# lionnus/I-ViT

Hardware: AMD Instinct MI355X
Metric: images/sec DeiT-B INT8 @batch256, 1→8 MI355X; % INT8 MFMA peak (higher is better)
Workload: dtype int8; 1 GPU; DeiT-B INT8 integer-only forward, batch 256 per GPU, 224x224; global_batch=256, parallelism=dp1, launch=hip-graph replay, bitwidth=8, activation_ranges=power-of-two, operators=I-ViT (IVITIntLayerNorm, Shiftmax, ShiftGELU)

## Files before the change

i-vit_amd/_lib.py:

```python
from __future__ import annotations

import ctypes as C
import os
import subprocess

_HERE = os.path.dirname(os.path.abspath(__file__))
LIB_PATH = os.path.join(_HERE, "libivit_hip.so")
CSRC = os.path.join(_HERE, "csrc")

i64, i32, u32, f32, vp = C.c_int64, C.c_int32, C.c_uint32, C.c_float, C.c_void_p
ci = C.c_int

SIGNATURES = {
    "ivit_quantize_input_f32_i8": [vp, vp, i64, f32, vp],
    "ivit_quantize_patchify_f32_i8": [vp, vp, ci, ci, ci, ci, f32, vp],
    "ivit_gemm_i8_requant": [vp, i64, vp, i64, vp, vp, vp, vp, i64, ci, ci, ci, vp],
    "ivit_gemm_i8_requant_residual": [vp, i64, vp, i64, vp, vp, vp, vp, i64, u32, i32, u32, i32, vp, i64, ci, ci, ci, vp],
    "ivit_attention_fused_i8_ex": [vp, vp, ci, ci, ci, ci, u32, i32, f32, u32, i32, ci, vp],
    "ivit_layernorm_i8_ex": [vp, i64, ci, ci, vp, vp, vp, vp, vp, i64, ci, vp],
    "ivit_layernorm_i8_compat": [vp, i64, ci, ci, vp, vp, vp, vp, vp, vp, vp, i64, ci, vp],
    "ivit_attention_fused_i8_compat": [vp, vp, ci, ci, ci, ci, u32, i32, f32, u32, i32, vp, ci, vp],
    "ivit_attention_fused_i8_compat_band": [vp, vp, ci, ci, ci, ci, u32, i32, f32, u32, i32, vp, vp, ci, ci, vp],
    "ivit_attention_fused_i8_wide": [vp, vp, ci, ci, ci, ci, u32, i32, f32, u32, i32, vp, vp, ci, ci, ci, vp],
    "ivit_attention_fused_i8_long": [vp, vp, ci, ci, ci, ci, u32, i32, f32, u32, i32, vp, vp, ci, ci, vp],
    "ivit_attention_fused_i8_wide_long": [vp, vp, ci, ci, ci, ci, u32, i32, f32, u32, i32, vp, vp, ci, ci, ci, vp],
    "ivit_attention_cls_i8": [vp, vp, vp, vp, i64, ci, ci, ci, ci, u32, i32, f32, u32, i32, vp, vp, ci, vp],
    "ivit_shiftgelu_build_lut_ex": [f32, u32, i32, vp, vp, vp],
    "ivit_shiftgelu_lut_i8_ex": [vp, i64, ci, ci, vp, vp, i64, ci, vp],
    "ivit_pack_weight_frags_i8": [vp, i64, ci, ci, vp, vp],
    "ivit_pack_weight_frags16_i8": [vp, i64, ci, ci, vp, vp],
    "ivit_tile_operand_i8": [vp, i64, i64, ci, vp, vp],
    "ivit_untile_operand_i8": [vp, i64, ci, vp, i64, vp],
    "ivit_gemm_i8_requant_ex": [vp, i64, vp, i64, vp, vp, vp, vp, i64, ci, ci, ci, ci, vp],
    "ivit_gemm_i8_requant_residual_ex": [vp, i64, vp, i64, vp, vp, vp, vp, i64, u32, i32, u32, i32, vp, i64, ci, ci, ci, ci, vp],
    "ivit_gemm_i8_requant_bits_ex": [vp, i64, vp, i64, vp, vp, vp, vp, i64, ci, ci, ci, ci, ci, vp],
    "ivit_gemm_i8_requant_residual_bits_ex": [vp, i64, vp, i64, vp, vp, vp, vp, i64, u32, i32, u32, i32, vp, i64, ci, ci, ci, ci, ci, ci, vp],
    "ivit_gemm_i8_requant_qkv_ex": [vp, i64, vp, i64, vp, vp, vp, vp, ci, ci, ci, ci, ci, ci, ci, vp],
    "ivit_gemm_i8_requant_qkv_planes_ex": [vp, i64, vp, i64, vp, vp, vp, vp, ci, ci, ci, ci, ci, ci, ci, ci, ci, vp],
    "ivit_gemm_plan": [ci, ci, ci, ci, ci, vp],
    "ivit_gemm_i8_requant_residual_i16": [vp, i64, vp, i64, vp, vp, vp, vp, i64, u32, i32, u32, i32, vp, i64, ci, ci, ci, vp],
    "ivit_gemm_i8_requant_lut_ex": [vp, i64, vp, i64, vp, vp, vp, vp, vp, i64, ci, ci, ci, ci, vp],
    "ivit_gemm_i8_requant_i16": [vp, i64, vp, i64, vp, vp, vp, vp, i64, ci, ci, ci, vp],
    "ivit_gemm_i8_requant_residual_i16_ex": [vp, i64, vp, i64, vp, vp, vp, vp, i64, u32, i32, u32, i32, vp, i64, ci, ci, ci, ci, vp],
    "ivit_gemm_i8_requant_i16_residual_i16_ex": [vp, i64, vp, i64, vp, vp, vp, vp, i64, u32, i32, u32, i32, vp, i64, ci, ci, ci, ci, vp],
    "ivit_gemm_i8_requant_qkv": [vp, i64, vp, i64, vp, vp, vp, vp, ci, ci, ci, ci, ci, ci, vp],
    "ivit_gemm_i8_i32": [vp, i64, vp, i64, vp, vp, i64, ci, ci, ci, vp],
    "ivit_attention_fused_i8": [vp, vp, ci, ci, ci, ci, u32, i32, f32, u32, i32, vp],
    "ivit_layernorm_i8": [vp, i64, ci, ci, vp, vp, vp, vp, vp, i64, vp],
    "ivit_layernorm_i32_f32": [vp, i64, ci, ci, vp, vp, vp, i64, vp],
    "ivit_layernorm_i8_f32": [vp, i64, ci, ci, ci, ci, ci, vp, vp, vp, vp, vp, i64, ci, vp],
    "ivit_layernorm_i16_f32": [vp, i64, ci, ci, ci, ci, ci, f32, vp, vp, vp, i64, ci, vp],
    "ivit_ibert_layernorm_i8_f32": [vp, i64, ci, ci, ci, ci, ci, f32, vp, vp, f32, vp, i64, ci, vp],
    "ivit_ibert_layernorm_i16_f32": [vp, i64, ci, ci, ci, ci, ci, f32, vp, vp, f32, vp, i64, ci, vp],
    "ivit_layernorm_f32_f32": [vp, i64, ci, ci, vp, ci, vp, vp, vp, i64, vp],
    "ivit_layernorm_f32_f32_ex": [vp, i64, ci, ci, vp, ci, vp, vp, vp, i64, ci, vp],
    "ivit_shiftmax_f32_i8": [vp, i64, ci, ci, f32, vp, i64, vp],
    "ivit_shiftmax_f32_i16": [vp, i64, ci, ci, f32, ci, vp, i64, vp],
    "ivit_bgemm_pv_i16_i8": [vp, vp, vp, ci, ci, ci, ci, vp],
    "ivit_bgemm_pv_i32_i8": [vp, vp, vp, ci, ci, ci, ci, i64, vp],
    "ivit_quantize_input_f32_i32": [vp, vp, i64, f32, ci, vp],
    "ivit_shiftgelu_i8": [vp, i64, ci, ci, f32, u32, i32, vp, i64, vp],
    "ivit_shiftgelu_i8_i32": [vp, i64, ci, ci, f32, vp, i64, vp],
    "ivit_shiftgelu_build_lut": [f32, u32, i32, vp, vp],
    "ivit_shiftgelu_lut_i8": [vp, i64, ci, ci, vp, vp, i64, vp],
    "ivit_shiftmax_i8": [vp, i64, ci, ci, f32, vp, i64, vp],
    "ivit_requant_i32": [vp, i64, ci, vp, vp, ci, vp, vp, vp, ci, ci, vp, vp],
    "ivit_residual_requant_i8": [vp, u32, i32, vp, u32, i32, vp, i64, vp],
    "ivit_residual_requant_i8_bits": [vp, u32, i32, vp, u32, i32, vp, i64, ci, vp],
    "ivit_embed_assemble_i8": [vp, vp, vp, u32, i32, vp, ci, ci, ci, vp],
    "ivit_embed_assemble_i8_bits": [vp, vp, vp, u32, i32, vp, ci, ci, ci, ci, vp],
    "ivit_embed_assemble_i16": [vp, vp, vp, u32, i32, vp, ci, ci, ci, vp],
    "ivit_head_argmax": [vp, vp, ci, ci, vp, vp, vp],
    "ivit_head_topk": [vp, vp, ci, ci, ci, ci, vp, vp, vp, vp, vp],
    "ivit_logits_topk_f32": [vp, ci, ci, ci, ci, vp, vp, vp, vp],
    "ivit_bgemm_qk_i8": [vp, vp, vp, ci, ci, ci, ci, vp],
    "ivit_bgemm_pv_i8": [vp, vp, vp, ci, ci, ci, ci, vp],
    "ivit_f32_to_i32": [vp, i64, ci, vp, ci, ci, vp, vp],
    "ivit_i32_to_f32": [vp, i64, ci, vp, ci, vp, vp],
    "ivit_narrow_i32_i8": [vp, vp, i64, vp, vp],
    "ivit_quantize_patchify_ld_f32_i8": [vp, vp, i64, ci, ci, ci, ci, f32, vp],
    "ivit_quantize_patchify_u8_i8": [vp, vp, i64, ci, ci, ci, ci, vp, vp],
    "ivit_quantize_patchify_hw_f32_i8": [vp, vp, i64, ci, ci, ci, ci, ci, f32, vp],
    "ivit_quantize_patchify_hw_u8_i8": [vp, vp, i64, ci, ci, ci, ci, ci, vp, vp],
    "ivit_minmax_f32": [vp, i64, vp, vp],
    "ivit_quantile_pair_f32": [vp, i64, f32, f32, vp, vp, i64, vp],
    "ivit_weight_quant_rows_f32_i8": [vp, i64, ci, ci, vp, vp, i64, vp, vp],
    "ivit_bias_quant_f32_i32": [vp, vp, ci, f32, vp, vp, vp, vp],
    "ivit_shiftmax_i32_i8": [vp, i64, ci, ci, f32, vp, i64, vp],
    "ivit_requant_i8_i16": [vp, u32, i32, vp, i64, vp],
    "ivit_residual_requant_i16": [vp, ci, vp, vp, u32, i32, vp, u32, i32, vp, i64, ci, ci, ci, ci, ci, vp],
    "ivit_layernorm_i16_i8": [vp, ci, ci, vp, vp, vp, vp, vp, i64, ci, ci, ci, ci, vp],
    "ivit_layernorm_i16_i8_compat": [vp, ci, ci, f32, ci, vp, vp, vp, vp, vp, i64, ci, ci, ci, ci, vp],
    "ivit_patch_merge_i16": [vp, vp, ci, ci, ci, ci, vp],
    "ivit_window_rows": [vp, vp, ci, ci, ci, i64, ci, ci, ci, vp],
    "ivit_avgpool_requant_i8": [vp, vp, ci, ci, ci, u32, i32, vp],
    "ivit_avgpool_requant_i8_literal": [vp, vp, ci, ci, ci, f32, u32, i32, vp],
    "ivit_avgpool_f32_literal": [vp, vp, ci, ci, ci, vp],
    "ivit_ibert_gelu_i32": [vp, i64, f32, f32, f32, vp, vp],
    "ivit_ibert_softmax_i32": [vp, i64, ci, ci, f32, f32, f32, f32, f32, u32, i32, ci, vp, i64, vp, vp],
    "ivit_ibert_layernorm_i32_f32": [vp, i64, ci, ci, vp, vp, f32, vp, i64, vp],
    "ivit_ibert_layernorm_i32_f32_ex": [vp, i64, ci, ci, vp, vp, f32, vp, i64, ci, vp],
    "ivit_ibert_gelu_build_lut": [f32, f32, f32, f32, f32, u32, i32, vp, vp],
    "ivit_ibert_softmax_build_table": [f32, f32, f32, f32, f32, f32, u32, i32, vp, vp],
    "ivit_attention_fused_i8_ibert": [vp, vp, ci, ci, ci, ci, u32, i32, u32, i32, vp, vp, ci, ci, vp],
    "ivit_attention_fused_i8_ibert_wide": [vp, vp, ci, ci, ci, ci, u32, i32, u32, i32, vp, vp, ci, ci, ci, vp],
    "ivit_attention_fused_i8_ibert_long": [vp, vp, ci, ci, ci, ci, u32, i32, u32, i32, vp, vp, ci, ci, vp],
    "ivit_attention_probs_u8": [vp, vp, i64, ci, ci, ci, ci, ci, u32, i32, f32, vp, vp, ci, vp],
    "ivit_attention_probs_u8_ibert": [vp, vp, i64, ci, ci, ci, ci, ci, u32, i32, vp, vp, ci, vp],
    "ivit_ibert_layernorm_i8": [vp, i64, ci, ci, f32, vp, vp, f32, vp, vp, vp, i64, ci, vp],
    "ivit_ibert_layernorm_i16_i8": [vp, i64, ci, ci, f32, vp, vp, f32, vp, vp, vp, i64, vp],
    "ivit_ibert_layernorm_i16_i8_ex": [vp, i64, ci, ci, f32, vp, vp, f32, vp, vp, vp, i64, ci, vp],
    "ivit_ibert_layernorm_i16_i8_win": [vp, i64, ci, ci, f32, vp, vp, f32, vp, vp, vp, i64, ci, ci, ci, ci, ci, vp],
    "ivit_ibert_gelu_f32_f32": [vp, i64, f32, f32, f32, f32, f32, vp, vp],
    "ivit_ibert_softmax_f32_f32": [vp, i64, ci, ci, f32, f32, f32, f32, f32, f32, u32, i32, ci, vp, i64, vp, vp],
    "ivit_ibert_layernorm_f32_f32": [vp, i64, ci, ci, vp, ci, vp, vp, f32, vp, i64, vp],
    "ivit_ibert_layernorm_f32_f32_ex": [vp, i64, ci, ci, vp, ci, vp, vp, f32, vp, i64, ci, vp],
    "ivit_window_attention_i8": [vp, vp, i64, vp, vp, ci, ci, ci, ci, ci, ci, u32, i32, u32, i32, f32, u32, i32, vp],
    "ivit_window_attention_i8_compat": [vp, vp, i64, vp, vp, ci, ci, ci, ci, ci, ci, u32, i32, u32, i32, f32, u32, i32, vp, vp, vp],
    "ivit_window_attention_i8_band": [vp, vp, i64, vp, vp, ci, ci, ci, ci, ci, u32, i32, u32, i32, f32, u32, i32, vp, ci, ci, ci, ci, ci, ci, vp],
    "ivit_window_attention_i8_unwindow": [vp, vp, i64, vp, vp, ci, ci, ci, ci, ci, ci, u32, i32, u32, i32, f32, u32, i32, vp, vp,
                                          ci, ci, ci, ci, vp],
    "ivit_window_attention_i8_long": [vp, vp, i64, vp, vp, ci, ci, ci, ci, ci, ci, u32, i32, u32, i32, f32, u32, i32, vp, vp, vp, ci,
                                      ci, ci, ci, ci, ci, ci, vp],
    "ivit_window_attention_i8_ibert": [vp, vp, i64, vp, vp, f32, ci, ci, ci, ci, ci, u32, i32, u32, i32, u32, i32, vp, ci, ci, ci, ci,
                                       ci, ci, vp],
    "ivit_window_attention_probs_u8": [vp, vp, i64, vp, vp, ci, ci, ci, ci, ci, ci, u32, i32, u32, i32, f32, vp, vp, vp, ci, ci, vp],
    "ivit_window_attention_probs_u8_ibert": [vp, vp, i64, vp, vp, f32, ci, ci, ci, ci, ci, u32, i32, u32, i32, vp, ci, vp],
    "ivit_eval_geometry": [ci, ci, ci, ci, vp],
    "ivit_resize_crop_workspace": [vp, ci, ci, vp, vp],
    "ivit_resize_crop_bicubic_u8": [vp, vp, vp, ci, ci, ci, ci, ci, vp, i64, vp, vp],
    "ivit_eval_geometry_hw": [ci, ci, ci, ci, ci, ci, ci, vp],
    "ivit_resize_crop_workspace_hw": [vp, ci, ci, ci, vp, vp],
    "ivit_resize_crop_bicubic_hw_u8": [vp, vp, vp, ci, ci, ci, ci, ci, ci, vp, i64, vp, vp],
    "ivit_jpeg_probe": [vp, i64, vp],
    "ivit_jpeg_plan_image": [vp, i64, vp, i64, vp],
    "ivit_jpeg_workspace": [vp, i64, vp, vp, ci, vp, vp],
    "ivit_jpeg_decode_host": [vp, i64, vp, i64],
    "ivit_jpeg_decode_u8": [vp, vp, ci, i64, i64, i64, vp, i64, vp, vp, vp],
    "ivit_tokens_to_nchw_i8_f32": [vp, i64, ci, ci, ci, ci, ci, f32, vp, vp],
    "ivit_tokens_to_nchw_i16_f32": [vp, i64, ci, ci, ci, ci, ci, f32, vp, vp],
    "ivit_tokens_to_nchw_i8": [vp, i64, ci, ci, ci, ci, ci, vp, vp],
    "ivit_tokens_to_nchw_i16": [vp, i64, ci, ci, ci, ci, ci, vp, vp],
    "ivit_dequant_rows_i8_f32": [vp, i64, i64, ci, f32, vp, i64, vp],
    "ivit_rows_rnorm_i8_f32": [vp, i64, i64, ci, vp, vp],
    "ivit_knn_topk_i8": [vp, i64, ci, vp, i64, ci, ci, vp, ci, ci, vp, vp, vp, i64, vp],
    "ivit_knn_workspace_bytes": [ci, ci, ci, ci, vp],
    "ivit_knn_vote_f32": [vp, vp, vp, ci, ci, ci, ci, vp, vp, vp],
    "ivit_gram_i8_i64": [vp, i64, i64, ci, ci, ci, vp, vp, i64, vp],
    "ivit_gram_workspace_bytes": [i64, ci, ci, vp],
    "ivit_group_sums_i8_i64": [vp, i64, i64, ci, vp, vp, ci, ci, vp, vp],
}


LAB_SIGNATURES = {
# ... 99 lines not shown
```

i-vit_amd/csrc/gemm.hip:

```cpp
#include <type_traits>
#include "gemm_common.h"

namespace {

template <int EPIW>
__global__ __launch_bounds__(NT) void gemm_i8_kernel(GemmArgs g)
{
    constexpr int EPI = epi_kind(EPIW);
    __shared__ __attribute__((aligned(16))) char smem[SMEM_BYTES + BN * 8];

    const int nblk = g.tiles_m * g.tiles_n;
    const int bid = blockIdx.x;
    const int q8 = nblk >> 3, r8 = nblk & 7, xcd = bid & 7;
    const int lid = (xcd < r8 ? xcd * (q8 + 1) : r8 * (q8 + 1) + (xcd - r8) * q8) + (bid >> 3);
    const int tm = lid / g.tiles_n, tn = lid - tm * g.tiles_n;
    const int m0 = tm * BM, n0 = tn * BN;

    const int tid = threadIdx.x;
    const int lane = tid & 63, wave = tid >> 6;
    const int wm = wave >> 1, wn = wave & 1;
    const int h = lane >> 5, l31 = lane & 31;
    if constexpr (EPI != EPI_I32 && EPI != EPI_RQ16 && EPI != EPI_RQ16_RES16) fill_rq_table(g, smem + SMEM_BYTES, n0, BN, tid);

    const int srow = tid >> 2, sc = tid & 3;
// ... 653 lines not shown
            lds_read16_async_off<128>(bq[2], ba);
            lds_read16_async_off<192>(bq[3], ba);
#pragma unroll
            for (int i = 0; i < 4; ++i) {
                lds_wait(bq[i]);
#pragma unroll
                for (int j = 0; j < 2 * TJ; ++j) acc16[i][j] = bq[i];
            }
        } else {
        v4i bq[2][4];
#pragma unroll
        for (int i = 0; i < 2; ++i)
#pragma unroll
            for (int q = 0; q < 4; ++q)
                lds_read16_async(bq[i][q], lds_addr(tab) + (unsigned)(WR_CH * 8 + 4 * (64 * wave + 32 * i + 8 * q + 4 * h)));
#pragma unroll
        for (int i = 0; i < 2; ++i)
#pragma unroll
            for (int q = 0; q < 4; ++q) {
                lds_wait(bq[i][q]);
                const v4i b4 = bq[i][q];
#pragma unroll
                for (int j = 0; j < TJ; ++j) {
                    acc[i][j][4 * q + 0] = b4.x;
                    acc[i][j][4 * q + 1] = b4.y;
                    acc[i][j][4 * q + 2] = b4.z;
                    acc[i][j][4 * q + 3] = b4.w;
                }
            }
        }
        load_frags(I0{}, I0{}, af0);
        if constexpr (ABL & 16)
            { if constexpr (ABL & 2048) tv[1] = __builtin_amdgcn_s_memtime(); else if (stamp) stamp[1] = __builtin_amdgcn_s_memtime(); }
        int kt = 0;
        for (; kt + 3 < nk; kt += 3) {
            step(kt, wr0, wr1, wr2, T{}, F{}, I0{});
            step(kt + 1, wr1, wr2, wr0, T{}, F{}, I1{});
            step(kt + 2, wr2, wr0, wr1, T{}, F{}, I2{});
        }
        step(kt, wr0, wr1, wr2, T{}, F{}, I0{});
        step(kt + 1, wr1, wr2, wr0, F{}, F{}, I1{});
        step(kt + 2, wr2, wr0, wr1, F{}, T{}, I2{});
        if constexpr (ABL & 16)
            { if constexpr (ABL & 2048) tv[2] = __builtin_amdgcn_s_memtime(); else if (stamp) stamp[2] = __builtin_amdgcn_s_memtime(); }
        const bool more = nxt.m0 >= 0;
        prefetch(more ? nxt : cur);
        struct Hook {
            decltype(table_issue)& ti;
            decltype(table_write)& tw;
            int n0;
            char* dst;
            bool more;
            mutable PersTableLoad ld;
            IVIT_DEV void issue() const { if (more) ld = ti(n0); }
            IVIT_DEV void consume() const
            {
                asm volatile("s_waitcnt vmcnt(0)" ::: "memory");
                if (more) tw(ld, dst);
            }
        };
        Hook hook{table_issue, table_write, nxt.n0, tab_next, more, PersTableLoad{0u, 0, 0, false}};
        if constexpr (ABL & 1) {
            int sum = 0;
            if constexpr (S16) {
#pragma unroll
                for (int i = 0; i < 4; ++i)
#pragma unroll
                    for (int j = 0; j < 2 * TJ; ++j) sum ^= acc16[i][j][0] ^ acc16[i][j][1] ^ acc16[i][j][2] ^ acc16[i][j][3];
            } else {
#pragma unroll
            for (int i = 0; i < 2; ++i)
#pragma unroll
                for (int j = 0; j < TJ; ++j)
#pragma unroll
                    for (int r = 0; r < 16; ++r) sum ^= acc[i][j][r];
            }
            if (sum == 0x12345679) reinterpret_cast<int*>(g.out)[tid] = sum;
            hook.issue();
            hook.consume();
        } else {
            int tid_o = tid;
            asm volatile("" : "+v"(tid_o));
            if constexpr (S16) asm volatile("s_nop 15\n\ts_nop 15" ::: "memory");
            if constexpr (S16 && (EPI == EPI_RQ || EPI == EPI_RESID || EPI == EPI_QKV)) {
                epilogue_direct_16<EPIW, 2 * TJ, (ABL & (2048 | 4096)), Hook>(acc16, g, tab, cur.m0 + wtok, cur.n0, wch, (tid_o >> 4) & 3, tid_o & 15, hook,
                                                                               g.lut ? reinterpret_cast<const unsigned char*>(smem + WR_LUT) : nullptr,
                                                                               (ABL & 2048) ? tv : nullptr);
            } else if constexpr (S16) {
                static_assert(!S16 || EPI != EPI_RQ16_RES16, "the 16-bit epilogue exists for the 32x32 form only");
                epilogue_i8_16<EPIW, 2 * TJ, BIG_NT, WR_CH, Hook>(acc16, g, cs, tab, cur.m0, cur.n0, 64 * wave, tid_o, (tid_o >> 4) & 3,
                                                                          tid_o & 15, hook,
                                                                          g.lut ? reinterpret_cast<const unsigned char*>(smem + WR_LUT) : nullptr);
            } else if constexpr (EPI == EPI_RQ16_RES16)
                epilogue_rq16_res16<TJ, BIG_NT, Hook>(acc, g, cs, cur.m0, cur.n0, 64 * wave, tid_o, (tid_o >> 5) & 1, tid_o & 31, hook);
            else
            epilogue_i8<EPIW, 2, TJ, 32 * TJ, BIG_NT, WR_CH, Hook>(acc, g, cs, tab, cur.m0, cur.n0, 64 * wave, 0, tid_o, (tid_o >> 5) & 1,
                                                                      tid_o & 31, hook,
                                                                      g.lut ? reinterpret_cast<const unsigned char*>(smem + WR_LUT) : nullptr);
        }
    };

    const int G = gridDim.x, b = blockIdx.x;
    WrWork cur = wr_work(g, 0, b, G);
    if (cur.m0 < 0) return;
    table_write(table_issue(cur.n0), smem + WR_RING + WR_CS);
    if (g.lut) smem[WR_LUT + tid] = (char)g.lut[tid];
    prefetch(cur);
    asm volatile("s_waitcnt vmcnt(1)" ::: "memory");

    for (int it = 0; cur.m0 >= 0; ++it) {
        char* tab = smem + WR_RING + WR_CS + (it & 1) * WR_TAB;
        char* tab_next = smem + WR_RING + WR_CS + ((it + 1) & 1) * WR_TAB;
        const WrWork nxt = wr_work(g, it + 1, b, G);
        if constexpr (ABL & 16) {
            unsigned long long* sbase = (ABL & 2048) ? g.stamp : reinterpret_cast<unsigned long long*>(const_cast<int8_t*>(g.res));
            stamp = (tid == 0 && it < 4) ? sbase + (blockIdx.x * 4 + it) * 32 : nullptr;
            if constexpr (ABL & 2048) {
                tv[0] = __builtin_amdgcn_s_memtime();
                tv[7] = __builtin_amdgcn_s_memrealtime();
            } else if (stamp) {
                stamp[0] = __builtin_amdgcn_s_memtime();
                stamp[16] = __builtin_amdgcn_s_memrealtime();
            }
        }
        if constexpr (S16 && (EPI == EPI_RQ || EPI == EPI_RESID || EPI == EPI_QKV) && !(ABL & 16)) {
            if (cur.half == 2) run(std::integral_constant<int, 2>{}, cur, nxt, tab, tab_next);
            else if (cur.half) run(std::integral_constant<int, 1>{}, cur, nxt, tab, tab_next);
            else run(std::integral_constant<int, 0>{}, cur, nxt, tab, tab_next);
        } else {
            if (cur.half) run(std::integral_constant<int, 1>{}, cur, nxt, tab, tab_next);
            else run(std::integral_constant<int, 0>{}, cur, nxt, tab, tab_next);
        }
        if constexpr (ABL & 16)
            {
                if constexpr (ABL & 2048) {
                    if (stamp) {
                        stamp[0] = tv[0]; stamp[1] = tv[1]; stamp[2] = tv[2]; stamp[3] = __builtin_amdgcn_s_memtime();
                        stamp[20] = tv[4]; stamp[21] = tv[5]; stamp[22] = tv[6]; stamp[16] = tv[7];
                    }
                } else if (stamp) stamp[3] = __builtin_amdgcn_s_memtime();
            }
        cur = nxt;
    }
}

constexpr int SK_MAXN = 320, SK_MAXK = 128, SK_NT = 512, SK_WPB = SK_NT / 64;
constexpr int SK_SMEM = SK_MAXN * SK_MAXK + SK_MAXN * 12 + (SK_MAXN / 4) * 4;

template <int EPIW, int NKS = 0>
__global__ __launch_bounds__(SK_NT, 2) void gemm_i8_skinny_kernel(GemmArgs g)
{
    constexpr int EPI = epi_kind(EPIW);
    constexpr int QLO = epi_lo(EPIW, EPI_NARROW_MID), QHI = epi_hi(EPIW, EPI_NARROW_MID);
    static_assert(EPI == EPI_RQ || EPI == EPI_QKV, "skinny-K form: int8 outputs");
    __shared__ __attribute__((aligned(16))) char smem[SK_SMEM];
    const int tid = threadIdx.x, lane = tid & 63, wave = tid >> 6;
    const int g4 = lane >> 4, l15 = lane & 15;
    const int nks = NKS ? NKS : (g.K >> 5), nsub = g.N >> 4;
    float2* const lohi = reinterpret_cast<float2*>(smem + SK_MAXN * SK_MAXK);
    int* const bias = reinterpret_cast<int*>(smem + SK_MAXN * SK_MAXK + SK_MAXN * 8);
    unsigned* const coff = reinterpret_cast<unsigned*>(smem + SK_MAXN * SK_MAXK + SK_MAXN * 12);
    for (int q = tid; q < nsub * nks * 64; q += SK_NT) {
        const int f = q >> 6, L = q & 63, i = f / nks, ks = f - i * nks;
        *reinterpret_cast<long*>(smem + (size_t)q * 8) =
            *reinterpret_cast<const long*>(g.W + (int64_t)(16 * i + (L & 15)) * g.ldw + 8 * nks * (L >> 4) + 8 * ks);
    }
    if constexpr (EPI == EPI_QKV) {
        const int cdim = g.heads * g.head_dim, nb = g.M / g.tokens;
        for (int j = tid; j < (g.N >> 2); j += SK_NT) {
            const int c = 4 * j, which = c / cdim, rem = c - which * cdim;
            const int hh = rem / g.head_dim, d0 = rem - hh * g.head_dim;
            coff[j] = (unsigned)(((which * nb * g.heads + hh) * g.tokens) * g.head_dim + d0);
        }
    }
    for (int c = tid; c < g.N; c += SK_NT) {
        const int bv = g.bias ? g.bias[c] : 0;
        const double M = dyadic_mult(g.m[c], g.e[c]);
        const float mf = (float)M;
        const int bits = __float_as_int(mf);
        float lo = ((double)mf > M) ? __int_as_float(bits - 1) : mf, hi = ((double)mf < M) ? __int_as_float(bits + 1) : mf;
        lo = __int_as_float(__float_as_int(lo) - 2);
        hi = __int_as_float(__float_as_int(hi) + 2);
        lohi[c] = make_float2(lo, hi);
        bias[c] = bv;
    }
    __syncthreads();
    int8_t* const out = reinterpret_cast<int8_t*>(g.out);
    const int nstrips = (g.M + 15) >> 4;
    for (int strip = blockIdx.x * SK_WPB + wave; strip < nstrips; strip += gridDim.x * SK_WPB) {
        const int t = 16 * strip + l15;
        const int8_t* arow = g.A + (int64_t)min(t, g.M - 1) * g.lda + 8 * nks * g4;
        long bf[SK_MAXK / 32] = {0l, 0l, 0l, 0l};
        if (nks == 4) {
            const int4 u0 = *reinterpret_cast<const int4*>(arow), u1 = *reinterpret_cast<const int4*>(arow + 16);
            bf[0] = ((long)(unsigned)u0.y << 32) | (unsigned)u0.x; bf[1] = ((long)(unsigned)u0.w << 32) | (unsigned)u0.z;
            bf[2] = ((long)(unsigned)u1.y << 32) | (unsigned)u1.x; bf[3] = ((long)(unsigned)u1.w << 32) | (unsigned)u1.z;
        } else if (nks == 2) {
            const int4 u0 = *reinterpret_cast<const int4*>(arow);
            bf[0] = ((long)(unsigned)u0.y << 32) | (unsigned)u0.x; bf[1] = ((long)(unsigned)u0.w << 32) | (unsigned)u0.z;
        } else {
#pragma unroll
            for (int ks = 0; ks < SK_MAXK / 32; ++ks) bf[ks] = ks < nks ? *reinterpret_cast<const long*>(arow + 8 * ks) : 0l;
        }
        unsigned qrow_off = 0;
        if constexpr (EPI == EPI_QKV) {
            const int tt = min(t, g.M - 1);
            const int qb = tt / g.tokens, qtok = tt - qb * g.tokens;
            qrow_off = (unsigned)((qb * g.heads * g.tokens + qtok) * g.head_dim);
        }
        for (int i0 = 0; i0 < nsub; i0 += 4) {
            v4i acc[4];
#pragma unroll
            for (int ii = 0; ii < 4; ++ii) {
                const int i = min(i0 + ii, nsub - 1);
                acc[ii] = *reinterpret_cast<const v4i*>(bias + 16 * i + 4 * g4);
#pragma unroll
                for (int ks = 0; ks < SK_MAXK / 32; ++ks)
                    if (ks < nks)
                        acc[ii] = __builtin_amdgcn_mfma_i32_16x16x32_i8(*reinterpret_cast<const long*>(smem + ((size_t)(i * nks + ks) * 64 + lane) * 8),
                                                                         bf[ks], acc[ii], 0, 0, 0);
            }
            int b[4][4];
            unsigned unc = 0;
#pragma unroll
            for (int ii = 0; ii < 4; ++ii) {
                const int i = min(i0 + ii, nsub - 1);
#pragma unroll
                for (int r = 0; r < 4; ++r) {
                    const float2 lh = lohi[16 * i + 4 * g4 + r];
                    const float a = (float)acc[ii][r];
                    const int tl = __float_as_int(__builtin_fmaf(a, lh.x, 12582912.0f));
                    const int th = __float_as_int(__builtin_fmaf(a, lh.y, 12582912.0f));
                    asm("v_sad_u32 %0, %1, %2, %3" : "=v"(unc) : "v"(tl), "v"(th), "v"(unc));
                    b[ii][r] = clamp_i32(tl, 0x4B400000 + QLO, 0x4B400000 + QHI);
                }
            }
            if (__builtin_amdgcn_ballot_w64(unc != 0) != 0) {
#pragma unroll
                for (int ii = 0; ii < 4; ++ii) {
                    const int c0 = 16 * min(i0 + ii, nsub - 1) + 4 * g4;
#pragma unroll
                    for (int r = 0; r < 4; ++r) {
                        const double tq = (double)acc[ii][r] * dyadic_mult(g.m[c0 + r], g.e[c0 + r]) + IVIT_MAGIC;
                        b[ii][r] = clamp_i32((int)(unsigned)__double_as_longlong(tq), QLO, QHI);
                    }
                }
            }
            unsigned D[4];
#pragma unroll
            for (int ii = 0; ii < 4; ++ii)
                D[ii] = __builtin_amdgcn_perm((unsigned)b[ii][1], (unsigned)b[ii][0], 0x0c0c0400u) |
                        __builtin_amdgcn_perm((unsigned)b[ii][3], (unsigned)b[ii][2], 0x04000c0cu);
            typedef unsigned v2u __attribute__((ext_vector_type(2)));
            const v2u ab = __builtin_amdgcn_permlane32_swap(D[0], D[2], false, false);
            const v2u cd = __builtin_amdgcn_permlane32_swap(D[1], D[3], false, false);
            const v2u ac = __builtin_amdgcn_permlane16_swap(ab.x, cd.x, false, false);
            const v2u bd = __builtin_amdgcn_permlane16_swap(ab.y, cd.y, false, false);
            const int ci = i0 + g4;
            if (ci < nsub && t < g.M) {
                const int4 v = make_int4((int)ac.x, (int)ac.y, (int)bd.x, (int)bd.y);
                if constexpr (EPI == EPI_QKV) *reinterpret_cast<int4*>(out + coff[4 * ci] + qrow_off) = v;
                else *reinterpret_cast<int4*>(out + (int64_t)t * g.ldo + 16 * ci) = v;
            }
        }
    }
}

constexpr bool epi_has_skinny(int epi) { return epi == EPI_RQ || epi == EPI_QKV; }
constexpr bool epi_has_wreg(int epi) { return epi != EPI_I32 && epi != EPI_RQ16; }
constexpr bool epi_has_wreg16(int epi) { return epi_has_wreg(epi) && epi != EPI_RQ16_RES16; }
constexpr bool epi_has_pers(int epi) { return epi_has_wreg(epi) && epi != EPI_RQ16_RES16; }
constexpr bool epi_int8_out(int epi) { return epi == EPI_RQ || epi == EPI_RESID || epi == EPI_QKV; }
constexpr bool wr_tiles_fit(int N) { return (N + WR_CH - 1) / WR_CH * WR_CH * WR_WASTE_DEN <= N * (WR_WASTE_DEN + 1); }

enum { GEMM_SMALL = IVIT_GEMM_FORM_SMALL, GEMM_PERS = IVIT_GEMM_FORM_PERS, GEMM_WREG = IVIT_GEMM_FORM_WREG, GEMM_WREG16 = IVIT_GEMM_FORM_WREG16,
       GEMM_SKINNY = IVIT_GEMM_FORM_SKINNY };
static_assert(EPI_RQ == IVIT_GEMM_EPI_RQ && EPI_RESID == IVIT_GEMM_EPI_RESID && EPI_QKV == IVIT_GEMM_EPI_QKV && EPI_I32 == IVIT_GEMM_EPI_I32 &&
              EPI_RESID16 == IVIT_GEMM_EPI_RESID16 && EPI_RQ16 == IVIT_GEMM_EPI_RQ16 && EPI_RQ16_RES16 == IVIT_GEMM_EPI_RQ16_RES16,
              "include/ivit_hip.h names the epilogue kinds for ivit_gemm_plan");

struct GemmPlan {
    int form;
    int nks;
    int res_f32;
    int narrow, stamped, ablation;
    int grid, lds;
    int tiles_m, tiles_n, split_from;
    int stagger, stagger_units, cu_turns;
};

int gemm_check(int EPI, const GemmArgs& g, const char* name, int qkv_planes)
{
    IVIT_REQUIRE(g.A && g.W && g.out, "%s: NULL operand", name);
    IVIT_REQUIRE(g.M > 0 && g.N > 0 && g.K > 0, "%s: empty problem M=%d N=%d K=%d", name, g.M, g.N, g.K);
    IVIT_REQUIRE(g.K % BK == 0, "%s: K=%d must be a multiple of %d", name, g.K, BK);
    IVIT_REQUIRE(g.lda >= g.K && g.ldw >= g.K && g.lda % 16 == 0 && g.ldw % 16 == 0,
                 "%s: lda=%lld ldw=%lld must be >= K and multiples of 16", name, (long long)g.lda, (long long)g.ldw);
    IVIT_REQUIRE(((uintptr_t)g.A % 16 == 0) && ((uintptr_t)g.W % 16 == 0) && ((uintptr_t)g.out % 16 == 0),
                 "%s: operands must be 16-byte aligned", name);
    if (EPI == EPI_I32 || EPI == EPI_RQ16 || EPI == EPI_RQ16_RES16) {
        IVIT_REQUIRE(g.N % 4 == 0 && g.ldo % 4 == 0 && g.ldo >= g.N, "%s: N=%d ldo=%lld must be multiples of 4", name,
                     g.N, (long long)g.ldo);
        if (EPI == EPI_RQ16 || EPI == EPI_RQ16_RES16)
            IVIT_REQUIRE(g.m && g.e && ((uintptr_t)g.m % 16 == 0) && ((uintptr_t)g.e % 16 == 0) && ((uintptr_t)g.out % 8 == 0),
                         "%s: requantiser tables missing or misaligned", name);
    } else {
        IVIT_REQUIRE(g.m && g.e, "%s: NULL requantiser table", name);
        IVIT_REQUIRE(((uintptr_t)g.bias % 16 == 0), "%s: bias must be 16-byte aligned", name);
        IVIT_REQUIRE(g.N % 16 == 0, "%s: N=%d must be a multiple of 16", name, g.N);
        IVIT_REQUIRE(((uintptr_t)g.m % 16 == 0) && ((uintptr_t)g.e % 16 == 0), "%s: m/e tables must be 16-byte aligned",
                     name);
    }
    if (EPI == EPI_RQ || EPI == EPI_RESID)
        IVIT_REQUIRE(g.ldo >= g.N && g.ldo % 16 == 0, "%s: ldo=%lld must be >= N and a multiple of 16", name,
                     (long long)g.ldo);
    if (EPI == EPI_RESID)
        IVIT_REQUIRE(g.res && g.ldr >= g.N && g.ldr % 16 == 0 && ((uintptr_t)g.res % 16 == 0),
                     "%s: residual operand missing or misaligned", name);
    if (EPI == EPI_RESID16 || EPI == EPI_RQ16_RES16)
        IVIT_REQUIRE(g.res && g.ldr >= g.N && g.ldr % 8 == 0 && ((uintptr_t)g.res % 16 == 0) && g.ldo >= g.N && g.ldo % 8 == 0,
                     "%s: 16-bit residual / output rows must be 16-byte aligned (ld multiples of 8 elements)", name);
    if (EPI == EPI_QKV) {
        IVIT_REQUIRE(g.tokens > 0 && g.heads > 0 && g.head_dim > 0 && g.head_dim % 16 == 0,
                     "%s: bad head geometry tokens=%d heads=%d head_dim=%d", name, g.tokens, g.heads, g.head_dim);
        IVIT_REQUIRE((int64_t)g.M * g.N < 2147483648ll, "%s: q/k/v output of %lld bytes exceeds the 2 GiB the 32-bit head-major offsets cover",
                     name, (long long)g.M * g.N);
        IVIT_REQUIRE(g.N == qkv_planes * g.heads * g.head_dim && g.M % g.tokens == 0,
                     "%s: N=%d != %d*heads*head_dim or M=%d %% tokens=%d != 0", name, g.N, qkv_planes, g.M, g.tokens);
    }
    return IVIT_OK;
}

int gemm_plan(int EPIW, const GemmArgs& g, const char* name, GemmPlan& p)
{
    const int EPI = epi_kind(EPIW);
    const bool lab_forms = IVIT_LAB && EPIW == EPI;
    const bool blocks = g.a_blocks || g.w_blocks;
    p = GemmPlan{};
    if (epi_has_skinny(EPI) && !blocks && !g.w_frags && !g.out_blocks && !g.lut && g.M >= SK_MIN_M && g.K >= 32 && g.K <= SK_MAXK &&
        g.K % 32 == 0 && g.N >= 16 && g.N <= SK_MAXN && g.N % 16 == 0 && g.lda % 16 == 0 && g.ldw % 8 == 0 && (EPI == EPI_QKV || g.ldo % 16 == 0) &&
        (EPI != EPI_QKV || g.head_dim % 16 == 0) && (int64_t)g.M * (EPI == EPI_QKV ? g.N : g.ldo) < 4294967296ll && !g_force_small &&
        !(g_debug_flags2 & LAB2_NO_SKINNY)) {
        const int nstrips = (g.M + 15) >> 4, wgs = (nstrips + SK_WPB - 1) / SK_WPB;
        p.form = GEMM_SKINNY;
        p.grid = wgs < WG_SLOTS ? wgs : WG_SLOTS;
        const bool any_k = (g_debug_flags2 & LAB2_SKINNY_ANY_K) != 0;
        p.nks = any_k ? 0 : g.K == 128 ? 4 : g.K == 64 ? 2 : 0;
        return IVIT_OK;
    }
    const bool big = g.M >= BIG_MIN_M && !g_force_small;
    if (blocks && !g.w_frags) {
        IVIT_REQUIRE(epi_has_wreg(EPI) && big && g.N >= BCH,
                     "%s: block-layout operands need the persistent kernel (M >= 2048, N >= 128, requantising epilogue)", name);
        IVIT_REQUIRE(!g.a_blocks || g.lda == g.K, "%s: a block-layout A operand is dense (lda == K)", name);
        IVIT_REQUIRE(!g.w_blocks || g.ldw == g.K, "%s: a block-layout W operand is dense (ldw == K)", name);
    }
    if (g.w_frags) IVIT_REQUIRE(!g.a_blocks || g.lda == g.K, "%s: a block-layout A operand is dense (lda == K)", name);
    IVIT_REQUIRE(!g.lut || (g.w_frags && EPI == EPI_RQ), "%s: the output map needs the fragment-packed weight form (IVIT_W_FRAGS)", name);
    if (g.w_frags) {
        IVIT_REQUIRE(epi_has_wreg(EPI) && big && g.N >= 128 && g.N % 64 == 0 && (g.K / BK) % 3 == 0 && !g.w_blocks,
                     "%s: the fragment-packed weight needs M >= 2048, N >= 128, N %% 64 == 0, K %% 192 == 0 and a requantising epilogue", name);
        p.tiles_m = (g.M + WR_TOK - 1) / WR_TOK;
        p.tiles_n = (g.N + WR_CH - 1) / WR_CH;
        if (IVIT_LAB && epi_int8_out(EPI) && g.w_frags == 2 && !g.lut && (g_debug_flags2 & LAB2_WR16_NARROW) && !(g_debug_flags2 & LAB2_WR16_STAMPS)) {
            p.narrow = 1;
            p.tiles_n = (g.N + WR_CH / 2 - 1) / (WR_CH / 2);
        }
        const int ntiles = p.tiles_m * p.tiles_n;
        const int rounds = ntiles / WG_SLOTS, R = ntiles - rounds * WG_SLOTS;
        const bool halves = !p.narrow && !(g_debug_flags & LAB_NO_HALVES);
        const bool split = halves && rounds > 0 && R > 0 && 2 * R <= ((g_debug_flags & LAB_SPLIT_ALL_SLOTS) ? WG_SLOTS : HALF_TILE_WGS);
        p.split_from = split ? rounds * WG_SLOTS : ntiles;
        const bool all_halves = halves && g.w_frags == 2 && rounds == 0 && 2 * ntiles <= WG_SLOTS;
        if (all_halves) p.split_from = 0;
        p.grid = all_halves ? 2 * ntiles : (ntiles < WG_SLOTS ? ntiles : WG_SLOTS);
        constexpr unsigned ABLATIONS = 1u << 1 | 1u << 2 | 1u << 4 | 1u << 6 | 1u << 7 | 1u << 8 | 1u << 14 | 1u << 15 | 1u << LAB_WR_STAMPS;
        const int abl = g_debug_flags & LAB_WR_ABLATION;
        if (lab_forms && EPI == EPI_RQ && ((ABLATIONS >> abl) & 1)) {
            p.form = GEMM_WREG;
            p.ablation = abl;
            if (abl == LAB_WR_STAMPS && (g_debug_flags & LAB_ONE_PER_CU)) p.grid = 256, p.lds = 40960;
            return IVIT_OK;
        }
        if (g.w_frags == 1) {
            p.form = GEMM_WREG;
            return IVIT_OK;
        }
        IVIT_REQUIRE(epi_has_wreg16(EPI), "%s: IVIT_W_FRAGS16 has no 16-bit epilogue; pack the weights with ivit_pack_weight_frags_i8", name);
        IVIT_REQUIRE(((int64_t)g.M + 16) * (EPI == EPI_QKV ? g.N : g.ldo) < 4294967296ll &&
                         (EPI != EPI_RESID || ((int64_t)g.M + 16) * g.ldr < 4294967296ll),
                     "%s: IVIT_W_FRAGS16 addresses its output (and residual) with 32-bit offsets: operand of 4 GiB or more", name);
        p.form = GEMM_WREG16;
        p.stamped = lab_forms && (EPI == EPI_RQ || EPI == EPI_RESID) && (g_debug_flags2 & LAB2_WR16_STAMPS) && g.stamp;
        p.res_f32 = EPI == EPI_RESID && g.res_f32;
        return IVIT_OK;
    }
    if (epi_has_pers(EPI) && big && g.N >= BCH) {
        p.form = GEMM_PERS;
        p.stagger = (g_debug_flags & LAB_NO_STAGGER) ? 0 : WG_SLOTS;
        p.tiles_m = (g.M + BTOK - 1) / BTOK;
        p.tiles_n = (g.N + BCH - 1) / BCH;
        const int ntiles = p.tiles_m * p.tiles_n;
        const bool one_per_cu = (g_debug_flags & LAB_ONE_PER_CU) != 0;
        const int SLOTS = (one_per_cu || (g_debug_flags & LAB_GRID_256)) ? WG_SLOTS / 2 : WG_SLOTS;
        const int rounds = ntiles / SLOTS, R = ntiles - rounds * SLOTS;
        const bool split = R > 0 && !(g_debug_flags & LAB_NO_HALVES) &&
                           2 * R <= ((g_debug_flags & LAB_SPLIT_ALL_SLOTS) ? SLOTS : HALF_TILE_WGS) && !one_per_cu;
        p.split_from = split ? rounds * SLOTS : ntiles;
        p.cu_turns = (g_debug_flags & LAB_CU_TURNS) ? 1 : 0;
        p.stagger_units = (g_debug_flags >> LAB_DELAY_SHIFT) & LAB_DELAY_MASK;
        p.grid = rounds > 0 ? SLOTS : (split ? 2 * R : R);
        p.lds = one_per_cu ? 20480 : 0;
        return IVIT_OK;
    }
    p.form = GEMM_SMALL;
    p.tiles_m = (g.M + BM - 1) / BM;
    p.tiles_n = (g.N + BN - 1) / BN;
    p.grid = p.tiles_m * p.tiles_n;
    return IVIT_OK;
}

#if IVIT_LAB
bool launch_wreg_ablation(GemmArgs& g, const GemmPlan& p, ivit_stream_t stream)
{
    if (p.ablation == LAB_WR_STAMPS) g.res = (const int8_t*)g_stamp_buf;
    switch (p.ablation) {
#define IVIT_WR_ABL(v) case v: hipLaunchKernelGGL((gemm_i8_wreg_kernel<EPI_RQ, v>), dim3(p.grid), dim3(BIG_NT), p.lds, ivit_stream(stream), g); return true
        IVIT_WR_ABL(16); IVIT_WR_ABL(1); IVIT_WR_ABL(2); IVIT_WR_ABL(4); IVIT_WR_ABL(6); IVIT_WR_ABL(8); IVIT_WR_ABL(14); IVIT_WR_ABL(15); IVIT_WR_ABL(7);
#undef IVIT_WR_ABL
        default: return false;
    }
}
#endif

template <int EPIW>
int gemm_launch(GemmArgs& g, const GemmPlan& p, const char* name, ivit_stream_t stream)
{
    constexpr int EPI = epi_kind(EPIW);
    g.tiles_m = p.tiles_m; g.tiles_n = p.tiles_n; g.split_from = p.split_from; g.narrow = p.narrow;
    g.stagger = p.stagger; g.stagger_units = p.stagger_units; g.cu_turns = p.cu_turns;
#define IVIT_GEMM_LAUNCH(kernel, threads) hipLaunchKernelGGL(kernel, dim3(p.grid), dim3(threads), p.lds, ivit_stream(stream), g)
#define IVIT_GEMM_NO_KERNEL IVIT_REQUIRE(false, "%s: no kernel of form %d for this epilogue", name, p.form)
    switch (p.form) {
        case GEMM_SKINNY:
            if constexpr (epi_has_skinny(EPI)) {
                if (p.nks == 4) IVIT_GEMM_LAUNCH((gemm_i8_skinny_kernel<EPIW, 4>), SK_NT);
                else if (p.nks == 2) IVIT_GEMM_LAUNCH((gemm_i8_skinny_kernel<EPIW, 2>), SK_NT);
                else IVIT_GEMM_LAUNCH((gemm_i8_skinny_kernel<EPIW, 0>), SK_NT);
                break;
            }
            IVIT_GEMM_NO_KERNEL;
        case GEMM_WREG16:
            if constexpr (epi_has_wreg16(EPI)) {
#if IVIT_LAB
                if constexpr ((EPI == EPI_RQ || EPI == EPI_RESID) && EPIW == EPI) {
                    if (p.stamped) {
                        if (p.res_f32) IVIT_GEMM_LAUNCH((gemm_i8_wreg_kernel<EPI, 16 | 2048 | 4096, true>), BIG_NT);
                        else IVIT_GEMM_LAUNCH((gemm_i8_wreg_kernel<EPI, 16 | 2048, true>), BIG_NT);
                        break;
                    }
                }
#endif
                if constexpr (EPI == EPI_RESID) {
                    if (p.res_f32) {
                        IVIT_GEMM_LAUNCH((gemm_i8_wreg_kernel<EPIW, 4096, true>), BIG_NT);
                        break;
                    }
                }
                IVIT_GEMM_LAUNCH((gemm_i8_wreg_kernel<EPIW, 0, true>), BIG_NT);
                break;
            }
            IVIT_GEMM_NO_KERNEL;
        case GEMM_WREG:
            if constexpr (epi_has_wreg(EPI)) {
#if IVIT_LAB
                if constexpr (EPIW == EPI_RQ) {
                    if (launch_wreg_ablation(g, p, stream)) break;
                }
#endif
                IVIT_GEMM_LAUNCH((gemm_i8_wreg_kernel<EPIW>), BIG_NT);
                break;
            }
            IVIT_GEMM_NO_KERNEL;
        case GEMM_PERS:
            if constexpr (epi_has_pers(EPI)) {
                IVIT_GEMM_LAUNCH((gemm_i8_pers_kernel<EPIW>), BIG_NT);
                break;
            }
            IVIT_GEMM_NO_KERNEL;
        case GEMM_SMALL:
            IVIT_GEMM_LAUNCH(gemm_i8_kernel<EPIW>, NT);
            break;
        default:
            IVIT_GEMM_NO_KERNEL;
    }
#undef IVIT_GEMM_LAUNCH
#undef IVIT_GEMM_NO_KERNEL
    IVIT_CHECK_LAUNCH(name);
}

template <int EPIW>
int launch_gemm(GemmArgs& g, const char* name, ivit_stream_t stream, int qkv_planes = 3)
{
    if (const int rc = gemm_check(epi_kind(EPIW), g, name, qkv_planes)) return rc;
#if IVIT_LAB
    g.stamp = reinterpret_cast<unsigned long long*>(g_stamp_buf);
#endif
    GemmPlan p;
    if (const int rc = gemm_plan(EPIW, g, name, p)) return rc;
    return gemm_launch<EPIW>(g, p, name, stream);
}

GemmArgs gemm_args(const int8_t* A, int64_t lda, const int8_t* W, int64_t ldw, const int32_t* bias, const uint32_t* m, const int32_t* e,
                   void* out, int64_t ldo, int M, int N, int K)
{
    GemmArgs g{};
    g.A = A; g.lda = lda; g.W = W; g.ldw = ldw; g.bias = bias; g.m = m; g.e = e;
    g.out = out; g.ldo = ldo; g.M = M; g.N = N; g.K = K;
    return g;
}

int gemm_layouts(GemmArgs& g, int layouts, int allowed, const char* name)
{
    constexpr int FRAGS = IVIT_W_FRAGS | IVIT_W_FRAGS16;
    IVIT_REQUIRE((layouts & ~allowed) == 0 && (layouts & FRAGS) != FRAGS, "%s: unknown layout bits", name);
    g.a_blocks = (layouts & IVIT_A_BLOCKS) != 0;
    g.w_blocks = (layouts & IVIT_W_BLOCKS) != 0;
    g.out_blocks = (layouts & IVIT_OUT_BLOCKS) != 0;
    g.w_frags = (layouts & IVIT_W_FRAGS16) ? 2 : (layouts & IVIT_W_FRAGS) ? 1 : 0;
    IVIT_REQUIRE(!g.out_blocks || (g.N % 64 == 0 && g.ldo == g.N && ((int64_t)g.M + 15) * g.N < 2147483648ll),
                 "%s: block-layout output needs N %% 64 == 0, ldo == N and a buffer below 2 GiB", name);
    return IVIT_OK;
}
constexpr int LAYOUTS_RQ = IVIT_A_BLOCKS | IVIT_W_BLOCKS | IVIT_OUT_BLOCKS | IVIT_W_FRAGS | IVIT_W_FRAGS16;
constexpr int LAYOUTS_IN = LAYOUTS_RQ & ~IVIT_OUT_BLOCKS;
constexpr int LAYOUTS_RQ16_RES16 = IVIT_A_BLOCKS | IVIT_W_FRAGS;

__global__ __launch_bounds__(256) void pack_weight_frags_kernel(const int8_t* W, int64_t ldw, int N, int K, int8_t* dst)
{
    const int c16 = K >> 4, n64 = (N + 63) & ~63;
    const int64_t total = (int64_t)n64 * c16;
    for (int64_t q = (int64_t)blockIdx.x * 256 + threadIdx.x; q < total; q += (int64_t)gridDim.x * 256) {
        const int n = (int)(q / c16), k = (int)(q - (int64_t)n * c16) << 4;
        int4 v = make_int4(0, 0, 0, 0);
        if (n < N) v = *reinterpret_cast<const int4*>(W + (int64_t)n * ldw + k);
        const int64_t off = ((int64_t)(n >> 6) * (K >> 6) + (k >> 6)) * 4096 + ((((n >> 5) & 1) * 2 + ((k >> 5) & 1)) * 2 + ((k >> 4) & 1)) * 512 + (n & 31) * 16;
        *reinterpret_cast<int4*>(dst + off) = v;
    }
}

__global__ __launch_bounds__(256) void pack_weight_frags16_kernel(const int8_t* W, int64_t ldw, int N, int K, int8_t* dst)
{
    const int c16 = K >> 4, n64 = (N + 63) & ~63;
    const int64_t total = (int64_t)n64 * c16;
    for (int64_t q = (int64_t)blockIdx.x * 256 + threadIdx.x; q < total; q += (int64_t)gridDim.x * 256) {
        const int n = (int)(q / c16), k = (int)(q - (int64_t)n * c16) << 4;
        int4 v = make_int4(0, 0, 0, 0);
        if (n < N) v = *reinterpret_cast<const int4*>(W + (int64_t)n * ldw + k);
        const int64_t off = ((int64_t)(n >> 6) * (K >> 6) + (k >> 6)) * 4096 + ((n >> 4) & 3) * 1024 + ((k >> 4) & 3) * 256 + (n & 15) * 16;
        *reinterpret_cast<int4*>(dst + off) = v;
    }
}

}

IVIT_EXPORT int ivit_pack_weight_frags16_i8(const int8_t* W, int64_t ldw, int N, int K, int8_t* dst, ivit_stream_t stream)
{
    IVIT_REQUIRE(W && dst && N > 0 && K > 0 && K % 64 == 0 && ldw >= K && ldw % 16 == 0 && ((uintptr_t)W % 16 == 0) && ((uintptr_t)dst % 16 == 0),
                 "ivit_pack_weight_frags16_i8: bad operand (K must be a multiple of 64, rows 16-byte aligned)");
    const int64_t total = (int64_t)((N + 63) & ~63) * (K >> 4);
    const int grid = (int)((total + 255) / 256 < 4096 ? (total + 255) / 256 : 4096);
    hipLaunchKernelGGL(pack_weight_frags16_kernel, dim3(grid), dim3(256), 0, ivit_stream(stream), W, ldw, N, K, dst);
    IVIT_CHECK_LAUNCH("ivit_pack_weight_frags16_i8");
}

IVIT_EXPORT int ivit_pack_weight_frags_i8(const int8_t* W, int64_t ldw, int N, int K, int8_t* dst, ivit_stream_t stream)
{
    IVIT_REQUIRE(W && dst && N > 0 && K > 0 && K % 64 == 0 && ldw >= K && ldw % 16 == 0 && ((uintptr_t)W % 16 == 0) && ((uintptr_t)dst % 16 == 0),
                 "ivit_pack_weight_frags_i8: bad operand (K must be a multiple of 64, rows 16-byte aligned)");
    const int64_t total = (int64_t)((N + 63) & ~63) * (K >> 4);
    const int grid = (int)((total + 255) / 256 < 4096 ? (total + 255) / 256 : 4096);
    hipLaunchKernelGGL(pack_weight_frags_kernel, dim3(grid), dim3(256), 0, ivit_stream(stream), W, ldw, N, K, dst);
    IVIT_CHECK_LAUNCH("ivit_pack_weight_frags_i8");
}

template <int EPIW>
static int gemm_requant_ex(const char* name, const int8_t* A, int64_t lda, const int8_t* W, int64_t ldw, const int32_t* bias,
                           const uint32_t* m, const int32_t* e, int8_t* out, int64_t ldo, int M, int N, int K, int layouts,
                           ivit_stream_t stream)
{
    GemmArgs g = gemm_args(A, lda, W, ldw, bias, m, e, out, ldo, M, N, K);
    if (const int rc = gemm_layouts(g, layouts, LAYOUTS_RQ, name)) return rc;
    return launch_gemm<EPIW>(g, name, stream);
}

IVIT_EXPORT int ivit_gemm_i8_requant_ex(const int8_t* A, int64_t lda, const int8_t* W, int64_t ldw, const int32_t* bias,
                                     const uint32_t* m, const int32_t* e, int8_t* out, int64_t ldo, int M, int N,
                                     int K, int layouts, ivit_stream_t stream)
{
    return gemm_requant_ex<EPI_RQ>("ivit_gemm_i8_requant_ex", A, lda, W, ldw, bias, m, e, out, ldo, M, N, K, layouts, stream);
}

IVIT_EXPORT int ivit_gemm_i8_requant_bits_ex(const int8_t* A, int64_t lda, const int8_t* W, int64_t ldw, const int32_t* bias,
                                             const uint32_t* m, const int32_t* e, int8_t* out, int64_t ldo, int M, int N,
                                             int K, int layouts, int bits, ivit_stream_t stream)
{
    const char* name = "ivit_gemm_i8_requant_bits_ex";
    IVIT_REQUIRE(bits == 4 || bits == 8, "%s: bits=%d must be 4 or 8", name, bits);
    if (bits == 8) return gemm_requant_ex<EPI_RQ>(name, A, lda, W, ldw, bias, m, e, out, ldo, M, N, K, layouts, stream);
    return gemm_requant_ex<EPI_RQ | EPI_NARROW_MID>(name, A, lda, W, ldw, bias, m, e, out, ldo, M, N, K, layouts, stream);
}

IVIT_EXPORT int ivit_gemm_i8_requant_lut_ex(const int8_t* A, int64_t lda, const int8_t* W, int64_t ldw, const int32_t* bias,
                                            const uint32_t* m, const int32_t* e, const int8_t* lut, int8_t* out, int64_t ldo,
                                            int M, int N, int K, int layouts, ivit_stream_t stream)
{
    const char* name = "ivit_gemm_i8_requant_lut_ex";
    GemmArgs g = gemm_args(A, lda, W, ldw, bias, m, e, out, ldo, M, N, K);
    g.lut = lut;
// ... 3 lines not shown
}

IVIT_EXPORT int ivit_gemm_i8_requant(const int8_t* A, int64_t lda, const int8_t* W, int64_t ldw, const int32_t* bias,
                                     const uint32_t* m, const int32_t* e, int8_t* out, int64_t ldo, int M, int N,
                                     int K, ivit_stream_t stream)
{
    return ivit_gemm_i8_requant_ex(A, lda, W, ldw, bias, m, e, out, ldo, M, N, K, 0, stream);
}

static void residual_f32_form(GemmArgs& g)
{
    g.Mf_main = (float)g.M_main;
    g.Mf_res = (float)g.M_res;
    g.res_f32 = 0;
    if (!(g.M_main > 0.0 && g.M_res > 0.0 && g.M_main < 16384.0 && g.M_res < 16384.0)) return;
    const double Md[2] = {g.M_main, g.M_res};
    const float Mf[2] = {g.Mf_main, g.Mf_res};
    for (int t = 0; t < 2; ++t)
        for (int k = -128; k <= 127; ++k) {
            const float tf = __builtin_fmaf((float)k, Mf[t], 12582912.0f);
            int bits;
            __builtin_memcpy(&bits, &tf, 4);
            const double td = __builtin_fma((double)k, Md[t], IVIT_MAGIC);
            long long lb;
            __builtin_memcpy(&lb, &td, 8);
            if (bits - 0x4B400000 != (int)(unsigned)lb) return;
        }
    g.res_f32 = 1;
}

template <int EPIW>
static int gemm_residual_ex(const char* name, const int8_t* A, int64_t lda, const int8_t* W, int64_t ldw, const int32_t* bias,
                            const uint32_t* m, const int32_t* e, const int8_t* res, int64_t ldr, uint32_t m_main, int32_t e_main,
                            uint32_t m_res, int32_t e_res, int8_t* out, int64_t ldo, int M, int N, int K, int layouts,
                            ivit_stream_t stream)
{
    GemmArgs g = gemm_args(A, lda, W, ldw, bias, m, e, out, ldo, M, N, K);
    g.res = res; g.ldr = ldr;
    g.M_main = ivit_dyadic_to_double(m_main, e_main);
    g.M_res = ivit_dyadic_to_double(m_res, e_res);
    residual_f32_form(g);
    IVIT_REQUIRE(g.M_main < 1048576.0 && g.M_res < 1048576.0, "%s: residual multiplier >= 2^20 is outside the int8 fast path", name);
    if (const int rc = gemm_layouts(g, layouts, LAYOUTS_IN, name)) return rc;
    return launch_gemm<EPIW>(g, name, stream);
}

IVIT_EXPORT int ivit_gemm_i8_requant_residual_ex(const int8_t* A, int64_t lda, const int8_t* W, int64_t ldw,
                                              const int32_t* bias, const uint32_t* m, const int32_t* e,
                                              const int8_t* res, int64_t ldr, uint32_t m_main, int32_t e_main,
                                              uint32_t m_res, int32_t e_res, int8_t* out, int64_t ldo, int M, int N,
                                              int K, int layouts, ivit_stream_t stream)
{
    return gemm_residual_ex<EPI_RESID>("ivit_gemm_i8_requant_residual_ex", A, lda, W, ldw, bias, m, e, res, ldr, m_main, e_main, m_res,
                                       e_res, out, ldo, M, N, K, layouts, stream);
}

IVIT_EXPORT int ivit_gemm_i8_requant_residual_bits_ex(const int8_t* A, int64_t lda, const int8_t* W, int64_t ldw,
                                                      const int32_t* bias, const uint32_t* m, const int32_t* e,
                                                      const int8_t* res, int64_t ldr, uint32_t m_main, int32_t e_main,
                                                      uint32_t m_res, int32_t e_res, int8_t* out, int64_t ldo, int M, int N,
                                                      int K, int layouts, int bits_mid, int bits_out, ivit_stream_t stream)
{
    const char* name = "ivit_gemm_i8_requant_residual_bits_ex";
    IVIT_REQUIRE((bits_mid == 4 || bits_mid == 8) && (bits_out == 4 || bits_out == 8), "%s: bits_mid=%d, bits_out=%d must be 4 or 8",
                 name, bits_mid, bits_out);
#define IVIT_RESID_BITS(EPIW) \
    return gemm_residual_ex<EPIW>(name, A, lda, W, ldw, bias, m, e, res, ldr, m_main, e_main, m_res, e_res, out, ldo, M, N, K, layouts, stream)
    if (bits_mid == 8 && bits_out == 8) IVIT_RESID_BITS(EPI_RESID);
    if (bits_mid == 4 && bits_out == 8) IVIT_RESID_BITS(EPI_RESID | EPI_NARROW_MID);
    if (bits_mid == 8) IVIT_RESID_BITS(EPI_RESID | EPI_NARROW_OUT);
    IVIT_RESID_BITS(EPI_RESID | EPI_NARROW_MID | EPI_NARROW_OUT);
#undef IVIT_RESID_BITS
}

IVIT_EXPORT int ivit_gemm_i8_requant_residual(const int8_t* A, int64_t lda, const int8_t* W, int64_t ldw,
                                              const int32_t* bias, const uint32_t* m, const int32_t* e,
                                              const int8_t* res, int64_t ldr, uint32_t m_main, int32_t e_main,
                                              uint32_t m_res, int32_t e_res, int8_t* out, int64_t ldo, int M, int N,
                                              int K, ivit_stream_t stream)
{
    return ivit_gemm_i8_requant_residual_ex(A, lda, W, ldw, bias, m, e, res, ldr, m_main, e_main, m_res, e_res, out, ldo, M, N, K, 0, stream);
}

IVIT_EXPORT int ivit_gemm_i8_requant_residual_i16_ex(const int8_t* A, int64_t lda, const int8_t* W, int64_t ldw,
                                                  const int32_t* bias, const uint32_t* m, const int32_t* e,
                                                  const int16_t* res, int64_t ldr, uint32_t m_main, int32_t e_main,
                                                  uint32_t m_res, int32_t e_res, int16_t* out, int64_t ldo, int M, int N,
                                                  int K, int layouts, ivit_stream_t stream)
{
    GemmArgs g = gemm_args(A, lda, W, ldw, bias, m, e, out, ldo, M, N, K);
    if (const int rc = gemm_layouts(g, layouts, LAYOUTS_IN, "ivit_gemm_i8_requant_residual_i16_ex")) return rc;
    g.res = reinterpret_cast<const int8_t*>(res); g.ldr = ldr;
    g.M_main = ivit_dyadic_to_double(m_main, e_main);
    g.M_res = ivit_dyadic_to_double(m_res, e_res);
    IVIT_REQUIRE(g.M_main < 32768.0 && g.M_res < 32768.0, "ivit_gemm_i8_requant_residual_i16: residual multiplier too large");
    return launch_gemm<EPI_RESID16>(g, "ivit_gemm_i8_requant_residual_i16", stream);
}

IVIT_EXPORT int ivit_gemm_i8_requant_residual_i16(const int8_t* A, int64_t lda, const int8_t* W, int64_t ldw,
                                                  const int32_t* bias, const uint32_t* m, const int32_t* e,
                                                  const int16_t* res, int64_t ldr, uint32_t m_main, int32_t e_main,
                                                  uint32_t m_res, int32_t e_res, int16_t* out, int64_t ldo, int M, int N,
                                                  int K, ivit_stream_t stream)
{
    return ivit_gemm_i8_requant_residual_i16_ex(A, lda, W, ldw, bias, m, e, res, ldr, m_main, e_main, m_res, e_res, out, ldo, M, N, K, 0, stream);
}

IVIT_EXPORT int ivit_gemm_i8_requant_qkv_ex(const int8_t* A, int64_t lda, const int8_t* W, int64_t ldw,
                                         const int32_t* bias, const uint32_t* m, const int32_t* e, int8_t* qkv,
                                         int tokens, int heads, int head_dim, int M, int N, int K,
                                         int layouts, ivit_stream_t stream)
{
    GemmArgs g = gemm_args(A, lda, W, ldw, bias, m, e, qkv, 0, M, N, K);
    g.tokens = tokens; g.heads = heads; g.head_dim = head_dim;
    if (const int rc = gemm_layouts(g, layouts, LAYOUTS_IN, "ivit_gemm_i8_requant_qkv_ex")) return rc;
    return launch_gemm<EPI_QKV>(g, "ivit_gemm_i8_requant_qkv_ex", stream);
}

IVIT_EXPORT int ivit_gemm_i8_requant_qkv_planes_ex(const int8_t* A, int64_t lda, const int8_t* W, int64_t ldw,
                                                   const int32_t* bias, const uint32_t* m, const int32_t* e, int8_t* qkv,
                                                   int tokens, int heads, int head_dim, int plane0, int nplanes, int M, int N,
                                                   int K, int layouts, ivit_stream_t stream)
{
    IVIT_REQUIRE(plane0 >= 0 && nplanes >= 1 && plane0 + nplanes <= 3, "ivit_gemm_i8_requant_qkv_planes_ex: planes %d .. %d outside q, k, v",
                 plane0, plane0 + nplanes - 1);
    IVIT_REQUIRE(qkv && M > 0 && heads > 0 && head_dim > 0 && (int64_t)3 * M * heads * head_dim < 2147483648ll,
                 "ivit_gemm_i8_requant_qkv_planes_ex: NULL output or a q/k/v buffer beyond 2 GiB");
    GemmArgs g = gemm_args(A, lda, W, ldw, bias, m, e, qkv + (int64_t)plane0 * M * heads * head_dim, 0, M, N, K);
    g.tokens = tokens; g.heads = heads; g.head_dim = head_dim;
    if (const int rc = gemm_layouts(g, layouts, LAYOUTS_IN, "ivit_gemm_i8_requant_qkv_planes_ex")) return rc;
    return launch_gemm<EPI_QKV>(g, "ivit_gemm_i8_requant_qkv_planes_ex", stream, nplanes);
}

IVIT_EXPORT int ivit_gemm_i8_requant_qkv(const int8_t* A, int64_t lda, const int8_t* W, int64_t ldw,
                                         const int32_t* bias, const uint32_t* m, const int32_t* e, int8_t* qkv,
                                         int tokens, int heads, int head_dim, int M, int N, int K,
                                         ivit_stream_t stream)
{
    return ivit_gemm_i8_requant_qkv_ex(A, lda, W, ldw, bias, m, e, qkv, tokens, heads, head_dim, M, N, K, 0, stream);
}

IVIT_EXPORT int ivit_gemm_i8_requant_i16(const int8_t* A, int64_t lda, const int8_t* W, int64_t ldw, const int32_t* bias,
                                         const uint32_t* m, const int32_t* e, int16_t* out, int64_t ldo, int M, int N, int K,
                                         ivit_stream_t stream)
{
    GemmArgs g = gemm_args(A, lda, W, ldw, bias, m, e, out, ldo, M, N, K);
    return launch_gemm<EPI_RQ16>(g, "ivit_gemm_i8_requant_i16", stream);
}

IVIT_EXPORT int ivit_gemm_i8_requant_i16_residual_i16_ex(const int8_t* A, int64_t lda, const int8_t* W, int64_t ldw,
                                                         const int32_t* bias, const uint32_t* m, const int32_t* e,
                                                         const int16_t* res, int64_t ldr, uint32_t m_main, int32_t e_main,
                                                         uint32_t m_res, int32_t e_res, int16_t* out, int64_t ldo, int M, int N,
                                                         int K, int layouts, ivit_stream_t stream)
{
    GemmArgs g = gemm_args(A, lda, W, ldw, bias, m, e, out, ldo, M, N, K);
    IVIT_REQUIRE((layouts & ~LAYOUTS_RQ16_RES16) == 0 && ((layouts & IVIT_W_FRAGS) || !(layouts & IVIT_A_BLOCKS)),
                 "ivit_gemm_i8_requant_i16_residual_i16_ex: layouts is 0 or IVIT_W_FRAGS (| IVIT_A_BLOCKS)");
    if (const int rc = gemm_layouts(g, layouts, LAYOUTS_RQ16_RES16, "ivit_gemm_i8_requant_i16_residual_i16_ex")) return rc;
    g.res = reinterpret_cast<const int8_t*>(res); g.ldr = ldr;
    g.M_main = ivit_dyadic_to_double(m_main, e_main);
    g.M_res = ivit_dyadic_to_double(m_res, e_res);
    IVIT_REQUIRE(g.M_main < 32768.0 && g.M_res < 32768.0, "ivit_gemm_i8_requant_i16_residual_i16_ex: residual multiplier too large");
    IVIT_REQUIRE(ldo % 8 == 0 && ldr % 8 == 0 && ((uintptr_t)res % 16 == 0) && ((uintptr_t)out % 16 == 0) && N % 8 == 0,
                 "ivit_gemm_i8_requant_i16_residual_i16_ex: 16-bit rows must be 16-byte aligned");
    return launch_gemm<EPI_RQ16_RES16>(g, "ivit_gemm_i8_requant_i16_residual_i16_ex", stream);
}

IVIT_EXPORT int ivit_gemm_i8_i32(const int8_t* A, int64_t lda, const int8_t* W, int64_t ldw, const int32_t* bias,
                                 int32_t* out, int64_t ldo, int M, int N, int K, ivit_stream_t stream)
{
    GemmArgs g = gemm_args(A, lda, W, ldw, bias, nullptr, nullptr, out, ldo, M, N, K);
    return launch_gemm<EPI_I32>(g, "ivit_gemm_i8_i32", stream);
}

IVIT_EXPORT int ivit_gemm_plan(int epilogue, int M, int N, int K, int layouts, int32_t* out8)
{
    alignas(16) static int8_t operand[16];
    static const int allowed[] = {LAYOUTS_RQ, LAYOUTS_IN, LAYOUTS_IN, 0, LAYOUTS_IN, 0, LAYOUTS_RQ16_RES16};
    const char* name = "ivit_gemm_plan";
    IVIT_REQUIRE(out8 && epilogue >= EPI_RQ && epilogue <= EPI_RQ16_RES16, "%s: NULL out8 or epilogue %d outside IVIT_GEMM_EPI_*", name, epilogue);
    const bool qkv = epilogue == EPI_QKV;
    GemmArgs g = gemm_args(operand, K, operand, K, reinterpret_cast<const int32_t*>(operand), reinterpret_cast<const uint32_t*>(operand),
                           reinterpret_cast<const int32_t*>(operand), operand, qkv ? 0 : N, M, N, K);
    g.res = operand; g.ldr = N;
    g.tokens = 1; g.heads = N / 16; g.head_dim = 16;
    if (const int rc = gemm_layouts(g, layouts, allowed[epilogue], name)) return rc;
    IVIT_REQUIRE(epilogue != EPI_RQ16_RES16 || g.w_frags || !g.a_blocks, "%s: layouts is 0 or IVIT_W_FRAGS (| IVIT_A_BLOCKS)", name);
    if (const int rc = gemm_check(epilogue, g, name, 1)) return rc;
    GemmPlan p;
    if (const int rc = gemm_plan(epilogue, g, name, p)) return rc;
    const int32_t v[8] = {p.form, p.grid, p.tiles_m, p.tiles_n, p.split_from, p.nks, p.lds, wr_tiles_fit(N) ? 1 : 0};
    for (int i = 0; i < 8; ++i) out8[i] = v[i];
    return IVIT_OK;
}

#if IVIT_LAB
bool g_force_small = false;
void* g_stamp_buf = nullptr;
int g_debug_flags = 0;
int g_debug_flags2 = 0;

IVIT_EXPORT int ivit_debug_force_small_gemm(int on)
{
    g_force_small = (on != 0);
    return IVIT_OK;
}

IVIT_EXPORT int ivit_debug_set_gemm_flags(int flags)
{
    g_debug_flags = flags;
    return IVIT_OK;
}

IVIT_EXPORT int ivit_debug_set_gemm_flags2(int flags)
{
    g_debug_flags2 = flags;
    return IVIT_OK;
}

IVIT_EXPORT int ivit_debug_set_stamp_buffer(void* buf)
{
    g_stamp_buf = buf;
    return IVIT_OK;
}
#endif
```

i-vit_amd/csrc/gemm_common.h:

```cpp
#pragma once
#include <type_traits>

#include "common.h"

#if IVIT_LAB
extern bool g_force_small;
extern void* g_stamp_buf;
extern int g_debug_flags;
extern int g_debug_flags2;
#else
constexpr bool g_force_small = false;
constexpr int g_debug_flags = 0;
constexpr int g_debug_flags2 = 0;
#endif
constexpr int LAB_WR_ABLATION = 31;
constexpr int LAB_WR_STAMPS = 16;
constexpr int LAB_NO_STAGGER = 64;
constexpr int LAB_SPLIT_ALL_SLOTS = 2048;
constexpr int LAB_ONE_PER_CU = 4096;
constexpr int LAB_CU_TURNS = 32768;
constexpr int LAB_DELAY_SHIFT = 16, LAB_DELAY_MASK = 63;
constexpr int LAB_GRID_256 = 1 << 26;
constexpr int LAB_NO_HALVES = 1 << 27;
constexpr int LAB2_WR16_STAMPS = 256;
constexpr int LAB2_WR16_NARROW = 8192;
constexpr int LAB2_NO_SKINNY = 1 << 20;
constexpr int LAB2_SKINNY_ANY_K = 1 << 21;

namespace {

constexpr int BM = 128;
constexpr int BN = 128;
constexpr int BK = 64;
constexpr int NT = 256;
constexpr int STAGE_BYTES = (BM + BN) * BK;
constexpr int W_OFF = BM * BK;
constexpr int SMEM_BYTES = 2 * STAGE_BYTES;

enum { EPI_RQ = 0, EPI_RESID = 1, EPI_QKV = 2, EPI_I32 = 3, EPI_RESID16 = 4, EPI_RQ16 = 5, EPI_RQ16_RES16 = 6 };
constexpr int EPI_NARROW_MID = 0x100, EPI_NARROW_OUT = 0x200;
constexpr int epi_kind(int epiw) { return epiw & 0xff; }
constexpr int epi_lo(int epiw, int flag) { return (epiw & flag) ? -8 : -128; }
constexpr int epi_hi(int epiw, int flag) { return (epiw & flag) ? 7 : 127; }


struct GemmArgs {
    const int8_t* A;
    int64_t lda;
    const int8_t* W;
    int64_t ldw;
    const int32_t* bias;
    const uint32_t* m;
    const int32_t* e;
    void* out;
    int64_t ldo;
    const int8_t* res;
    int64_t ldr;
    double M_main, M_res;
    float Mf_main, Mf_res;
    int res_f32;
    int M, N, K;
    int tokens, heads, head_dim;
    int tiles_m, tiles_n;
    int flags;
    int stagger;
    int cu_turns;
    int stagger_units;
    int split_from;
    int narrow;
    int a_blocks, w_blocks;
    int out_blocks;
    int w_frags;
    unsigned long long* stamp;
    const int8_t* lut;
};

IVIT_DEV int swz(int r, int c) { return r * BK + ((c ^ ((r >> 2) & 3)) << 4); }

typedef __attribute__((address_space(3))) void* lds_ptr_t;
typedef float v4f __attribute__((ext_vector_type(4)));
typedef int v2i __attribute__((ext_vector_type(2)));
IVIT_DEV unsigned lds_addr(const void* p) { return (unsigned)(__UINTPTR_TYPE__)(lds_ptr_t)p; }
IVIT_DEV void lds_read16_async(v4f& d, unsigned a) { asm volatile("ds_read_b128 %0, %1" : "=v"(d) : "v"(a)); }
IVIT_DEV void lds_read16_async(v4i& d, unsigned a) { asm volatile("ds_read_b128 %0, %1" : "=v"(d) : "v"(a)); }
template <int OFF> IVIT_DEV void lds_read16_async_off(v4i& d, unsigned a) { asm volatile("ds_read_b128 %0, %1 offset:%2" : "=v"(d) : "v"(a), "n"(OFF)); }
template <int OFF> IVIT_DEV void lds_read16_async_off(v4f& d, unsigned a) { asm volatile("ds_read_b128 %0, %1 offset:%2" : "=v"(d) : "v"(a), "n"(OFF)); }
IVIT_DEV void lds_read8x2_async(v2i& d, unsigned a) { asm volatile("ds_read2_b32 %0, %1 offset1:1" : "=v"(d) : "v"(a)); }
IVIT_DEV void lds_wait(v4f& a, v4f& b) { asm volatile("s_waitcnt lgkmcnt(0)" : "+v"(a), "+v"(b)); }
IVIT_DEV void lds_wait(v4i& a) { asm volatile("s_waitcnt lgkmcnt(0)" : "+v"(a)); }
IVIT_DEV void lds_wait(v2i& a, v2i& b) { asm volatile("s_waitcnt lgkmcnt(0)" : "+v"(a), "+v"(b)); }

IVIT_DEV int rne_clamp16(double p)
{
    p = __builtin_fmin(__builtin_fmax(p, -32768.0), 32767.0);
    return (int)(unsigned)__double_as_longlong(p + IVIT_MAGIC);
}

IVIT_DEV int pack4_i8(int a, int b, int c, int d)
{
    return (a & 0xff) | ((b & 0xff) << 8) | ((c & 0xff) << 16) | ((d & 0xff) << 24);
}


IVIT_DEV void fill_rq_table(const GemmArgs& g, char* rq_lds, int n0, int nch, int tid)
{
    if (tid < nch) {
        float2 lh = make_float2(0.f, 0.f);
        const int c = n0 + tid;
        if (c < g.N) {
            const double M = dyadic_mult(g.m[c], g.e[c]);
            const float mf = (float)M;
            const double back = (double)mf;
            const int bits = __float_as_int(mf);
            lh.x = (back > M) ? __int_as_float(bits - 1) : mf;
            lh.y = (back < M) ? __int_as_float(bits + 1) : mf;
        }
        reinterpret_cast<float2*>(rq_lds)[tid] = lh;
    }
}

struct NoHook {
    IVIT_DEV void issue() const {}
    IVIT_DEV void consume() const {}
};

template <int EPIW, int TOK, int NTHREADS, int CH, typename Hook>
IVIT_DEV void epilogue_phase2(const GemmArgs& g, char* smem, int m0, int n0, int tid, const Hook& hook, const unsigned char* lut_lds)
{
    constexpr int EPI = epi_kind(EPIW);
    constexpr int CSS = CH + 4;
    constexpr int CPR = CH / 16;
    constexpr int NIT = TOK * CPR / NTHREADS;
    int4 rv[NIT];
    int4 rw[EPI == EPI_RESID16 ? NIT : 1][2];
    const bool interior = (m0 + TOK <= g.M) && (n0 + CH <= g.N);
    constexpr int RPI = NTHREADS / CPR;
    static_assert(NTHREADS % CPR == 0, "a thread keeps its chunk column");
    if constexpr (EPI == EPI_RESID || EPI == EPI_RESID16) {
        const int8_t* rbase = g.res + (int64_t)(m0 + tid / CPR) * g.ldr + (n0 + 16 * (tid % CPR));
#pragma unroll
        for (int it = 0; it < NIT; ++it) {
            const int q = tid + NTHREADS * it;
            const int tl = q / CPR, cc = q % CPR;
            const int t = min(m0 + tl, g.M - 1), cn = min(n0 + 16 * cc, g.N - 16);
            if constexpr (EPI == EPI_RESID) {
                rv[it] = *reinterpret_cast<const int4*>(interior ? rbase + (int64_t)(it * RPI) * g.ldr : g.res + (int64_t)t * g.ldr + cn);
            } else {
                const int4* rp = reinterpret_cast<const int4*>(reinterpret_cast<const int16_t*>(g.res) + (int64_t)t * g.ldr + cn);
                rw[it][0] = rp[0];
                rw[it][1] = rp[1];
            }
        }
    }
    asm volatile("s_waitcnt lgkmcnt(0)" ::: "memory");
    __builtin_amdgcn_s_barrier();
    asm volatile("" ::: "memory");

// ... 211 lines not shown
            int b[4][4];
            unsigned unc = 0;
#pragma unroll
            for (int j = 0; j < 4; ++j)
#pragma unroll
                for (int r = 0; r < 4; ++r) {
                    const float a = (float)acc[i][jb + j][r];
                    const int tl = __float_as_int(__builtin_fmaf(a, lo[r], 12582912.0f));
                    const int th = __float_as_int(__builtin_fmaf(a, hi[r], 12582912.0f));
                    asm("v_sad_u32 %0, %1, %2, %3" : "=v"(unc) : "v"(tl), "v"(th), "v"(unc));
                    b[j][r] = clamp_i32(tl, 0x4B400000 + QLO, 0x4B400000 + QHI);
                }
            const bool bad = unc != 0;
            if (__builtin_amdgcn_ballot_w64(bad) != 0) {
                const int c0 = min(n0 + cl, g.N - 4);
                const uint4 m4 = *reinterpret_cast<const uint4*>(g.m + c0);
                const int4 e4 = *reinterpret_cast<const int4*>(g.e + c0);
                const double Mc[4] = {dyadic_mult(m4.x, e4.x), dyadic_mult(m4.y, e4.y), dyadic_mult(m4.z, e4.z), dyadic_mult(m4.w, e4.w)};
#pragma unroll
                for (int j = 0; j < 4; ++j)
#pragma unroll
                    for (int r = 0; r < 4; ++r) {
                        const double t = (double)acc[i][jb + j][r] * Mc[r] + IVIT_MAGIC;
                        b[j][r] = clamp_i32((int)(unsigned)__double_as_longlong(t), QLO, QHI);
                    }
            }
#pragma unroll
            for (int j = 0; j < 4; ++j) {
                const int tl_ = 16 * (jb + j) + l15;
                const unsigned w01 = __builtin_amdgcn_perm((unsigned)b[j][1], (unsigned)b[j][0], 0x0c0c0400u);
                const unsigned w23 = __builtin_amdgcn_perm((unsigned)b[j][3], (unsigned)b[j][2], 0x04000c0cu);
                *reinterpret_cast<unsigned*>(smem + tl_ * CSS + cl) = w01 | w23;
            }
        }
        __builtin_amdgcn_sched_barrier(0);
    }
    epilogue_phase2<EPIW, 16 * NJ, NTHREADS, CH, Hook>(g, smem, m0, n0, tid, hook, lut_lds);
}

template <int LO = -128, int HI = 127>
IVIT_DEV void residual_chunk_f32(int (&v)[4], const int4& res, float Mf_main, float Mf_res, float magic_v)
{
    const int rr[4] = {res.x, res.y, res.z, res.w};
#pragma unroll
    for (int d = 0; d < 4; ++d) {
        unsigned o[4];
#pragma unroll
        for (int bb = 0; bb < 4; ++bb) {
            const float kf = (float)(int)(int8_t)(v[d] >> (8 * bb));
            const float xf = (float)(int)(int8_t)(rr[d] >> (8 * bb));
            float f1, f2;
            asm("v_fma_f32 %0, %1, %2, %3" : "=v"(f1) : "v"(kf), "s"(Mf_main), "v"(magic_v));
            asm("v_fma_f32 %0, %1, %2, %3" : "=v"(f2) : "v"(xf), "s"(Mf_res), "v"(magic_v));
            o[bb] = (unsigned)clamp_i32((int)((unsigned)__float_as_int(f1) + (unsigned)__float_as_int(f2) - 2u * 0x4B400000u), LO, HI);
        }
        v[d] = (int)(__builtin_amdgcn_perm(o[1], o[0], 0x0c0c0400u) | __builtin_amdgcn_perm(o[3], o[2], 0x04000c0cu));
    }
}

template <int LO = -128, int HI = 127>
IVIT_DEV void residual_chunk_f64(int (&v)[4], const int4& res, double M_main, double M_res)
{
    const int rr[4] = {res.x, res.y, res.z, res.w};
#pragma unroll
    for (int d = 0; d < 4; ++d) {
        int o[4];
#pragma unroll
        for (int bb = 0; bb < 4; ++bb) {
            const int k3 = (int)(int8_t)(v[d] >> (8 * bb));
            const int xr = (int)(int8_t)(rr[d] >> (8 * bb));
            o[bb] = clamp_i32(requant_exact(k3, M_main) + requant_exact(xr, M_res), LO, HI);
        }
        v[d] = pack4_i8(o[0], o[1], o[2], o[3]);
    }
}

template <int EPIW, int NJ, int ABL, typename Hook>
IVIT_DEV void epilogue_direct_16(v4i (&acc)[4][NJ], const GemmArgs& g, const char* rq_lds, int m0, int n0, int wch, int g4, int l15,
                                 const Hook& hook, const unsigned char* lut_lds, unsigned long long* st = nullptr)
{
    constexpr int EPI = epi_kind(EPIW);
    constexpr int QLO = epi_lo(EPIW, EPI_NARROW_MID), QHI = epi_hi(EPIW, EPI_NARROW_MID);
    constexpr int RLO = epi_lo(EPIW, EPI_NARROW_OUT), RHI = epi_hi(EPIW, EPI_NARROW_OUT);
    static_assert(NJ % 4 == 0 && (EPI == EPI_RQ || EPI == EPI_RESID || EPI == EPI_QKV), "direct epilogue: int8 outputs");
    __builtin_amdgcn_s_setprio(2);
    hook.issue();
    const unsigned rq_a = lds_addr(rq_lds) + 8u * (unsigned)(wch + 4 * g4);
    const int ncol = n0 + wch;
    const bool col_ok = ncol < g.N;
    const int c = ncol + 16 * g4;
    constexpr int NB = NJ / 4;
    unsigned D[NB][4][4];
    int4 rv[EPI == EPI_RESID ? NB : 1][4];
    v4f lhbuf[2][2];
    lds_read16_async(lhbuf[0][0], rq_a);
    lds_read16_async(lhbuf[0][1], rq_a + 16u);
#pragma unroll
    for (int bi = 0; bi < NB; ++bi) {
        const int jb = 4 * bi;
#pragma unroll
        for (int i = 0; i < 4; ++i) {
            const int sidx = jb + i;
            v4f& lh01 = lhbuf[sidx & 1][0];
            v4f& lh23 = lhbuf[sidx & 1][1];
            lds_wait(lh01, lh23);
            if (sidx + 1 < NJ) {
                const unsigned nxt = rq_a + 8u * (unsigned)(16 * ((i + 1) & 3));
                lds_read16_async(lhbuf[(sidx + 1) & 1][0], nxt);
                lds_read16_async(lhbuf[(sidx + 1) & 1][1], nxt + 16u);
            }
            const float lo[4] = {lh01.x, lh01.z, lh23.x, lh23.z};
            const float hi[4] = {lh01.y, lh01.w, lh23.y, lh23.w};
            int b[4][4];
            unsigned unc = 0;
#pragma unroll
            for (int j = 0; j < 4; ++j)
#pragma unroll
                for (int r = 0; r < 4; ++r) {
                    const float a = (float)acc[i][jb + j][r];
                    const int tl = __float_as_int(__builtin_fmaf(a, lo[r], 12582912.0f));
                    const int th = __float_as_int(__builtin_fmaf(a, hi[r], 12582912.0f));
                    asm("v_sad_u32 %0, %1, %2, %3" : "=v"(unc) : "v"(tl), "v"(th), "v"(unc));
                    b[j][r] = clamp_i32(tl, 0x4B400000 + QLO, 0x4B400000 + QHI);
                }
            if (__builtin_amdgcn_ballot_w64(unc != 0) != 0) {
                const int c0 = min(ncol + 16 * i + 4 * g4, g.N - 4);
                const uint4 m4 = *reinterpret_cast<const uint4*>(g.m + c0);
                const int4 e4 = *reinterpret_cast<const int4*>(g.e + c0);
                const double Mc[4] = {dyadic_mult(m4.x, e4.x), dyadic_mult(m4.y, e4.y), dyadic_mult(m4.z, e4.z), dyadic_mult(m4.w, e4.w)};
#pragma unroll
                for (int j = 0; j < 4; ++j)
#pragma unroll
                    for (int r = 0; r < 4; ++r) {
                        const double t = (double)acc[i][jb + j][r] * Mc[r] + IVIT_MAGIC;
                        b[j][r] = clamp_i32((int)(unsigned)__double_as_longlong(t), QLO, QHI);
                    }
            }
#pragma unroll
            for (int j = 0; j < 4; ++j)
                D[bi][i][j] = __builtin_amdgcn_perm((unsigned)b[j][1], (unsigned)b[j][0], 0x0c0c0400u) |
                              __builtin_amdgcn_perm((unsigned)b[j][3], (unsigned)b[j][2], 0x04000c0cu);
        }
        if constexpr (EPI == EPI_RESID) {
#pragma unroll
            for (int b2 = 0; b2 < NB; ++b2) {
                if (bi != 0) continue;
#pragma unroll
                for (int j = 0; j < 4; ++j) {
                    const int t = min(m0 + 16 * (4 * b2 + j) + l15, g.M - 1);
                    rv[b2][j] = *reinterpret_cast<const int4*>(g.res + ((unsigned)t * (unsigned)g.ldr + (unsigned)min(c, g.N - 16)));
                }
            }
        }
        __builtin_amdgcn_sched_barrier(0);
    }
    int8_t* const out = reinterpret_cast<int8_t*>(g.out);
    float magic_v = 12582912.0f;
    asm volatile("" : "+v"(magic_v));
    unsigned off0, ostep;
    int q_b = 0, q_tok = 0;
    if constexpr (EPI == EPI_QKV) {
        const int cc = min(c, g.N - 16);
        const int cdim = g.heads * g.head_dim;
        const int which = cc / cdim, rem = cc - which * cdim;
        const int hh = rem / g.head_dim, d0 = rem - hh * g.head_dim;
        const int nb = g.M / g.tokens;
        off0 = (unsigned)(((which * nb * g.heads + hh) * g.tokens) * g.head_dim + d0);
        ostep = 0;
        const int t0 = min(m0 + l15, g.M - 1);
        q_b = t0 / g.tokens;
        q_tok = t0 - q_b * g.tokens;
    } else if (EPI == EPI_RQ && g.out_blocks) {
        off0 = block_off(block_row(m0 + l15, g.N), block_col(min(c, g.N - 16)));
        ostep = (unsigned)(g.N >> 6) * 1024u;
    } else {
        off0 = (unsigned)(m0 + l15) * (unsigned)g.ldo + (unsigned)c;
        ostep = 16u * (unsigned)g.ldo;
    }
    if constexpr (ABL & 2048) st[4] = __builtin_amdgcn_s_memtime();
#pragma unroll
    for (int bi = 0; bi < NB; ++bi) {
        const int jb = 4 * bi;
        if (bi == NB - 1) {
            if constexpr (ABL & 2048) st[5] = __builtin_amdgcn_s_memtime();
            hook.consume();
            if constexpr (ABL & 2048) st[6] = __builtin_amdgcn_s_memtime();
        }
#pragma unroll
        for (int j = 0; j < 4; ++j) {
            typedef unsigned v2u __attribute__((ext_vector_type(2)));
            const v2u ab = __builtin_amdgcn_permlane32_swap(D[bi][0][j], D[bi][2][j], false, false);
            const v2u cd = __builtin_amdgcn_permlane32_swap(D[bi][1][j], D[bi][3][j], false, false);
            const v2u ac = __builtin_amdgcn_permlane16_swap(ab.x, cd.x, false, false);
            const v2u bd = __builtin_amdgcn_permlane16_swap(ab.y, cd.y, false, false);
            int v[4] = {(int)ac.x, (int)ac.y, (int)bd.x, (int)bd.y};
            if constexpr (EPI == EPI_RESID) {
                if constexpr (ABL & 4096) residual_chunk_f32<RLO, RHI>(v, rv[bi][j], g.Mf_main, g.Mf_res, magic_v);
                else residual_chunk_f64<RLO, RHI>(v, rv[bi][j], g.M_main, g.M_res);
            }
            if constexpr (EPI == EPI_RQ) {
                if (lut_lds) {
#pragma unroll
                    for (int d = 0; d < 4; ++d) {
                        const unsigned u = (unsigned)v[d] ^ 0x80808080u;
                        v[d] = (int)((unsigned)lut_lds[u & 255] | ((unsigned)lut_lds[(u >> 8) & 255] << 8) |
                                     ((unsigned)lut_lds[(u >> 16) & 255] << 16) | ((unsigned)lut_lds[u >> 24] << 24));
                    }
                }
            }
            const int t = m0 + 16 * (jb + j) + l15;
            unsigned off;
            if constexpr (EPI == EPI_QKV) {
                if (jb + j > 0) {
                    if (g.tokens >= 16) {
                        q_tok += 16;
                        if (q_tok >= g.tokens) { q_tok -= g.tokens; ++q_b; }
                    } else {
                        const int tt = min(t, g.M - 1);
                        q_b = tt / g.tokens;
                        q_tok = tt - q_b * g.tokens;
                    }
                }
                off = off0 + (unsigned)((q_b * g.heads * g.tokens + q_tok) * g.head_dim);
            } else {
                off = off0 + (unsigned)(jb + j) * ostep;
            }
            if (col_ok && t < g.M) *reinterpret_cast<int4*>(out + off) = make_int4(v[0], v[1], v[2], v[3]);
        }
    }
}

template <int TJ, int NTHREADS, typename Hook>
IVIT_DEV void epilogue_rq16_res16(v16i (&acc)[2][TJ], const GemmArgs& g, char* cs, int m0, int n0, int wch, int tid, int h, int l31,
                                  const Hook& hook)
{
    constexpr int CH = 256;
    constexpr int RS = CH * 2 + 8;
    constexpr int CPR = CH / 8;
    constexpr int NIT = 64 * CPR / NTHREADS;
    static_assert(TJ % 2 == 0 && 64 * CPR % NTHREADS == 0, "rounds of 64 tokens");
    __builtin_amdgcn_s_setprio(2);
    hook.issue();
    const int16_t* res = reinterpret_cast<const int16_t*>(g.res);
    int16_t* out = reinterpret_cast<int16_t*>(g.out);
#pragma unroll
    for (int rd = 0; rd < TJ / 2; ++rd) {
#pragma unroll
        for (int grp = 0; grp < 8; ++grp) {
            const int i = grp >> 2, q = grp & 3;
            const int cl = wch + 32 * i + 8 * q + 4 * h;
            const int c0 = min(n0 + cl, g.N - 4);
            const uint4 m4 = *reinterpret_cast<const uint4*>(g.m + c0);
            const int4 e4 = *reinterpret_cast<const int4*>(g.e + c0);
            const double Mc[4] = {dyadic_mult(m4.x, e4.x), dyadic_mult(m4.y, e4.y), dyadic_mult(m4.z, e4.z), dyadic_mult(m4.w, e4.w)};
#pragma unroll
            for (int jj = 0; jj < 2; ++jj) {
                int o[4];
#pragma unroll
                for (int r = 0; r < 4; ++r) {
                    const double p = (double)acc[i][2 * rd + jj][4 * q + r] * Mc[r];
                    o[r] = rne_clamp16(p);
                }
                v2i ow;
                ow.x = (o[0] & 0xffff) | (o[1] << 16);
                ow.y = (o[2] & 0xffff) | (o[3] << 16);
                *reinterpret_cast<v2i*>(cs + (32 * jj + l31) * RS + 2 * cl) = ow;
            }
        }
        v4i rr[NIT];
#pragma unroll
        for (int it = 0; it < NIT; ++it) {
            const int qd = tid + NTHREADS * it;
            const int tl = qd / CPR, cc = qd % CPR;
            const int t = min(m0 + 64 * rd + tl, g.M - 1), cn = min(n0 + 8 * cc, g.N - 8);
            rr[it] = *reinterpret_cast<const v4i*>(res + (int64_t)t * g.ldr + cn);
        }
        asm volatile("s_waitcnt lgkmcnt(0)" ::: "memory");
        __builtin_amdgcn_s_barrier();
        asm volatile("" ::: "memory");
#pragma unroll
        for (int hb = 0; hb < 2; ++hb) {
            constexpr int NH = NIT / 2;
            v4i kk[NH];
#pragma unroll
            for (int u = 0; u < NH; ++u) {
                const int qd = tid + NTHREADS * (NH * hb + u);
                lds_read16_async(kk[u], lds_addr(cs) + (unsigned)((qd / CPR) * RS + 16 * (qd % CPR)));
            }
#pragma unroll
            for (int u = 0; u < NH; ++u) lds_wait(kk[u]);
            if (hb == 1 && rd + 1 < TJ / 2) {
                __builtin_amdgcn_s_barrier();
                asm volatile("" ::: "memory");
            }
            if (rd == 0 && hb == 0) hook.consume();
#pragma unroll
            for (int u = 0; u < NH; ++u) {
                const int it = NH * hb + u;
                const int qd = tid + NTHREADS * it;
                const int tl = qd / CPR, cc = qd % CPR;
                const int t = m0 + 64 * rd + tl, cn = n0 + 8 * cc;
                v4i ov;
#pragma unroll
                for (int d = 0; d < 4; ++d) {
                    const int kw = kk[u][d], rw = rr[it][d];
                    const int lo = clamp_i32(requant_exact((int)(int16_t)kw, g.M_main) + requant_exact((int)(int16_t)rw, g.M_res), -32768, 32767);
// ... 133 lines not shown
```

i-vit_amd/csrc/rowops.hip:

```cpp
#include <limits.h>

#include "common.h"
#include "rowsum.h"

#if IVIT_LAB
int g_ln_wave_per_row = 0;
int g_ln_ablate = 0;
int g_ln_stream_cfg = 0;
unsigned long long* g_ln_stamps = nullptr;
#else
constexpr int g_ln_wave_per_row = 0;
constexpr int g_ln_ablate = 0;
constexpr int g_ln_stream_cfg = 0;
#endif

namespace {

constexpr int NT = 256;
constexpr int WPB = NT / 64;

IVIT_DEV int sx8(int v, int byte) { return (int)(int8_t)(v >> (8 * byte)); }

IVIT_DEV int pack4(int a, int b, int c, int d)
{
    return (a & 0xff) | ((b & 0xff) << 8) | ((c & 0xff) << 16) | ((d & 0xff) << 24);
}

#include "ln_chain.h"

static inline int grid_for_rows(int64_t rows, int rows_per_wave = 1)
{
    int64_t blocks = (rows + WPB * rows_per_wave - 1) / (WPB * rows_per_wave);
    return (int)(blocks < 4096 ? blocks : 4096);
}

struct LnArgs {
    const void* x;
    int64_t ldx;
    int rows, C;
    const float* bias_int;
    const float* s_ln;
    const uint32_t* m;
    const int32_t* e;
    void* out;
    int64_t ldo;
    int out_blocks;
    const int8_t* remap;
    const float* phi;
    int abl;
    int outer;
#if IVIT_LAB
    unsigned long long* stamps;
#endif
};

IVIT_DEV void ln_mean(int sum, int C, int& mean_int)
{
    float mean = (float)sum / (float)C;
    mean_int = (int)rintf(mean);
}

IVIT_DEV float ln_factor(long long var)
{
    const float t = ln_newton10_literal((float)var);
    return floorf((1.0f / t) * 2147483648.0f);
}

IVIT_DEV float ln_newton10(float varf)
{
    float t = 65536.0f;
#pragma unroll
    for (int it = 0; it < 10; ++it) {
        float q = floorf(varf * __builtin_amdgcn_rcpf(t));
        const float r = __builtin_fmaf(-q, t, varf);
        q = (r >= t) ? q + 1.0f : q;
        q = (r < 0.0f) ? q - 1.0f : q;
        t = floorf((t + q) * 0.5f);
    }
    return t;
}

constexpr float LN_NEWTON_CONVERGED = 142883.0f;
IVIT_DEV float ln_std10(int var)
// ... 887 lines not shown
    int64_t i = ((int64_t)blockIdx.x * NT + threadIdx.x) * 4;
    const int64_t stride = (int64_t)gridDim.x * NT * 4;
    for (; i + 3 < n; i += stride) {
        float4 v = *reinterpret_cast<const float4*>(x + i);
        *reinterpret_cast<int*>(out + i) = pack4(quant_sym_i8(v.x, inv_scale), quant_sym_i8(v.y, inv_scale),
                                                 quant_sym_i8(v.z, inv_scale), quant_sym_i8(v.w, inv_scale));
    }
    if (blockIdx.x == 0 && threadIdx.x == 0)
        for (int64_t t = n & ~(int64_t)3; t < n; ++t) out[t] = (int8_t)quant_sym_i8(x[t], inv_scale);
}

__global__ __launch_bounds__(NT) void quantize_i32_kernel(const float* x, int32_t* out, int64_t n, float inv_scale, float lo,
                                                          float hi)
{
    for (int64_t i = (int64_t)blockIdx.x * NT + threadIdx.x; i < n; i += (int64_t)gridDim.x * NT) {
        float v = rintf(inv_scale * x[i]);
        v = fminf(fmaxf(v, lo), hi);
        out[i] = (int32_t)fminf(v, 2147483520.0f);
    }
}

__global__ __launch_bounds__(NT) void patchify_kernel(const float* img, int8_t* A, int64_t lda, int batch, int chans,
                                                      int hw, int patch, float inv_scale)
{
    const int g = hw / patch;
    const int pw4 = patch >> 2;
    const int64_t total = (int64_t)batch * chans * hw * (hw >> 2);
    if (total < 2147483648ll) {
        const unsigned w4 = (unsigned)(hw >> 2), tot = (unsigned)total;
        for (unsigned q = blockIdx.x * NT + threadIdx.x; q < tot; q += gridDim.x * NT) {
            const unsigned r = q / w4, x4 = q - r * w4;
            const unsigned r2 = r / (unsigned)hw, y = r - r2 * (unsigned)hw;
            const unsigned b = r2 / (unsigned)chans, c = r2 - b * (unsigned)chans;
            const float4 v = *reinterpret_cast<const float4*>(img + (size_t)r * hw + 4 * x4);
            const unsigned px = x4 / (unsigned)pw4, kw = (x4 - px * pw4) * 4;
            const unsigned py = y / (unsigned)patch, kh = y - py * patch;
            const int64_t row = ((int64_t)b * g + py) * g + px;
            const unsigned col = (c * patch + kh) * patch + kw;
            *reinterpret_cast<int*>(A + row * lda + col) = pack4(quant_sym_i8(v.x, inv_scale), quant_sym_i8(v.y, inv_scale),
                                                                 quant_sym_i8(v.z, inv_scale), quant_sym_i8(v.w, inv_scale));
        }
        return;
    }
    for (int64_t q = (int64_t)blockIdx.x * NT + threadIdx.x; q < total; q += (int64_t)gridDim.x * NT) {
        int x4 = (int)(q % (hw >> 2));
        int64_t r = q / (hw >> 2);
        int y = (int)(r % hw);
        r /= hw;
        int c = (int)(r % chans);
        int b = (int)(r / chans);
        float4 v = *reinterpret_cast<const float4*>(img + (((int64_t)b * chans + c) * hw + y) * hw + 4 * x4);
        int px = x4 / pw4, kw = (x4 - px * pw4) * 4;
        int py = y / patch, kh = y - py * patch;
        int64_t row = ((int64_t)b * g + py) * g + px;
        int col = (c * patch + kh) * patch + kw;
        *reinterpret_cast<int*>(A + row * lda + col) = pack4(quant_sym_i8(v.x, inv_scale), quant_sym_i8(v.y, inv_scale),
                                                             quant_sym_i8(v.z, inv_scale), quant_sym_i8(v.w, inv_scale));
    }
}

__global__ __launch_bounds__(NT) void patchify_u8_kernel(const uint8_t* img, int8_t* A, int64_t lda, int batch, int chans, int hw,
                                                         int patch, const int8_t* lut)
{
    __shared__ int8_t s_lut[4 * 256];
    for (int i = threadIdx.x; i < chans * 256; i += NT) s_lut[i] = lut[i];
    __syncthreads();
    const int g = hw / patch;
    const int pw4 = patch >> 2;
    const int64_t total = (int64_t)batch * chans * hw * (hw >> 2);
    for (int64_t q = (int64_t)blockIdx.x * NT + threadIdx.x; q < total; q += (int64_t)gridDim.x * NT) {
        int x4 = (int)(q % (hw >> 2));
        int64_t r = q / (hw >> 2);
        int y = (int)(r % hw);
        r /= hw;
        int c = (int)(r % chans);
        int b = (int)(r / chans);
        const unsigned v = *reinterpret_cast<const unsigned*>(img + (((int64_t)b * chans + c) * hw + y) * hw + 4 * x4);
        const int8_t* t = s_lut + 256 * c;
        int px = x4 / pw4, kw = (x4 - px * pw4) * 4;
        int py = y / patch, kh = y - py * patch;
        int64_t row = ((int64_t)b * g + py) * g + px;
        int col = (c * patch + kh) * patch + kw;
        *reinterpret_cast<int*>(A + row * lda + col) = pack4(t[v & 255], t[(v >> 8) & 255], t[(v >> 16) & 255], t[v >> 24]);
    }
}

template <typename TP>
__global__ __launch_bounds__(NT) void patchify_hw_kernel(const TP* img, int8_t* A, int64_t lda, int batch, int chans, int h, int w,
                                                         int patch, float inv_scale, const int8_t* lut)
{
    constexpr bool U8 = sizeof(TP) == 1;
    __shared__ int8_t s_lut[U8 ? 4 * 256 : 4];
    if constexpr (U8) {
        for (int i = threadIdx.x; i < chans * 256; i += NT) s_lut[i] = lut[i];
        __syncthreads();
    }
    const unsigned gh = (unsigned)(h / patch), gw = (unsigned)(w / patch), pw4 = (unsigned)patch >> 2, w4 = (unsigned)w >> 2;
    auto run = [&](auto q, auto total, auto stride) {
        using IT = decltype(q);
        for (; q < total; q += stride) {
            const IT r = q / (IT)w4;
            const unsigned x4 = (unsigned)(q - r * (IT)w4);
            const IT r2 = r / (IT)h;
            const unsigned y = (unsigned)(r - r2 * (IT)h);
            const IT b = r2 / (IT)chans;
            const unsigned c = (unsigned)(r2 - b * (IT)chans);
            const unsigned px = x4 / pw4, kw = (x4 - px * pw4) * 4;
            const unsigned py = y / (unsigned)patch, kh = y - py * (unsigned)patch;
            const int64_t row = ((int64_t)b * gh + py) * gw + px;
            const unsigned col = (c * patch + kh) * patch + kw;
            const TP* src = img + (size_t)r * w + 4 * x4;
            int packed;
            if constexpr (U8) {
                const unsigned v = *reinterpret_cast<const unsigned*>(src);
                const int8_t* t = s_lut + 256 * c;
                packed = pack4(t[v & 255], t[(v >> 8) & 255], t[(v >> 16) & 255], t[v >> 24]);
            } else {
                const float4 v = *reinterpret_cast<const float4*>(src);
                packed = pack4(quant_sym_i8(v.x, inv_scale), quant_sym_i8(v.y, inv_scale), quant_sym_i8(v.z, inv_scale),
                               quant_sym_i8(v.w, inv_scale));
            }
            *reinterpret_cast<int*>(A + row * lda + col) = packed;
        }
    };
    const int64_t total = (int64_t)batch * chans * h * w4;
    if (total < 2147483648ll)
        run((unsigned)(blockIdx.x * NT + threadIdx.x), (unsigned)total, (unsigned)(gridDim.x * NT));
    else
        run((int64_t)blockIdx.x * NT + threadIdx.x, total, (int64_t)gridDim.x * NT);
}

template <int LO, int HI>
__global__ __launch_bounds__(NT) void embed_kernel(const int8_t* patch, const int16_t* pos_add, const int8_t* cls_row,
                                                   double Mq, int8_t* out, int batch, int tokens, int C)
{
    const int cd = C >> 2;
    const int64_t total = (int64_t)batch * tokens * cd;
    for (int64_t q = (int64_t)blockIdx.x * NT + threadIdx.x; q < total; q += (int64_t)gridDim.x * NT) {
        int d = (int)(q % cd);
        int64_t r = q / cd;
        int tok = (int)(r % tokens);
        int b = (int)(r / tokens);
        int res;
        if (tok == 0) {
            res = *reinterpret_cast<const int*>(cls_row + 4 * d);
        } else {
            int w = *reinterpret_cast<const int*>(patch + ((int64_t)b * (tokens - 1) + tok - 1) * C + 4 * d);
            const int16_t* pa = pos_add + (int64_t)tok * C + 4 * d;
            int o[4];
#pragma unroll
            for (int c = 0; c < 4; ++c) o[c] = clamp_i32(requant_exact(sx8(w, c), Mq) + (int)pa[c], LO, HI);
            res = pack4(o[0], o[1], o[2], o[3]);
        }
        *reinterpret_cast<int*>(out + ((int64_t)b * tokens + tok) * C + 4 * d) = res;
    }
}

__global__ __launch_bounds__(NT) void embed16_kernel(const int16_t* patch, const int32_t* pos_add, const int16_t* cls_row,
                                                     double Mq, int16_t* out, int batch, int tokens, int C)
{
    const int cd = C >> 2;
    const int64_t total = (int64_t)batch * tokens * cd;
    for (int64_t q = (int64_t)blockIdx.x * NT + threadIdx.x; q < total; q += (int64_t)gridDim.x * NT) {
        const int d = (int)(q % cd);
        const int64_t r = q / cd;
        const int tok = (int)(r % tokens);
// ... 676 lines not shown
                                 ivit_stream_t stream)
{
    return launch_shiftmax<int8_t>("ivit_shiftmax_i8", x, ldx, rows, L, s, out, ldo, stream);
}

IVIT_EXPORT int ivit_shiftmax_i32_i8(const int32_t* x, int64_t ldx, int rows, int L, float s, int8_t* out, int64_t ldo,
                                     ivit_stream_t stream)
{
    return launch_shiftmax<int32_t>("ivit_shiftmax_i32_i8", x, ldx, rows, L, s, out, ldo, stream);
}

IVIT_EXPORT int ivit_minmax_f32(const float* x, int64_t n, float* out_min_max, ivit_stream_t stream)
{
    IVIT_REQUIRE(x && out_min_max && n > 0, "ivit_minmax_f32: bad operand");
    IVIT_REQUIRE(((uintptr_t)out_min_max % 4 == 0) && ((uintptr_t)x % 4 == 0), "ivit_minmax_f32: misaligned");
    hipStream_t st = ivit_stream(stream);
    unsigned* keys = reinterpret_cast<unsigned*>(out_min_max);
    hipLaunchKernelGGL(minmax_init_kernel, dim3(1), dim3(1), 0, st, keys);
    hipLaunchKernelGGL(minmax_kernel, dim3(ew_grid(n) < 2048 ? ew_grid(n) : 2048), dim3(NT), 0, st, x, n, keys);
    hipLaunchKernelGGL(minmax_finish_kernel, dim3(1), dim3(1), 0, st, keys);
    IVIT_CHECK_LAUNCH("ivit_minmax_f32");
}

IVIT_EXPORT int ivit_quantize_input_f32_i8(const float* x, int8_t* out, int64_t n, float inv_scale,
                                           ivit_stream_t stream)
{
    IVIT_REQUIRE(x && out && n > 0, "ivit_quantize_input_f32_i8: bad operand");
    IVIT_REQUIRE(((uintptr_t)x % 16 == 0) && ((uintptr_t)out % 4 == 0), "ivit_quantize_input_f32_i8: misaligned");
    hipLaunchKernelGGL(quantize_kernel, dim3(ew_grid(n / 4 + 1)), dim3(NT), 0, ivit_stream(stream), x, out, n,
                       inv_scale);
    IVIT_CHECK_LAUNCH("ivit_quantize_input_f32_i8");
}

IVIT_EXPORT int ivit_quantize_input_f32_i32(const float* x, int32_t* out, int64_t n, float inv_scale, int bits,
                                            ivit_stream_t stream)
{
    IVIT_REQUIRE(x && out && n > 0 && bits >= 2 && bits <= 32, "ivit_quantize_input_f32_i32: bad operand");
    const float lo = -__builtin_ldexpf(1.0f, bits - 1), hi = __builtin_ldexpf(1.0f, bits - 1) - 1.0f;
    hipLaunchKernelGGL(quantize_i32_kernel, dim3(ew_grid(n)), dim3(NT), 0, ivit_stream(stream), x, out, n, inv_scale, lo, hi);
    IVIT_CHECK_LAUNCH("ivit_quantize_input_f32_i32");
}

static int launch_patchify(const char* who, const float* img, int8_t* A, int64_t lda, int batch, int chans, int hw, int patch,
                           float inv_scale, ivit_stream_t stream)
{
    IVIT_REQUIRE(img && A && batch > 0 && chans > 0, "%s: bad operand", who);
    IVIT_REQUIRE(patch > 0 && patch % 4 == 0 && hw % patch == 0, "%s: hw=%d patch=%d", who, hw, patch);
    IVIT_REQUIRE(lda >= (int64_t)chans * patch * patch && lda % 4 == 0, "%s: lda=%lld too small or not a multiple of 4", who,
                 (long long)lda);
    IVIT_REQUIRE(((uintptr_t)img % 16 == 0) && ((uintptr_t)A % 4 == 0), "%s: misaligned", who);
    const int64_t total = (int64_t)batch * chans * hw * (hw / 4);
    hipLaunchKernelGGL(patchify_kernel, dim3(ew_grid(total)), dim3(NT), 0, ivit_stream(stream), img, A, lda, batch, chans,
                       hw, patch, inv_scale);
    IVIT_CHECK_LAUNCH(who);
}

IVIT_EXPORT int ivit_quantize_patchify_f32_i8(const float* img, int8_t* A, int batch, int chans, int hw, int patch,
                                              float inv_scale, ivit_stream_t stream)
{
    return launch_patchify("ivit_quantize_patchify_f32_i8", img, A, (int64_t)chans * patch * patch, batch, chans, hw, patch,
                           inv_scale, stream);
}

IVIT_EXPORT int ivit_quantize_patchify_u8_i8(const uint8_t* img, int8_t* A, int64_t lda, int batch, int chans, int hw, int patch,
                                             const int8_t* lut, ivit_stream_t stream)
{
    IVIT_REQUIRE(img && A && lut && batch > 0 && chans > 0 && chans <= 4 && hw > 0 && patch > 0 && hw % patch == 0 && patch % 4 == 0,
                 "ivit_quantize_patchify_u8_i8: bad shape (up to 4 channels, hw %% patch == 0, patch %% 4 == 0)");
    IVIT_REQUIRE(lda >= (int64_t)chans * patch * patch && lda % 4 == 0 && ((uintptr_t)img % 4 == 0) && ((uintptr_t)A % 4 == 0),
                 "ivit_quantize_patchify_u8_i8: lda too small or misaligned operand");
    const int64_t total = (int64_t)batch * chans * hw * (hw / 4);
    hipLaunchKernelGGL(patchify_u8_kernel, dim3(ew_grid(total)), dim3(NT), 0, ivit_stream(stream), img, A, lda, batch, chans, hw,
                       patch, lut);
    IVIT_CHECK_LAUNCH("ivit_quantize_patchify_u8_i8");
}

IVIT_EXPORT int ivit_quantize_patchify_ld_f32_i8(const float* img, int8_t* A, int64_t lda, int batch, int chans, int hw,
                                                 int patch, float inv_scale, ivit_stream_t stream)
{
    return launch_patchify("ivit_quantize_patchify_ld_f32_i8", img, A, lda, batch, chans, hw, patch, inv_scale, stream);
}

template <typename TP>
static int launch_patchify_hw(const char* who, const TP* img, int8_t* A, int64_t lda, int batch, int chans, int h, int w, int patch,
                              float inv_scale, const int8_t* lut, ivit_stream_t stream)
{
    constexpr bool U8 = sizeof(TP) == 1;
    IVIT_REQUIRE(img && A && (lut || !U8), "%s: NULL operand", who);
    IVIT_REQUIRE(batch > 0 && chans > 0 && (!U8 || chans <= 4), "%s: batch=%d chans=%d (at least 1%s)", who, batch, chans,
                 U8 ? ", at most 4 channels" : "");
    IVIT_REQUIRE(patch > 0 && patch % 4 == 0 && h > 0 && w > 0 && h % patch == 0 && w % patch == 0,
                 "%s: h=%d w=%d patch=%d (h %% patch == 0, w %% patch == 0, patch %% 4 == 0)", who, h, w, patch);
    IVIT_REQUIRE(lda >= (int64_t)chans * patch * patch && lda % 4 == 0, "%s: lda=%lld too small or not a multiple of 4", who,
                 (long long)lda);
    IVIT_REQUIRE(((uintptr_t)img % (4 * sizeof(TP)) == 0) && ((uintptr_t)A % 4 == 0), "%s: misaligned", who);
    const int64_t total = (int64_t)batch * chans * h * (w / 4);
    hipLaunchKernelGGL(patchify_hw_kernel<TP>, dim3(ew_grid(total)), dim3(NT), 0, ivit_stream(stream), img, A, lda, batch, chans, h,
                       w, patch, inv_scale, lut);
    IVIT_CHECK_LAUNCH(who);
}

IVIT_EXPORT int ivit_quantize_patchify_hw_f32_i8(const float* img, int8_t* A, int64_t lda, int batch, int chans, int h, int w,
                                                 int patch, float inv_scale, ivit_stream_t stream)
{
    return launch_patchify_hw<float>("ivit_quantize_patchify_hw_f32_i8", img, A, lda, batch, chans, h, w, patch, inv_scale, nullptr,
                                     stream);
}

IVIT_EXPORT int ivit_quantize_patchify_hw_u8_i8(const uint8_t* img, int8_t* A, int64_t lda, int batch, int chans, int h, int w,
                                                int patch, const int8_t* lut, ivit_stream_t stream)
{
    return launch_patchify_hw<uint8_t>("ivit_quantize_patchify_hw_u8_i8", img, A, lda, batch, chans, h, w, patch, 0.0f, lut, stream);
}

namespace {
int launch_embed_i8(const char* name, const int8_t* patch, const int16_t* pos_add, const int8_t* cls_row, uint32_t m, int32_t e,
                    int8_t* out, int batch, int tokens, int C, int bits, ivit_stream_t stream)
{
    IVIT_REQUIRE(bits == 4 || bits == 8, "%s: bits=%d must be 4 or 8", name, bits);
    IVIT_REQUIRE(patch && pos_add && cls_row && out, "%s: NULL operand", name);
    IVIT_REQUIRE(batch > 0 && tokens > 1 && C > 0 && C % 4 == 0, "%s: bad shape", name);
    IVIT_REQUIRE(((uintptr_t)patch % 4 == 0) && ((uintptr_t)out % 4 == 0) && ((uintptr_t)cls_row % 4 == 0) &&
                     ((uintptr_t)pos_add % 8 == 0),
                 "%s: misaligned", name);
    const double Mq = ivit_dyadic_to_double(m, e);
    IVIT_REQUIRE(Mq < 1048576.0, "%s: requant multiplier too large", name);
    const int64_t total = (int64_t)batch * tokens * (C / 4);
    if (bits == 8)
        hipLaunchKernelGGL((embed_kernel<-128, 127>), dim3(ew_grid(total)), dim3(NT), 0, ivit_stream(stream), patch, pos_add, cls_row,
                           Mq, out, batch, tokens, C);
    else
        hipLaunchKernelGGL((embed_kernel<-8, 7>), dim3(ew_grid(total)), dim3(NT), 0, ivit_stream(stream), patch, pos_add, cls_row,
                           Mq, out, batch, tokens, C);
    IVIT_CHECK_LAUNCH(name);
}
}

IVIT_EXPORT int ivit_embed_assemble_i8(const int8_t* patch, const int16_t* pos_add, const int8_t* cls_row, uint32_t m,
                                       int32_t e, int8_t* out, int batch, int tokens, int C, ivit_stream_t stream)
{
    return launch_embed_i8("ivit_embed_assemble_i8", patch, pos_add, cls_row, m, e, out, batch, tokens, C, 8, stream);
}

IVIT_EXPORT int ivit_embed_assemble_i8_bits(const int8_t* patch, const int16_t* pos_add, const int8_t* cls_row, uint32_t m,
                                            int32_t e, int8_t* out, int batch, int tokens, int C, int bits, ivit_stream_t stream)
{
    return launch_embed_i8("ivit_embed_assemble_i8_bits", patch, pos_add, cls_row, m, e, out, batch, tokens, C, bits, stream);
}

IVIT_EXPORT int ivit_embed_assemble_i16(const int16_t* patch, const int32_t* pos_add, const int16_t* cls_row, uint32_t m,
                                        int32_t e, int16_t* out, int batch, int tokens, int C, ivit_stream_t stream)
{
    IVIT_REQUIRE(patch && pos_add && cls_row && out, "ivit_embed_assemble_i16: NULL operand");
    IVIT_REQUIRE(batch > 0 && tokens > 1 && C > 0 && C % 4 == 0, "ivit_embed_assemble_i16: bad shape");
    IVIT_REQUIRE(((uintptr_t)patch % 8 == 0) && ((uintptr_t)out % 8 == 0) && ((uintptr_t)cls_row % 8 == 0) &&
                     ((uintptr_t)pos_add % 16 == 0),
                 "ivit_embed_assemble_i16: misaligned");
    const double Mq = ivit_dyadic_to_double(m, e);
    IVIT_REQUIRE(Mq < 32768.0, "ivit_embed_assemble_i16: requant multiplier too large");
    const int64_t total = (int64_t)batch * tokens * (C / 4);
    hipLaunchKernelGGL(embed16_kernel, dim3(ew_grid(total)), dim3(NT), 0, ivit_stream(stream), patch, pos_add, cls_row,
                       Mq, out, batch, tokens, C);
    IVIT_CHECK_LAUNCH("ivit_embed_assemble_i16");
}

IVIT_EXPORT int ivit_head_argmax(const int32_t* acc, const float* s_acc, int batch, int N, float* logits_f32,
// ... 154 lines not shown
```

i-vit_amd/engine.py:

```python
from __future__ import annotations

import os

import numpy as np
import torch

from . import _lib, gemm_forms
from .engine_common import (EngineBase, _np, attention, attention_probs, attention_spec, block_copy, frag_copy, intermediate_indices,
                            layernorm, layernorm_f32, ln_spec, token_format, tokens_to_nchw)
from .prepare import dyadic, dyadic1, f32, pad_head, quant_sym, requant_host
from .topk import TOPK_MAX


class IntViTEngine(EngineBase):
    frags16 = os.environ.get("IVIT_FRAGS16", "1") != "0"
    LONG_TOKENS = 1025

    def __init__(self, float_state=None, ranges=None, embed_dim: int = 768, depth: int = 12, num_heads: int = 12,
                 device="cuda:0", max_batch: int = 256, source=None, family: str = "ivit", stream_bits: int = 8,
                 softmax_bits: int = 8, pos_bits: int = 8, img_size=224, patch_size: int = 16, int_sqrt: bool = False):
        self.C, self.D, self.H = embed_dim, depth, num_heads
        ih, iw = (int(v) for v in img_size) if isinstance(img_size, (tuple, list)) else (int(img_size),) * 2
        self.IMG_H, self.IMG_W, self.P = ih, iw, int(patch_size)
        self.IMG = ih if ih == iw else (ih, iw)
        tokens = (ih // self.P) * (iw // self.P) + 1 if self.P > 0 else 0
        if self.P <= 0 or ih % self.P or iw % self.P or (3 * self.P * self.P) % 64 or tokens > self.LONG_TOKENS:
            raise ValueError(f"geometry {self.IMG} / {self.P}: needs height and width % patch_size == 0, 3 * patch_size^2 % 64 == 0 and "
                             f"at most {self.LONG_TOKENS} tokens")
        self.grid = (ih // self.P, iw // self.P)
        self.NP = self.grid[0] * self.grid[1]
        self.T = self.NP + 1
        if family not in ("ivit", "ibert"):
            raise ValueError(f"operator family {family!r}: the fused engine implements 'ivit' and 'ibert'")
        self.family = family
        if int_sqrt and family != "ibert":
            raise ValueError("int_sqrt (use_int_sqrt) is a parameter of the 'ibert' LayerNorm")
        self.int_sqrt = bool(int_sqrt)
        if stream_bits not in (4, 8, 16):
            raise ValueError("stream_bits must be 4, 8 or 16")
        if self.T > 207 and (family != "ivit" or stream_bits == 16):
            raise ValueError(f"geometry {self.IMG} / {self.P}: {self.T} tokens; the I-BERT softmax and the 16-bit stream take at most "
                             "207 tokens (more: family 'ivit' with stream_bits = 8 or 4)")
        self.stream_bits = sb = stream_bits
        other = {8: (8,), 16: (8, 16), 4: (4, 8)}[sb]
        if softmax_bits not in other or pos_bits not in other:
            raise ValueError("softmax_bits / pos_bits: 8, or 16 together with stream_bits = 16, or 4 together with stream_bits = 4")
        self.softmax_bits, self.pos_bits = softmax_bits, pos_bits
        self.hd = embed_dim // num_heads
        if self.hd != 64:
            raise ValueError("fused attention kernel supports head_dim 64 only")
        self.dev = torch.device(device)
        self.max_batch = max_batch
        _lib.lib()
        if source is None:
            from .export import FloatSource
            source = FloatSource({k: _np(v) for k, v in float_state.items()}, ranges)
        C, H, hd = self.C, self.H, self.hd
        T = self.T
        s = source.act_scale

        dev = self._upload

        def lin_dev(lp, s_out):
            m, e = lp.requant_to(s_out)
            return dict(W=dev(lp.W8), b=dev(lp.b32), m=dev(m.view(np.int32)), e=dev(e), K=lp.K, N=lp.W8.shape[0])

        def ln_shift(prefix):
            if family != "ibert":
                return None
            try:
                return float(np.asarray(source.tensor(prefix + ".shift")).reshape(-1)[0])
            except KeyError:
                return 0.0

        def ln_dev(prefix, s_out, s_in):
            return self._ln_spec(source.layernorm(prefix, s_out), s_in, 16 if sb == 16 else 8, ln_shift(prefix), self.int_sqrt)

        def ranges_of(name):
            if ranges is None or name not in ranges:
                raise KeyError(f"the 'ibert' engine needs the range of {name} (the softmax's internal 16-bit QuantAct)")
            return float(ranges[name][0]), float(ranges[name][1])

        self.natural_sites = 0
        s0 = s("qact_input")
        self.inv_s0 = float(f32(1.0) / s0)
        self.s0 = float(s0)
        self.input_lut = None
        pe = source.linear("patch_embed.proj", s0)
        s_pe = s("patch_embed.qact", sb)
        self.patch = lin_dev(pe, s_pe)
        s_pos, s_x = s("qact_pos", pos_bits), s("qact1", sb)
        m1, e1 = dyadic(s_pe, s_x)
        m2, e2 = dyadic(s_pos, s_x)
        kpos = quant_sym(source.tensor("pos_embed").reshape(T, C), s_pos, pos_bits)
        pos_add = requant_host(kpos, m2[0], e2[0])
        z_cls = np.rint((source.tensor("cls_token").reshape(C) / s_pe).astype(f32))
        qlim = 2 ** (sb - 1)
        cls_row = np.clip(requant_host(z_cls, m1[0], e1[0]) + pos_add[0], -qlim, qlim - 1)
        if sb == 16:
            assert np.abs(pos_add).max() < 2 ** 31
            self.pos_add = dev(pos_add.astype(np.int32))
            self.cls_row = dev(cls_row.astype(np.int16))
        else:
            assert np.abs(pos_add).max() < 32768
            self.pos_add = dev(pos_add.astype(np.int16))
            self.cls_row = dev(cls_row.astype(np.int8))
        self.embed_me = (int(m1[0]), int(e1[0]))

        self.blocks = []
        for i in range(depth):
            p = f"blocks.{i}."
            blk = {}
            s_q1 = s(p + "qact1")
            blk["ln1"] = ln_dev(p + "norm1", s_q1, s_x)
            s_a1 = s(p + "attn.qact1")
            blk["qkv"] = lin_dev(source.linear(p + "attn.qkv", s_q1), s_a1)
            s_S = f32(f32(s_a1 * s_a1) * f32(hd ** -0.5))
            s_at = s(p + "attn.qact_attn1")
            s_pv = f32(f32(1.0 / 2 ** (softmax_bits - 1)) * s_a1)
            s_a2 = s(p + "attn.qact2")
            blk["attn"] = a = attention_spec(family, s_S, s_at, s_pv, s_a2, dev, self.dev, self._stream(),
                                             ranges_of(p + "attn.int_softmax.act") if family == "ibert" else None)
            self.natural_sites += int(family == "ivit" and (a["band"] is not None or a["exp2d"] is not None))
            s_a3 = s(p + "attn.qact3", sb)
            blk["proj"] = lin_dev(source.linear(p + "attn.proj", s_a2), s_a3)
            s_b2 = s(p + "qact2", sb)
            blk["res1"] = dyadic1(s_a3, s_b2) + dyadic1(s_x, s_b2)
            s_b3 = s(p + "qact3")
            blk["ln2"] = ln_dev(p + "norm2", s_b3, s_b2)
            s_g = s(p + "mlp.qact_gelu")
            blk["fc1"] = lin_dev(source.linear(p + "mlp.fc1", s_b3), s_g)
            s_m1 = s(p + "mlp.qact1")
            blk["gelu_lut"] = self._gelu_lut(family, s_g, s_m1)
            s_m2 = s(p + "mlp.qact2", sb)
            blk["fc2"] = lin_dev(source.linear(p + "mlp.fc2", s_m1), s_m2)
            s_b4 = s(p + "qact4", sb)
            blk["res2"] = dyadic1(s_m2, s_b4) + dyadic1(s_b2, s_b4)
            s_x = s_b4
            blk["s_out"] = float(s_b4)
            self.blocks.append(blk)

        s_q2 = s("qact2")
        self.ln_f = ln_dev("norm", s_q2, s_x)
        self._norm_lp = source.layernorm("norm", s_q2)
        self._norm_shift = ln_shift("norm")
        self._ln_tok = {depth - 1: self.ln_f}
        self.s_feat = float(s_q2)
        try:
            head = source.linear("head", s_q2)
        except KeyError:
            head = None
        if head is None:
            self.head, self.head_scale, self.num_classes = None, None, 0
        else:
            hW, hb, hs, self.num_classes = pad_head(head.W8, head.b32, head.s_acc)
            self.head = dict(W=dev(hW), b=dev(hb), K=head.K, N=hW.shape[0])
            self.head_scale = dev(hs)
        self.int8_weight_bytes = sum(int(b[k]["W"].numel()) for b in self.blocks for k in ("qkv", "proj", "fc1", "fc2")) \
            + int(self.patch["W"].numel()) + (0 if self.head is None else int(self.head["W"].numel()))
        lins = [self.patch] + [b[k] for b in self.blocks for k in ("qkv", "proj", "fc1", "fc2")]
        for lin in lins:
            lin["Wb"] = block_copy(lin["W"], self._stream())
        wide = {id(b[k]) for b in self.blocks for k in ("proj", "fc2")} if self.stream_bits == 16 else set()
        for lin in lins:
            narrow = id(lin) not in wide
            lin["Wf"], lin["Wf_bit"] = frag_copy(lin["W"], self._stream(), order16=self.frags16 and narrow, narrow=narrow)
        for b in self.blocks:
            b["q"] = dict(b["qkv"], N=C)
        self.weight_frags = True
        self.block_operands = True
        self.block_a = {"ln": True, "attn": True, "gelu": True}
        self.gelu_in_place = True
        self.fuse_res16 = True
        self.fuse_ibert_gelu = True
        self.probe = None
        self._alloc(max_batch)
        self._compact(True)
        torch.cuda.synchronize(self.dev)

    def _alloc(self, B):
        C, T = self.C, self.T
        M = B * T
        M16 = (M + 15) // 16 * 16
        i8 = dict(dtype=torch.int8, device=self.dev)
        self.ws = dict(
            a0=torch.empty(B * self.NP, 3 * self.P * self.P, **i8),
            pe=torch.empty(B * self.NP, C, **i8),
            x=torch.empty(M, C, **i8), x2=torch.empty(M, C, **i8), h=torch.empty(M16, C, **i8),
            qkv=torch.empty(3 * M * C, **i8), ao=torch.empty(M16, C, **i8),
            f1=torch.empty(M16, 4 * C, **i8), g=torch.empty(M16, 4 * C, **i8), untile=torch.empty(M, 4 * C, **i8),
            cls=torch.empty(B, C, **i8),
            c_h=torch.empty(B, C, **i8), c_q=torch.empty(B, C, **i8), c_ao=torch.empty(B, C, **i8), c_x=torch.empty(B, C, **i8),
            c_y=torch.empty(B, C, **i8), c_f1=torch.empty(B, 4 * C, **i8),
            **({} if self.stream_bits == 8 else dict(
                pe16=torch.empty(B * self.NP, C, dtype=torch.int16, device=self.dev),
                x16=torch.empty(M, C, dtype=torch.int16, device=self.dev), y16=torch.empty(M, C, dtype=torch.int16, device=self.dev),
                k16=torch.empty(M, C, dtype=torch.int16, device=self.dev),
                cls16=torch.empty(B, C, dtype=torch.int16, device=self.dev))),
            **({} if self.head is None else dict(
                logits=torch.empty(B, self.head["N"], dtype=torch.int32, device=self.dev),
                logits_f=torch.empty(B, self.head["N"], dtype=torch.float32, device=self.dev))),
            top1=torch.empty(B, dtype=torch.int32, device=self.dev),
            topk=torch.empty(B * TOPK_MAX, dtype=torch.int32, device=self.dev),
        )

    def _w(self, lin, epi, M, blocks, row0=0):
        W, bit = gemm_forms.weight(lin, epi, M, frags=blocks and self.weight_frags, blocks=blocks)
        assert row0 % 64 == 0
        return _lib.ptr(W.view(-1)[row0 * lin["K"]:] if row0 else W), bit

    def _compact(self, on=True):
        ws = self.ws
        if "_own" not in ws:
            ws["_own"] = {k: ws[k] for k in ("x2", "ao", "qkv")}
        if on:
            ws["x2"] = ws["x"]
            ws["ao"] = ws["h"]
            ws["qkv"] = ws["f1"].view(-1)[: ws["_own"]["qkv"].numel()]
        else:
            ws.update(ws["_own"])

    def _gemm(self, A, lda, lin, out, ldo, M, st, a_blocks=False, blocks=False, out_blocks=False, bits=8):
        w, lay = self._w(lin, gemm_forms.RQ, M, blocks)
        lay |= (gemm_forms.A_BLOCKS if a_blocks else 0) | (gemm_forms.OUT_BLOCKS if out_blocks else 0)
        if bits == 8:
            _lib.call("ivit_gemm_i8_requant_ex", _lib.ptr(A), lda, w, lin["K"], _lib.ptr(lin["b"]),
                      _lib.ptr(lin["m"]), _lib.ptr(lin["e"]), _lib.ptr(out), ldo, M, lin["N"], lin["K"], lay, st)
        else:
            _lib.call("ivit_gemm_i8_requant_bits_ex", _lib.ptr(A), lda, w, lin["K"], _lib.ptr(lin["b"]),
                      _lib.ptr(lin["m"]), _lib.ptr(lin["e"]), _lib.ptr(out), ldo, M, lin["N"], lin["K"], lay, bits, st)

    def _gemm_res(self, A, lda, lin, res, me4, out, M, st, blocks=False, a_blocks=False, ldr=None):
        C, r = self.C, me4
        ldr = C if ldr is None else ldr
        if self.stream_bits == 16 and not self.fuse_res16:
            k16 = self.ws["k16"]
            _lib.call("ivit_gemm_i8_requant_i16", _lib.ptr(A), lda, _lib.ptr(lin["W"]), lin["K"], _lib.ptr(lin["b"]),
                      _lib.ptr(lin["m"]), _lib.ptr(lin["e"]), _lib.ptr(k16), C, M, C, lin["K"], st)
            _lib.call("ivit_residual_requant_i16", _lib.ptr(k16), 16, None, None, r[0], r[1], _lib.ptr(res), r[2], r[3],
                      _lib.ptr(out), M, C, 0, 0, 0, 0, st)
            return
        probe = self.probe
        if probe is not None:
            probe.begin("gemm_resid", st)
        w, lay = self._w(lin, gemm_forms.RESID if self.stream_bits != 16 else gemm_forms.RQ16_RES16, M, blocks)
        lay |= gemm_forms.A_BLOCKS if a_blocks else 0
        if self.stream_bits == 8:
            _lib.call("ivit_gemm_i8_requant_residual_ex", _lib.ptr(A), lda, w, lin["K"],
                      _lib.ptr(lin["b"]), _lib.ptr(lin["m"]), _lib.ptr(lin["e"]), _lib.ptr(res), ldr,
                      r[0], r[1], r[2], r[3], _lib.ptr(out), C, M, lin["N"], lin["K"], lay, st)
        elif self.stream_bits == 4:
            _lib.call("ivit_gemm_i8_requant_residual_bits_ex", _lib.ptr(A), lda, w, lin["K"],
                      _lib.ptr(lin["b"]), _lib.ptr(lin["m"]), _lib.ptr(lin["e"]), _lib.ptr(res), ldr,
                      r[0], r[1], r[2], r[3], _lib.ptr(out), C, M, lin["N"], lin["K"], lay, 4, 4, st)
        else:
            _lib.call("ivit_gemm_i8_requant_i16_residual_i16_ex", _lib.ptr(A), lda, w,
                      lin["K"], _lib.ptr(lin["b"]), _lib.ptr(lin["m"]), _lib.ptr(lin["e"]), _lib.ptr(res), C, r[0], r[1], r[2], r[3],
                      _lib.ptr(out), C, M, C, lin["K"], lay, st)
        if probe is not None:
            probe.end("gemm_resid", st, (M, lin["N"], lin["K"]))

    def _patchify(self, images, B, st):
        ws = self.ws
        if images.dtype == torch.uint8 and self.input_lut is None:
            self.set_input_normalisation()
        if self.IMG_H != self.IMG_W:
            if images.dtype == torch.uint8:
                _lib.call("ivit_quantize_patchify_hw_u8_i8", _lib.ptr(images), _lib.ptr(ws["a0"]), 3 * self.P * self.P, B, 3, self.IMG_H,
                          self.IMG_W, self.P, _lib.ptr(self.input_lut), st)
            else:
                _lib.call("ivit_quantize_patchify_hw_f32_i8", _lib.ptr(images), _lib.ptr(ws["a0"]), 3 * self.P * self.P, B, 3, self.IMG_H,
                          self.IMG_W, self.P, self.inv_s0, st)
        elif images.dtype == torch.uint8:
            _lib.call("ivit_quantize_patchify_u8_i8", _lib.ptr(images), _lib.ptr(ws["a0"]), 3 * self.P * self.P, B, 3, self.IMG, self.P,
                      _lib.ptr(self.input_lut), st)
        else:
            _lib.call("ivit_quantize_patchify_f32_i8", _lib.ptr(images), _lib.ptr(ws["a0"]), B, 3, self.IMG, self.P, self.inv_s0, st)

    def forward(self, images: torch.Tensor, taps: dict | None = None, cls_tail: bool = False):
        return self._forward(images, taps, cls_tail=cls_tail)

    @property
    def cls_tail_ok(self):
        return self.family == "ivit" and self.stream_bits == 8 and self.T <= 207

    def _graph_forward(self, images):
        return self._forward(images, cls_tail=self.cls_tail_ok)

    def _graph_forward_topk(self, images, k, targets, hits):
        return self._forward(images, None, (k, targets, hits), cls_tail=self.cls_tail_ok)

    def _cls_block(self, blk, x, B, st, a_ln, blk_l):
        C, H, hd, T = self.C, self.H, self.hd, self.T
        M, ws, q = B * T, self.ws, blk["qkv"]
        layernorm(blk["ln1"], x, C, M, C, ws["h"], C, st, blocks=a_ln)
        kvw, kvlay = self._w(q, gemm_forms.QKV, M, blk_l, row0=C)
        _lib.call("ivit_gemm_i8_requant_qkv_planes_ex", _lib.ptr(ws["h"]), C, kvw, q["K"], _lib.ptr(q["b"][C:]),
                  _lib.ptr(q["m"][C:]), _lib.ptr(q["e"][C:]), _lib.ptr(ws["qkv"]), T, H, hd, 1, 2, M, 2 * C, C, kvlay | (gemm_forms.A_BLOCKS if a_ln else 0), st)
        layernorm(blk["ln1"], x, T * C, B, C, ws["c_h"], C, st, blocks=False)
        self._gemm(ws["c_h"], C, blk["q"], ws["c_q"], C, B, st)
        a = blk["attn"]
        _lib.call("ivit_attention_cls_i8", _lib.ptr(ws["qkv"][M * C:]), _lib.ptr(ws["qkv"][2 * M * C:]), _lib.ptr(ws["c_q"]),
                  _lib.ptr(ws["c_ao"]), C, B, H, T, hd, a["ms"][0], a["ms"][1], a["s_attn"], a["mo"][0], a["mo"][1],
                  _lib.ptr(a["exp2d"]), _lib.ptr(a["band"]), a["band_w"], st)
        self._gemm_res(ws["c_ao"], C, blk["proj"], x, blk["res1"], ws["c_x"], B, st, ldr=T * C)
        layernorm(blk["ln2"], ws["c_x"], C, B, C, ws["c_h"], C, st, blocks=False)
        self._gemm(ws["c_h"], C, blk["fc1"], ws["c_f1"], 4 * C, B, st)
        _lib.call("ivit_shiftgelu_lut_i8_ex", _lib.ptr(ws["c_f1"]), 4 * C, B, 4 * C, _lib.ptr(blk["gelu_lut"]),
                  _lib.ptr(ws["c_f1"]), 4 * C, 0, st)
        self._gemm_res(ws["c_f1"], 4 * C, blk["fc2"], ws["c_x"], blk["res2"], ws["c_y"], B, st)
        return ws["c_y"]

    def attention_maps(self, images: torch.Tensor, layers=None, rows: str = "cls"):
        if self.softmax_bits != 8:
            raise ValueError(f"attention_maps: the softmax output is {self.softmax_bits} bits wide (the probability kernel writes 8-bit "
                             "probabilities only)")
        if rows not in ("cls", "all"):
            raise ValueError(f"rows={rows!r}: 'cls' (the class token's row) or 'all' (the full map)")
        layers = range(self.D) if layers is None else [int(i) for i in layers]
        if any(not 0 <= i < self.D for i in layers):
            raise ValueError(f"layers {list(layers)}: block indices in 0..{self.D - 1}")
        B, R = images.shape[0], 1 if rows == "cls" else self.T
        maps = {i: torch.empty(B, self.H, R, self.T, dtype=torch.uint8, device=self.dev) for i in layers}
        self._forward(images, maps=maps, stop="features" if self.head is None else None)
        return maps, 2.0 ** -7

    def forward_features(self, images: torch.Tensor, integers: bool = False, out: torch.Tensor | None = None):
        B = images.shape[0]
        out = self._features_out(B, self.C, integers, out)
        self._forward(images, cls_tail=self.cls_tail_ok, stop="features")
        return self._features_emit(self.ws["cls"], B, self.C, self.s_feat, out), self.s_feat

    def _graph_features(self, images, integers):
        return self.forward_features(images, integers)

    def forward_intermediates_early(self, images: torch.Tensor, indices=None, integers: bool = False):
        return self._intermediates(images, indices, integers, True)

    def forward_intermediates(self, images: torch.Tensor, indices=None, integers: bool = False):
        return self._intermediates(images, indices, integers, self.head is None)

    def _intermediates(self, images, indices, integers, stop_early):
        idx = intermediate_indices(indices, self.D, "block")
        B = images.shape[0]
        dt = torch.float32 if not integers else torch.int16 if self.stream_bits == 16 else torch.int8
        feats = {i: torch.empty(B, self.C, *self.grid, dtype=dt, device=self.dev) for i in idx}
        self._forward(images, feats=feats, stop=max(idx) if stop_early else None)
        return feats, {i: self.blocks[i]["s_out"] for i in idx}

    def _ln_tokens(self, i):
        if i not in self._ln_tok:
            self._ln_tok[i] = ln_spec(self._norm_lp, self._upload, self.blocks[i]["s_out"], 16 if self.stream_bits == 16 else 8,
                                      self._norm_shift, self.int_sqrt)
        return self._ln_tok[i]

    def forward_tokens(self, images: torch.Tensor, indices=None, fmt: str = "NLC", prefix: bool = True, integers: bool = False):
        token_format(fmt)
        idx = [self.D - 1] if indices is None else intermediate_indices(indices, self.D, "block")
        if integers and idx != [self.D - 1]:
            raise ValueError(f"integers=True: qact2 belongs to the last block's norm; indices must be ({self.D - 1},) or None, not {idx}")
        B, C, T, NP = images.shape[0], self.C, self.T, self.NP
        tokens, prefixes = {}, {}

        def emit(i, x, st):
            if integers:
                q = torch.empty(B * T, C, dtype=torch.int8, device=self.dev)
                layernorm(self.ln_f, x, C, B * T, C, q, C, st, blocks=False)
                q = q.view(B, T, C)
                if prefix:
                    prefixes[i] = q[:, :1]
                if fmt == "NLC":
                    tokens[i] = q[:, 1:]
                else:
                    tokens[i] = torch.empty(B, C, *self.grid, dtype=torch.int8, device=self.dev)
                    tokens_to_nchw(q, C, B, T, 1, NP, C, 1.0, tokens[i], st)
                return
            ln = self._ln_tokens(i)
            if fmt == "NLC":
                t0 = 0 if prefix else 1
                full = torch.empty(B, T - t0, C, dtype=torch.float32, device=self.dev)
                layernorm_f32(ln, x, C, B, T, t0, T - t0, C, full, C, st)
                tokens[i] = full[:, 1 - t0:]
                if prefix:
                    prefixes[i] = full[:, :1]
                return
            tokens[i] = torch.empty(B, C, *self.grid, dtype=torch.float32, device=self.dev)
            layernorm_f32(ln, x, C, B, T, 1, NP, C, tokens[i], NP, st, fmt="NCHW")
            if prefix:
                prefixes[i] = torch.empty(B, 1, C, dtype=torch.float32, device=self.dev)
                layernorm_f32(ln, x, C, B, T, 0, 1, C, prefixes[i], C, st)

        self._forward(images, toks={i: emit for i in idx}, stop=max(idx) if self.head is None else None)
        return {i: tokens[i] for i in idx}, {i: prefixes[i] for i in idx if prefix}, (self.s_feat if integers else self.ln_f["s"])

    def _forward(self, images: torch.Tensor, taps: dict | None = None, topk=None, cls_tail: bool = False, maps: dict | None = None,
                 feats: dict | None = None, stop=None, toks: dict | None = None):
        assert images.is_cuda and images.dtype in (torch.float32, torch.uint8) and images.is_contiguous()
        B = images.shape[0]
        assert images.shape[1:] == (3, self.IMG_H, self.IMG_W) and 0 < B <= self.max_batch
        if stop is None:
            self._require_head("forward")
        wide = self.stream_bits == 16
        if wide and taps is not None:
            raise NotImplementedError("taps are not recorded on the 16-bit-stream path")
        if cls_tail and (taps is not None or not self.cls_tail_ok):
            raise ValueError("cls_tail: I-ViT operators, 8-bit stream, at most 207 tokens, no taps (ivit_attention_cls_i8 has no width)")
        C, H, hd, T = self.C, self.H, self.hd, self.T
        M = B * T
        ws = self.ws
        st = self._stream()

        blk_l = bool(self.block_operands) and gemm_forms.block_operands_apply(M, C, C)
        a_ln, a_at, a_ge = (blk_l and not wide and self.block_a[k] for k in ("ln", "attn", "gelu"))

        def tap(name, t, shape, blocks=False):
            if taps is not None:
                if blocks:
                    rows, K = int(np.prod(shape[:-1])), shape[-1]
                    _lib.call("ivit_untile_operand_i8", _lib.ptr(t), rows, K, _lib.ptr(ws["untile"]), K, st)
                    t = ws["untile"]
                taps[name] = t.reshape(-1)[: int(np.prod(shape))].view(shape).clone()

        self._patchify(images, B, st)
        if wide:
            pt = self.patch
            _lib.call("ivit_gemm_i8_requant_i16", _lib.ptr(ws["a0"]), 3 * self.P * self.P, _lib.ptr(pt["W"]), pt["K"], _lib.ptr(pt["b"]),
                      _lib.ptr(pt["m"]), _lib.ptr(pt["e"]), _lib.ptr(ws["pe16"]), C, B * self.NP, C, pt["K"], st)
            x, x2 = ws["x16"], (ws["x16"] if self.fuse_res16 else ws["y16"])
        else:
            self._gemm(ws["a0"], 3 * self.P * self.P, self.patch, ws["pe"], C, B * self.NP, st,
                       blocks=bool(self.block_operands), bits=self.stream_bits)
            tap("patch_embed.qact", ws["pe"], (B, self.NP, C))
            x, x2 = ws["x"], ws["x2"]
        if self.stream_bits == 4:
            _lib.call("ivit_embed_assemble_i8_bits", _lib.ptr(ws["pe"]), _lib.ptr(self.pos_add), _lib.ptr(self.cls_row), self.embed_me[0],
                      self.embed_me[1], _lib.ptr(x), B, T, C, 4, st)
        else:
            _lib.call("ivit_embed_assemble_i16" if wide else "ivit_embed_assemble_i8", _lib.ptr(ws["pe16" if wide else "pe"]),
                      _lib.ptr(self.pos_add), _lib.ptr(self.cls_row), self.embed_me[0], self.embed_me[1], _lib.ptr(x), B, T, C, st)
        tap("qact1", x, (B, T, C))
        y_cls = None
        for i, blk in enumerate(self.blocks):
            p = f"blocks.{i}."
            if cls_tail and i == self.D - 1:
                y_cls = self._cls_block(blk, x, B, st, a_ln, blk_l)
                break
            layernorm(blk["ln1"], x, C, M, C, ws["h"], C, st, blocks=a_ln)
            tap(p + "qact1", ws["h"], (B, T, C), a_ln)
            q = blk["qkv"]
            qw, qlay = self._w(q, gemm_forms.QKV, M, blk_l)
            _lib.call("ivit_gemm_i8_requant_qkv_ex", _lib.ptr(ws["h"]), C, qw, q["K"], _lib.ptr(q["b"]),
                      _lib.ptr(q["m"]), _lib.ptr(q["e"]), _lib.ptr(ws["qkv"]), T, H, hd, M, 3 * C, C, qlay | (gemm_forms.A_BLOCKS if a_ln else 0), st)
            tap(p + "attn.qkv_headmajor", ws["qkv"], (3, B, H, T, hd))
            if maps is not None and i in maps:
                attention_probs(blk["attn"], self.family, ws["qkv"], maps[i], B, H, T, hd, maps[i].shape[2], st)
            attention(blk["attn"], self.family, ws["qkv"], ws["ao"], B, H, T, hd, st, blocks=a_at,
                      softmax_bits=self.softmax_bits if self.stream_bits != 8 else None)
            tap(p + "attn.qact2", ws["ao"], (B, T, C), a_at)
            self._gemm_res(ws["ao"], C, blk["proj"], x, blk["res1"], x2, M, st, blocks=blk_l, a_blocks=a_at)
            tap(p + "qact2", x2, (B, T, C))
            layernorm(blk["ln2"], x2, C, M, C, ws["h"], C, st, blocks=a_ln)
            tap(p + "qact3", ws["h"], (B, T, C), a_ln)
            f1 = blk["fc1"]
            f1w, f1lay = self._w(f1, gemm_forms.RQ, M, blk_l) if self.family == "ibert" and self.fuse_ibert_gelu and taps is None else (None, 0)
            if f1lay & gemm_forms.FRAGS:
                g_buf = ws["f1"]
                _lib.call("ivit_gemm_i8_requant_lut_ex", _lib.ptr(ws["h"]), C, f1w, f1["K"], _lib.ptr(f1["b"]),
                          _lib.ptr(f1["m"]), _lib.ptr(f1["e"]), _lib.ptr(blk["gelu_lut"]), _lib.ptr(g_buf), 4 * C, M, f1["N"], f1["K"],
                          f1lay | (gemm_forms.A_BLOCKS if a_ln else 0) | (gemm_forms.OUT_BLOCKS if a_ge else 0), st)
            else:
                self._gemm(ws["h"], C, f1, ws["f1"], 4 * C, M, st, a_blocks=a_ln, blocks=blk_l, out_blocks=a_ge)
                tap(p + "mlp.qact_gelu", ws["f1"], (B, T, 4 * C), a_ge)
                g_buf = ws["f1"] if self.gelu_in_place or wide else ws["g"]
                _lib.call("ivit_shiftgelu_lut_i8_ex", _lib.ptr(ws["f1"]), 4 * C, M, 4 * C, _lib.ptr(blk["gelu_lut"]),
                          _lib.ptr(g_buf), 4 * C, 3 if a_ge else 0, st)
            tap(p + "mlp.qact1", g_buf, (B, T, 4 * C), a_ge)
            self._gemm_res(g_buf, 4 * C, blk["fc2"], x2, blk["res2"], x, M, st, blocks=blk_l, a_blocks=a_ge)
            tap(p + "qact4", x, (B, T, C))
            if feats is not None and i in feats:
                tokens_to_nchw(x, C, B, T, 1, T - 1, C, blk["s_out"], feats[i], st)
            if toks is not None and i in toks:
                toks[i](i, x, st)
            if stop == i:
                return None
        if wide:
            ws["cls16"][:B].copy_(x.view(-1, T, C)[:B, 0])
            layernorm(self.ln_f, ws["cls16"], C, B, C, ws["cls"], C, st, blocks=False)
        elif y_cls is not None:
            layernorm(self.ln_f, y_cls, C, B, C, ws["cls"], C, st, blocks=False)
        else:
            layernorm(self.ln_f, x, T * C, B, C, ws["cls"], C, st, blocks=False)
        tap("qact2", ws["cls"], (B, C))
        if stop == "features":
            return None
        hd_ = self.head
        _lib.call("ivit_gemm_i8_i32", _lib.ptr(ws["cls"]), C, _lib.ptr(hd_["W"]), hd_["K"], _lib.ptr(hd_["b"]),
                  _lib.ptr(ws["logits"]), hd_["N"], B, hd_["N"], C, st)
        return self._classify(B, st, topk)

    __call__ = forward
```

i-vit_amd/gemm_forms.py:

```python
from __future__ import annotations

A_BLOCKS, W_BLOCKS, OUT_BLOCKS, W_FRAGS, W_FRAGS16 = 1, 2, 4, 8, 16
FRAGS = W_FRAGS | W_FRAGS16
RQ, RESID, QKV, I32, RESID16, RQ16, RQ16_RES16 = range(7)
SMALL, PERS, WREG, WREG16, SKINNY = range(5)
LAYOUTS = {RQ: A_BLOCKS | W_BLOCKS | OUT_BLOCKS | FRAGS, RESID: A_BLOCKS | W_BLOCKS | FRAGS, QKV: A_BLOCKS | W_BLOCKS | FRAGS, I32: 0,
           RESID16: A_BLOCKS | W_BLOCKS | FRAGS, RQ16: 0, RQ16_RES16: A_BLOCKS | W_FRAGS}

BIG_MIN_M, BIG_MIN_N = 2048, 128
SK_MIN_M, SK_MAXK, SK_MAXN = 8192, 128, 320
WR_CH, WR_WASTE_DEN = 256, 8

_INT8_OUT = (RQ, RESID, QKV)
_NO_TILE_LOOP = (I32, RQ16)


def skinny_applies(epi: int, M: int, N: int, K: int) -> bool:
    return (epi in (RQ, QKV) and M >= SK_MIN_M and 32 <= K <= SK_MAXK and K % 32 == 0 and 16 <= N <= SK_MAXN and N % 16 == 0
            and M * N < 1 << 32)


def pers_applies(epi: int, M: int, N: int) -> bool:
    return epi not in _NO_TILE_LOOP and epi != RQ16_RES16 and M >= BIG_MIN_M and N >= BIG_MIN_N


def frags_shape(N: int, K: int) -> bool:
    return N >= BIG_MIN_N and N % 64 == 0 and K % 192 == 0


def frags_apply(epi: int, M: int, N: int, K: int, bit: int = W_FRAGS16) -> bool:
    return (epi not in _NO_TILE_LOOP and (bit == W_FRAGS or epi != RQ16_RES16) and M >= BIG_MIN_M and frags_shape(N, K)
            and (bit == W_FRAGS or (M + 16) * N < 1 << 32))


def tiles_fit(N: int) -> bool:
    return -(-N // WR_CH) * WR_CH * WR_WASTE_DEN <= N * (WR_WASTE_DEN + 1)


def frag_items_ok(bit: int, narrow: bool, N: int) -> bool:
    return (bit == W_FRAGS16 and narrow) or tiles_fit(N)


def blocks_shape(N: int, K: int) -> bool:
    return N >= BIG_MIN_N and N % 16 == 0 and K % 64 == 0


def block_operands_apply(M: int, N: int, K: int) -> bool:
    return M >= BIG_MIN_M and blocks_shape(N, K)


def form(epi: int, M: int, N: int, K: int, layouts: int = 0):
    int8_acc = epi not in (I32, RQ16, RQ16_RES16)
    if min(M, N, K) <= 0 or K % 64 or N % (16 if int8_acc else 8 if epi == RQ16_RES16 else 4):
        return None
    if layouts & ~LAYOUTS[epi] or layouts & FRAGS == FRAGS or (epi == RQ16_RES16 and layouts & A_BLOCKS and not layouts & FRAGS):
        return None
    if layouts & OUT_BLOCKS and (N % 64 or (M + 15) * N >= 1 << 31):
        return None
    if epi == QKV and M * N >= 1 << 31:
        return None
    if not layouts and skinny_applies(epi, M, N, K):
        return SKINNY
    if layouts & (A_BLOCKS | W_BLOCKS) and not layouts & FRAGS and not pers_applies(epi, M, N):
        return None
    if layouts & FRAGS:
        bit = layouts & FRAGS
        if layouts & W_BLOCKS or not frags_apply(epi, M, N, K, bit):
            return None
        return WREG if bit == W_FRAGS else WREG16
    return PERS if pers_applies(epi, M, N) else SMALL


def weight(lin: dict, epi: int, M: int, frags: bool = True, blocks: bool = True):
    N, K = lin["N"], lin["K"]
    if frags:
        for W, bit in ((lin.get("Wf"), lin.get("Wf_bit")), (lin.get("Wf32"), W_FRAGS)):
            if W is not None and frags_apply(epi, M, N, K, bit) and frag_items_ok(bit, epi in _INT8_OUT, N):
                return W, bit
    if blocks and lin.get("Wb") is not None and not skinny_applies(epi, M, N, K) and pers_applies(epi, M, N):
        return lin["Wb"], W_BLOCKS
    return lin["W"], 0
```

include/ivit_hip.h:

```cpp
#ifndef IVIT_HIP_H
#define IVIT_HIP_H

#include <stdint.h>

#ifdef __cplusplus
extern "C" {
#endif

#define IVIT_OK 0
#define IVIT_ERR_INVALID (-1)
#define IVIT_ERR_UNSUPPORTED (-2)
#define IVIT_ERR_LAUNCH (-3)

typedef void* ivit_stream_t;

int ivit_version(void);
const char* ivit_last_error_string(void);

int ivit_minmax_f32(const float* x, int64_t n, float* out_min_max, ivit_stream_t stream);

#define IVIT_QUANTILE_WS_BYTES 16640
int ivit_quantile_pair_f32(const float* x, int64_t n, float q_lo, float q_hi, float* out2, void* workspace, int64_t workspace_bytes,
                           ivit_stream_t stream);

int ivit_weight_quant_rows_f32_i8(const float* w, int64_t ldw, int rows, int cols, float* scale, int8_t* w8, int64_t ldo, float* w_int,
                                  ivit_stream_t stream);

int ivit_bias_quant_f32_i32(const float* bias, const float* scale, int n, float s_in, float* s_acc, int32_t* b32, float* b_int,
                            ivit_stream_t stream);

int ivit_quantize_input_f32_i8(const float* x, int8_t* out, int64_t n, float inv_scale, ivit_stream_t stream);
int ivit_quantize_input_f32_i32(const float* x, int32_t* out, int64_t n, float inv_scale, int bits, ivit_stream_t stream);

int ivit_quantize_patchify_f32_i8(const float* img, int8_t* A, int batch, int chans, int hw, int patch,
                                  float inv_scale, ivit_stream_t stream);
int ivit_quantize_patchify_ld_f32_i8(const float* img, int8_t* A, int64_t lda, int batch, int chans, int hw, int patch,
                                     float inv_scale, ivit_stream_t stream);
int ivit_quantize_patchify_u8_i8(const uint8_t* img, int8_t* A, int64_t lda, int batch, int chans, int hw, int patch,
                                 const int8_t* lut, ivit_stream_t stream);
int ivit_quantize_patchify_hw_f32_i8(const float* img, int8_t* A, int64_t lda, int batch, int chans, int h, int w, int patch,
                                     float inv_scale, ivit_stream_t stream);
int ivit_quantize_patchify_hw_u8_i8(const uint8_t* img, int8_t* A, int64_t lda, int batch, int chans, int h, int w, int patch,
                                    const int8_t* lut, ivit_stream_t stream);


#define IVIT_A_BLOCKS 1
#define IVIT_W_BLOCKS 2
#define IVIT_OUT_BLOCKS 4
#define IVIT_W_FRAGS 8
int ivit_pack_weight_frags_i8(const int8_t* W, int64_t ldw, int N, int K, int8_t* dst, ivit_stream_t stream);
#define IVIT_W_FRAGS16 16
int ivit_pack_weight_frags16_i8(const int8_t* W, int64_t ldw, int N, int K, int8_t* dst, ivit_stream_t stream);
int ivit_tile_operand_i8(const int8_t* src, int64_t ld, int64_t rows, int K, int8_t* dst, ivit_stream_t stream);
int ivit_untile_operand_i8(const int8_t* src, int64_t rows, int K, int8_t* dst, int64_t ld, ivit_stream_t stream);

int ivit_gemm_i8_requant(const int8_t* A, int64_t lda, const int8_t* W, int64_t ldw, const int32_t* bias,
                         const uint32_t* m, const int32_t* e, int8_t* out, int64_t ldo,
                         int M, int N, int K, ivit_stream_t stream);

int ivit_gemm_i8_requant_ex(const int8_t* A, int64_t lda, const int8_t* W, int64_t ldw, const int32_t* bias,
                            const uint32_t* m, const int32_t* e, int8_t* out, int64_t ldo,
                            int M, int N, int K, int layouts, ivit_stream_t stream);

int ivit_gemm_i8_requant_bits_ex(const int8_t* A, int64_t lda, const int8_t* W, int64_t ldw, const int32_t* bias,
                                 const uint32_t* m, const int32_t* e, int8_t* out, int64_t ldo,
                                 int M, int N, int K, int layouts, int bits, ivit_stream_t stream);

int ivit_gemm_i8_requant_lut_ex(const int8_t* A, int64_t lda, const int8_t* W, int64_t ldw, const int32_t* bias,
                                const uint32_t* m, const int32_t* e, const int8_t* lut, int8_t* out, int64_t ldo,
                                int M, int N, int K, int layouts, ivit_stream_t stream);

int ivit_gemm_i8_requant_residual(const int8_t* A, int64_t lda, const int8_t* W, int64_t ldw,
                                  const int32_t* bias, const uint32_t* m, const int32_t* e,
                                  const int8_t* res, int64_t ldr, uint32_t m_main, int32_t e_main,
                                  uint32_t m_res, int32_t e_res, int8_t* out, int64_t ldo,
                                  int M, int N, int K, ivit_stream_t stream);

int ivit_gemm_i8_requant_residual_ex(const int8_t* A, int64_t lda, const int8_t* W, int64_t ldw,
                                     const int32_t* bias, const uint32_t* m, const int32_t* e,
                                     const int8_t* res, int64_t ldr, uint32_t m_main, int32_t e_main,
                                     uint32_t m_res, int32_t e_res, int8_t* out, int64_t ldo,
                                     int M, int N, int K, int layouts, ivit_stream_t stream);

int ivit_gemm_i8_requant_residual_bits_ex(const int8_t* A, int64_t lda, const int8_t* W, int64_t ldw,
                                          const int32_t* bias, const uint32_t* m, const int32_t* e,
                                          const int8_t* res, int64_t ldr, uint32_t m_main, int32_t e_main,
                                          uint32_t m_res, int32_t e_res, int8_t* out, int64_t ldo,
                                          int M, int N, int K, int layouts, int bits_mid, int bits_out, ivit_stream_t stream);

int ivit_gemm_i8_requant_residual_i16(const int8_t* A, int64_t lda, const int8_t* W, int64_t ldw,
                                      const int32_t* bias, const uint32_t* m, const int32_t* e,
                                      const int16_t* res, int64_t ldr, uint32_t m_main, int32_t e_main,
                                      uint32_t m_res, int32_t e_res, int16_t* out, int64_t ldo,
                                      int M, int N, int K, ivit_stream_t stream);
int ivit_gemm_i8_requant_residual_i16_ex(const int8_t* A, int64_t lda, const int8_t* W, int64_t ldw,
                                         const int32_t* bias, const uint32_t* m, const int32_t* e,
                                         const int16_t* res, int64_t ldr, uint32_t m_main, int32_t e_main,
                                         uint32_t m_res, int32_t e_res, int16_t* out, int64_t ldo,
                                         int M, int N, int K, int layouts, ivit_stream_t stream);

int ivit_gemm_i8_requant_qkv(const int8_t* A, int64_t lda, const int8_t* W, int64_t ldw, const int32_t* bias,
                             const uint32_t* m, const int32_t* e, int8_t* qkv, int tokens, int heads,
                             int head_dim, int M, int N, int K, ivit_stream_t stream);
int ivit_gemm_i8_requant_qkv_ex(const int8_t* A, int64_t lda, const int8_t* W, int64_t ldw, const int32_t* bias,
                                const uint32_t* m, const int32_t* e, int8_t* qkv, int tokens, int heads,
                                int head_dim, int M, int N, int K, int layouts, ivit_stream_t stream);
int ivit_gemm_i8_requant_qkv_planes_ex(const int8_t* A, int64_t lda, const int8_t* W, int64_t ldw, const int32_t* bias,
                                       const uint32_t* m, const int32_t* e, int8_t* qkv, int tokens, int heads,
                                       int head_dim, int plane0, int nplanes, int M, int N, int K, int layouts,
                                       ivit_stream_t stream);

int ivit_gemm_i8_requant_i16(const int8_t* A, int64_t lda, const int8_t* W, int64_t ldw, const int32_t* bias,
                             const uint32_t* m, const int32_t* e, int16_t* out, int64_t ldo, int M, int N, int K,
                             ivit_stream_t stream);

int ivit_gemm_i8_requant_i16_residual_i16_ex(const int8_t* A, int64_t lda, const int8_t* W, int64_t ldw, const int32_t* bias,
                                             const uint32_t* m, const int32_t* e, const int16_t* res, int64_t ldr,
                                             uint32_t m_main, int32_t e_main, uint32_t m_res, int32_t e_res, int16_t* out,
                                             int64_t ldo, int M, int N, int K, int layouts, ivit_stream_t stream);

int ivit_gemm_i8_i32(const int8_t* A, int64_t lda, const int8_t* W, int64_t ldw, const int32_t* bias,
                     int32_t* out, int64_t ldo, int M, int N, int K, ivit_stream_t stream);

#define IVIT_GEMM_EPI_RQ 0
#define IVIT_GEMM_EPI_RESID 1
#define IVIT_GEMM_EPI_QKV 2
#define IVIT_GEMM_EPI_I32 3
#define IVIT_GEMM_EPI_RESID16 4
#define IVIT_GEMM_EPI_RQ16 5
#define IVIT_GEMM_EPI_RQ16_RES16 6
#define IVIT_GEMM_FORM_SMALL 0
#define IVIT_GEMM_FORM_PERS 1
#define IVIT_GEMM_FORM_WREG 2
#define IVIT_GEMM_FORM_WREG16 3
#define IVIT_GEMM_FORM_SKINNY 4
int ivit_gemm_plan(int epilogue, int M, int N, int K, int layouts, int32_t* out8);

int ivit_attention_fused_i8(const int8_t* qkv, int8_t* out, int batch, int heads, int tokens, int head_dim,
                            uint32_t m_s, int32_t e_s, float s_attn, uint32_t m_o, int32_t e_o,
                            ivit_stream_t stream);
int ivit_attention_fused_i8_ex(const int8_t* qkv, int8_t* out, int batch, int heads, int tokens, int head_dim,
                               uint32_t m_s, int32_t e_s, float s_attn, uint32_t m_o, int32_t e_o, int out_blocks,
                               ivit_stream_t stream);

int ivit_attention_fused_i8_compat(const int8_t* qkv, int8_t* out, int batch, int heads, int tokens, int head_dim,
                                   uint32_t m_s, int32_t e_s, float s_attn, uint32_t m_o, int32_t e_o,
                                   const uint32_t* exp2d, int out_blocks, ivit_stream_t stream);

int ivit_attention_fused_i8_compat_band(const int8_t* qkv, int8_t* out, int batch, int heads, int tokens, int head_dim,
                                        uint32_t m_s, int32_t e_s, float s_attn, uint32_t m_o, int32_t e_o,
                                        const uint32_t* exp2d, const uint32_t* band, int band_w, int out_blocks,
                                        ivit_stream_t stream);
int ivit_attention_fused_i8_wide(const int8_t* qkv, int8_t* out, int batch, int heads, int tokens, int head_dim, uint32_t m_s,
                                 int32_t e_s, float s_attn, uint32_t m_o, int32_t e_o, const uint32_t* exp2d,
                                 const uint32_t* band, int band_w, int softmax_bits, int out_blocks, ivit_stream_t stream);

int ivit_attention_fused_i8_long(const int8_t* qkv, int8_t* out, int batch, int heads, int tokens, int head_dim, uint32_t m_s,
                                 int32_t e_s, float s_attn, uint32_t m_o, int32_t e_o, const uint32_t* exp2d,
                                 const uint32_t* band, int band_w, int out_blocks, ivit_stream_t stream);

int ivit_attention_fused_i8_wide_long(const int8_t* qkv, int8_t* out, int batch, int heads, int tokens, int head_dim,
                                      uint32_t m_s, int32_t e_s, float s_attn, uint32_t m_o, int32_t e_o, const uint32_t* exp2d,
                                      const uint32_t* band, int band_w, int softmax_bits, int out_blocks, ivit_stream_t stream);

int ivit_attention_cls_i8(const int8_t* k, const int8_t* v, const int8_t* q, int8_t* out, int64_t ldo, int batch, int heads,
                          int tokens, int head_dim, uint32_t m_s, int32_t e_s, float s_attn, uint32_t m_o, int32_t e_o,
                          const uint32_t* exp2d, const uint32_t* band, int band_w, ivit_stream_t stream);

int ivit_layernorm_i8(const int8_t* x, int64_t ldx, int rows, int C, const float* bias_int, const float* s_ln,
                      const uint32_t* m, const int32_t* e, int8_t* out, int64_t ldo, ivit_stream_t stream);
int ivit_layernorm_i8_ex(const int8_t* x, int64_t ldx, int rows, int C, const float* bias_int, const float* s_ln,
                         const uint32_t* m, const int32_t* e, int8_t* out, int64_t ldo, int out_blocks,
                         ivit_stream_t stream);

int ivit_layernorm_i8_compat(const int8_t* x, int64_t ldx, int rows, int C, const float* bias_int, const float* s_ln,
                             const uint32_t* m, const int32_t* e, const int8_t* remap ,
                             const float* phi , int8_t* out, int64_t ldo, int flags,
                             ivit_stream_t stream);
#define IVIT_LN_OUT_BLOCKS 1
#define IVIT_LN_OUTER_MEAN(L) ((L) << 8)

int ivit_layernorm_i32_f32(const int32_t* x, int64_t ldx, int rows, int C, const float* bias_int,
                           const float* s_ln, float* out, int64_t ldo, ivit_stream_t stream);

#define IVIT_LN_F32_CHANNEL_MAJOR 1
#define IVIT_LN_F32_FAST_DIV 2
int ivit_layernorm_i8_f32(const int8_t* x, int64_t ldx, int B, int T_all, int t0, int T, int C, const float* bias_int,
                          const float* s_ln, const int8_t* remap , const float* phi ,
                          float* out, int64_t ldo, int flags, ivit_stream_t stream);
int ivit_layernorm_i16_f32(const int16_t* x, int64_t ldx, int B, int T_all, int t0, int T, int C, float s_in, const float* bias_int,
                           const float* s_ln, float* out, int64_t ldo, int flags, ivit_stream_t stream);

int ivit_layernorm_f32_f32(const float* x, int64_t ldx, int rows, int C, const float* s_in, int n_s,
                           const float* bias_int, const float* s_ln, float* out, int64_t ldo, ivit_stream_t stream);
int ivit_layernorm_f32_f32_ex(const float* x, int64_t ldx, int rows, int C, const float* s_in, int n_s,
                              const float* bias_int, const float* s_ln, float* out, int64_t ldo, int outer_mean,
                              ivit_stream_t stream);

int ivit_shiftgelu_i8(const int8_t* x, int64_t ldx, int rows, int L, float s, uint32_t m, int32_t e,
                      int8_t* out, int64_t ldo, ivit_stream_t stream);
int ivit_shiftgelu_i8_i32(const int8_t* x, int64_t ldx, int rows, int L, float s, int32_t* out, int64_t ldo,
                          ivit_stream_t stream);
int ivit_shiftgelu_build_lut(float s, uint32_t m, int32_t e, int8_t* lut , ivit_stream_t stream);
int ivit_shiftgelu_build_lut_ex(float s, uint32_t m, int32_t e, const int8_t* remap, int8_t* lut ,
                                ivit_stream_t stream);
int ivit_shiftgelu_lut_i8(const int8_t* x, int64_t ldx, int rows, int L, const int8_t* lut, int8_t* out,
                          int64_t ldo, ivit_stream_t stream);
int ivit_shiftgelu_lut_i8_ex(const int8_t* x, int64_t ldx, int rows, int L, const int8_t* lut, int8_t* out,
                             int64_t ldo, int layouts, ivit_stream_t stream);

int ivit_shiftmax_i8(const int8_t* x, int64_t ldx, int rows, int L, float s, int8_t* out, int64_t ldo,
                     ivit_stream_t stream);
int ivit_shiftmax_f32_i8(const float* x, int64_t ldx, int rows, int L, float s, int8_t* out, int64_t ldo,
                         ivit_stream_t stream);
int ivit_shiftmax_f32_i16(const float* x, int64_t ldx, int rows, int L, float s, int output_bit, int16_t* out, int64_t ldo,
                          ivit_stream_t stream);
int ivit_shiftmax_i32_i8(const int32_t* x, int64_t ldx, int rows, int L, float s, int8_t* out, int64_t ldo,
                         ivit_stream_t stream);

int ivit_requant_i32(const int32_t* z, int64_t rows, int C, const uint32_t* m, const int32_t* e, int n_me,
                     const int32_t* z2, const uint32_t* m2, const int32_t* e2, int n_me2, int bits,
                     int32_t* out, ivit_stream_t stream);

int ivit_residual_requant_i8(const int8_t* a, uint32_t m_a, int32_t e_a, const int8_t* b, uint32_t m_b,
                             int32_t e_b, int8_t* out, int64_t n, ivit_stream_t stream);
int ivit_residual_requant_i8_bits(const int8_t* a, uint32_t m_a, int32_t e_a, const int8_t* b, uint32_t m_b,
                                  int32_t e_b, int8_t* out, int64_t n, int bits, ivit_stream_t stream);

int ivit_embed_assemble_i8(const int8_t* patch, const int16_t* pos_add, const int8_t* cls_row, uint32_t m,
                           int32_t e, int8_t* out, int batch, int tokens, int C, ivit_stream_t stream);
int ivit_embed_assemble_i8_bits(const int8_t* patch, const int16_t* pos_add, const int8_t* cls_row, uint32_t m,
                                int32_t e, int8_t* out, int batch, int tokens, int C, int bits, ivit_stream_t stream);

int ivit_embed_assemble_i16(const int16_t* patch, const int32_t* pos_add, const int16_t* cls_row, uint32_t m,
                            int32_t e, int16_t* out, int batch, int tokens, int C, ivit_stream_t stream);

int ivit_head_argmax(const int32_t* acc, const float* s_acc, int batch, int N, float* logits_f32,
                     int32_t* top1, ivit_stream_t stream);

#define IVIT_TOPK_MAX 8
int ivit_head_topk(const int32_t* acc, const float* s_acc, int batch, int ld, int N, int k, float* logits_f32,
                   int32_t* topk, const int32_t* targets, uint64_t* hits, ivit_stream_t stream);
int ivit_logits_topk_f32(const float* logits, int batch, int ld, int N, int k, int32_t* topk, const int32_t* targets,
                         uint64_t* hits, ivit_stream_t stream);

int ivit_bgemm_qk_i8(const int8_t* Q, const int8_t* K, int32_t* S, int batch, int Tq, int Tk, int D,
                     ivit_stream_t stream);
int ivit_bgemm_pv_i8(const int8_t* P, const int8_t* V, int32_t* O, int batch, int Tq, int Tk, int D,
                     ivit_stream_t stream);
int ivit_bgemm_pv_i16_i8(const int16_t* P, const int8_t* V, int32_t* O, int batch, int Tq, int Tk, int D,
                         ivit_stream_t stream);
int ivit_bgemm_pv_i32_i8(const int32_t* P, const int8_t* V, int32_t* O, int batch, int Tq, int Tk, int D, int64_t p_absmax,
                         ivit_stream_t stream);

int ivit_f32_to_i32(const float* x, int64_t rows, int C, const float* s, int n_s, int mode, int32_t* z,
                    ivit_stream_t stream);
int ivit_i32_to_f32(const int32_t* z, int64_t rows, int C, const float* s, int n_s, float* y,
                    ivit_stream_t stream);

int ivit_narrow_i32_i8(const int32_t* z, int8_t* out, int64_t n, int32_t* overflow_flag, ivit_stream_t stream);


int ivit_requant_i8_i16(const int8_t* x, uint32_t m, int32_t e, int16_t* out, int64_t n, ivit_stream_t stream);

int ivit_residual_requant_i16(const void* a, int a_bits, const uint32_t* m_pre, const int32_t* e_pre, uint32_t m_a,
                              int32_t e_a, const int16_t* res, uint32_t m_r, int32_t e_r, int16_t* out, int64_t rows,
                              int C, int H, int W, int ws, int shift, ivit_stream_t stream);

int ivit_layernorm_i16_i8(const int16_t* x, int rows, int C, const float* bias_int, const float* s_ln,
                          const uint32_t* m, const int32_t* e, int8_t* out, int64_t ldo, int H, int W, int ws, int shift,
                          ivit_stream_t stream);
int ivit_layernorm_i16_i8_compat(const int16_t* x, int rows, int C, float s_in, int fast_division, const float* bias_int,
                                 const float* s_ln, const uint32_t* m, const int32_t* e, int8_t* out, int64_t ldo, int H, int W,
                                 int ws, int shift, ivit_stream_t stream);

int ivit_patch_merge_i16(const int16_t* x, int16_t* out, int batch, int H, int W, int C, ivit_stream_t stream);

int ivit_window_rows(const void* src, void* dst, int batch, int H, int W, int64_t row_bytes, int ws, int shift, int inverse,
                     ivit_stream_t stream);

int ivit_avgpool_requant_i8(const int8_t* x, int8_t* out, int batch, int tokens, int C, uint32_t m, int32_t e,
                            ivit_stream_t stream);
int ivit_avgpool_requant_i8_literal(const int8_t* x, int8_t* out, int batch, int tokens, int C, float s_in, uint32_t m, int32_t e,
                                    ivit_stream_t stream);
int ivit_avgpool_f32_literal(const float* x, float* out, int batch, int tokens, int C, ivit_stream_t stream);

int ivit_window_attention_i8(const int8_t* qkv, int8_t* out, int64_t ldo, const int16_t* bias_add,
                             const uint8_t* mask_region, int mask_value, int windows, int windows_per_image, int heads,
                             int tokens, int head_dim, uint32_t m_s, int32_t e_s, uint32_t m_b, int32_t e_b,
                             float s_attn, uint32_t m_o, int32_t e_o, ivit_stream_t stream);
int ivit_window_attention_i8_compat(const int8_t* qkv, int8_t* out, int64_t ldo, const int16_t* bias_add,
                                    const uint8_t* mask_region, int mask_value, int windows, int windows_per_image, int heads,
                                    int tokens, int head_dim, uint32_t m_s, int32_t e_s, uint32_t m_b, int32_t e_b,
                                    float s_attn, uint32_t m_o, int32_t e_o, const float* phi, const float* phi_masked,
                                    ivit_stream_t stream);
int ivit_window_attention_i8_band(const int8_t* qkv, int8_t* out, int64_t ldo, const int16_t* bias_add, const uint8_t* mask_region,
                                  int windows, int windows_per_image, int heads, int tokens, int head_dim, uint32_t m_s, int32_t e_s,
                                  uint32_t m_b, int32_t e_b, float s_attn, uint32_t m_o, int32_t e_o, const uint32_t* band,
                                  int band_w, int band_rows, int H, int W, int ws, int shift, ivit_stream_t stream);
int ivit_window_attention_i8_unwindow(const int8_t* qkv, int8_t* out, int64_t ldo, const int16_t* bias_add,
                                      const uint8_t* mask_region, int mask_value, int windows, int windows_per_image, int heads,
                                      int tokens, int head_dim, uint32_t m_s, int32_t e_s, uint32_t m_b, int32_t e_b,
                                      float s_attn, uint32_t m_o, int32_t e_o, const float* phi, const float* phi_masked,
                                      int H, int W, int ws, int shift, ivit_stream_t stream);
int ivit_window_attention_i8_long(const int8_t* qkv, int8_t* out, int64_t ldo, const int16_t* bias_add, const uint8_t* mask_region,
                                  int mask_value, int windows, int windows_per_image, int heads, int tokens, int head_dim, uint32_t m_s,
                                  int32_t e_s, uint32_t m_b, int32_t e_b, float s_attn, uint32_t m_o, int32_t e_o, const float* phi,
                                  const float* phi_masked, const uint32_t* band, int band_w, int band_rows, int H, int W, int ws,
                                  int shift, int image_order, ivit_stream_t stream);
int ivit_window_attention_i8_ibert(const int8_t* qkv, int8_t* out, int64_t ldo, const int16_t* bias_add, const uint8_t* mask_region,
                                   float masked_exp, int windows, int windows_per_image, int heads, int tokens, int head_dim,
                                   uint32_t m_s, int32_t e_s, uint32_t m_b, int32_t e_b, uint32_t m_o, int32_t e_o, const float* table,
                                   int band_w, int H, int W, int ws, int shift, int image_order, ivit_stream_t stream);
int ivit_window_attention_probs_u8(const int8_t* qkv, uint8_t* probs, int64_t ldp, const int16_t* bias, const uint8_t* region,
                                   int mask_value, int nwin, int windows_per_image, int heads, int tokens, int head_dim,
// ... 120 lines not shown
```

Before: 45440 images/s.

## Fuse patch-embed GEMM with positional add and class-token assembly

```diff
diff --git a/i-vit_amd/_lib.py b/i-vit_amd/_lib.py
--- a/i-vit_amd/_lib.py
+++ b/i-vit_amd/_lib.py
@@ -70,6 +70,9 @@
     "ivit_embed_assemble_i8": [vp, vp, vp, u32, i32, vp, ci, ci, ci, vp],
     "ivit_embed_assemble_i8_bits": [vp, vp, vp, u32, i32, vp, ci, ci, ci, ci, vp],
     "ivit_embed_assemble_i16": [vp, vp, vp, u32, i32, vp, ci, ci, ci, vp],
+    "ivit_quantize_patchify_f32_i8_ex": [vp, vp, ci, ci, ci, ci, f32, ci, vp],
+    "ivit_quantize_patchify_u8_i8_ex": [vp, vp, ci, ci, ci, ci, vp, ci, vp],
+    "ivit_gemm_i8_requant_embed_ex": [vp, i64, vp, i64, vp, vp, vp, vp, vp, u32, i32, u32, i32, vp, i64, ci, ci, ci, ci, ci, vp],
     "ivit_head_argmax": [vp, vp, ci, ci, vp, vp, vp],
     "ivit_head_topk": [vp, vp, ci, ci, ci, ci, vp, vp, vp, vp, vp],
     "ivit_logits_topk_f32": [vp, ci, ci, ci, ci, vp, vp, vp, vp],
diff --git a/i-vit_amd/csrc/gemm.hip b/i-vit_amd/csrc/gemm.hip
--- a/i-vit_amd/csrc/gemm.hip
+++ b/i-vit_amd/csrc/gemm.hip
@@ -759,7 +759,7 @@
             int tid_o = tid;
             asm volatile("" : "+v"(tid_o));
             if constexpr (S16) asm volatile("s_nop 15\n\ts_nop 15" ::: "memory");
-            if constexpr (S16 && (EPI == EPI_RQ || EPI == EPI_RESID || EPI == EPI_QKV)) {
+            if constexpr (S16 && (EPI == EPI_RQ || EPI == EPI_RESID || EPI == EPI_QKV || EPI == EPI_EMBED)) {
                 epilogue_direct_16<EPIW, 2 * TJ, (ABL & (2048 | 4096)), Hook>(acc16, g, tab, cur.m0 + wtok, cur.n0, wch, (tid_o >> 4) & 3, tid_o & 15, hook,
                                                                                g.lut ? reinterpret_cast<const unsigned char*>(smem + WR_LUT) : nullptr,
                                                                                (ABL & 2048) ? tv : nullptr);
@@ -800,7 +800,7 @@
                 stamp[16] = __builtin_amdgcn_s_memrealtime();
             }
         }
-        if constexpr (S16 && (EPI == EPI_RQ || EPI == EPI_RESID || EPI == EPI_QKV) && !(ABL & 16)) {
+        if constexpr (S16 && (EPI == EPI_RQ || EPI == EPI_RESID || EPI == EPI_QKV || EPI == EPI_EMBED) && !(ABL & 16)) {
             if (cur.half == 2) run(std::integral_constant<int, 2>{}, cur, nxt, tab, tab_next);
             else if (cur.half) run(std::integral_constant<int, 1>{}, cur, nxt, tab, tab_next);
             else run(std::integral_constant<int, 0>{}, cur, nxt, tab, tab_next);
@@ -944,16 +944,18 @@
 }
 
 constexpr bool epi_has_skinny(int epi) { return epi == EPI_RQ || epi == EPI_QKV; }
-constexpr bool epi_has_wreg(int epi) { return epi != EPI_I32 && epi != EPI_RQ16; }
-constexpr bool epi_has_wreg16(int epi) { return epi_has_wreg(epi) && epi != EPI_RQ16_RES16; }
+constexpr bool epi_has_small(int epi) { return epi != EPI_EMBED; }
+constexpr bool epi_has_wreg(int epi) { return epi != EPI_I32 && epi != EPI_RQ16 && epi != EPI_EMBED; }
+constexpr bool epi_has_wreg16(int epi) { return (epi_has_wreg(epi) && epi != EPI_RQ16_RES16) || epi == EPI_EMBED; }
 constexpr bool epi_has_pers(int epi) { return epi_has_wreg(epi) && epi != EPI_RQ16_RES16; }
-constexpr bool epi_int8_out(int epi) { return epi == EPI_RQ || epi == EPI_RESID || epi == EPI_QKV; }
+constexpr bool epi_int8_out(int epi) { return epi == EPI_RQ || epi == EPI_RESID || epi == EPI_QKV || epi == EPI_EMBED; }
 constexpr bool wr_tiles_fit(int N) { return (N + WR_CH - 1) / WR_CH * WR_CH * WR_WASTE_DEN <= N * (WR_WASTE_DEN + 1); }
 
 enum { GEMM_SMALL = IVIT_GEMM_FORM_SMALL, GEMM_PERS = IVIT_GEMM_FORM_PERS, GEMM_WREG = IVIT_GEMM_FORM_WREG, GEMM_WREG16 = IVIT_GEMM_FORM_WREG16,
        GEMM_SKINNY = IVIT_GEMM_FORM_SKINNY };
 static_assert(EPI_RQ == IVIT_GEMM_EPI_RQ && EPI_RESID == IVIT_GEMM_EPI_RESID && EPI_QKV == IVIT_GEMM_EPI_QKV && EPI_I32 == IVIT_GEMM_EPI_I32 &&
-              EPI_RESID16 == IVIT_GEMM_EPI_RESID16 && EPI_RQ16 == IVIT_GEMM_EPI_RQ16 && EPI_RQ16_RES16 == IVIT_GEMM_EPI_RQ16_RES16,
+              EPI_RESID16 == IVIT_GEMM_EPI_RESID16 && EPI_RQ16 == IVIT_GEMM_EPI_RQ16 && EPI_RQ16_RES16 == IVIT_GEMM_EPI_RQ16_RES16 &&
+              EPI_EMBED == IVIT_GEMM_EPI_EMBED,
               "include/ivit_hip.h names the epilogue kinds for ivit_gemm_plan");
 
 struct GemmPlan {
@@ -988,12 +990,17 @@
         IVIT_REQUIRE(((uintptr_t)g.m % 16 == 0) && ((uintptr_t)g.e % 16 == 0), "%s: m/e tables must be 16-byte aligned",
                      name);
     }
-    if (EPI == EPI_RQ || EPI == EPI_RESID)
+    if (EPI == EPI_RQ || EPI == EPI_RESID || EPI == EPI_EMBED)
         IVIT_REQUIRE(g.ldo >= g.N && g.ldo % 16 == 0, "%s: ldo=%lld must be >= N and a multiple of 16", name,
                      (long long)g.ldo);
-    if (EPI == EPI_RESID)
+    if (EPI == EPI_RESID || EPI == EPI_EMBED)
         IVIT_REQUIRE(g.res && g.ldr >= g.N && g.ldr % 16 == 0 && ((uintptr_t)g.res % 16 == 0),
                      "%s: residual operand missing or misaligned", name);
+    if (EPI == EPI_EMBED) {
+        IVIT_REQUIRE(g.cls_row && ((uintptr_t)g.cls_row % 16 == 0), "%s: class row missing or misaligned", name);
+        IVIT_REQUIRE(g.tokens >= 2 && g.M % (g.tokens - 1) == 0, "%s: M=%d is not a whole number of images of tokens - 1 = %d patches", name,
+                     g.M, g.tokens - 1);
+    }
     if (EPI == EPI_RESID16 || EPI == EPI_RQ16_RES16)
         IVIT_REQUIRE(g.res && g.ldr >= g.N && g.ldr % 8 == 0 && ((uintptr_t)g.res % 16 == 0) && g.ldo >= g.N && g.ldo % 8 == 0,
                      "%s: 16-bit residual / output rows must be 16-byte aligned (ld multiples of 8 elements)", name);
@@ -1014,6 +1021,7 @@
     const bool lab_forms = IVIT_LAB && EPIW == EPI;
     const bool blocks = g.a_blocks || g.w_blocks;
     p = GemmPlan{};
+    IVIT_REQUIRE(EPI != EPI_EMBED || g.w_frags == 2, "%s: the embedding epilogue exists for the IVIT_W_FRAGS16 form only", name);
     if (epi_has_skinny(EPI) && !blocks && !g.w_frags && !g.out_blocks && !g.lut && g.M >= SK_MIN_M && g.K >= 32 && g.K <= SK_MAXK &&
         g.K % 32 == 0 && g.N >= 16 && g.N <= SK_MAXN && g.N % 16 == 0 && g.lda % 16 == 0 && g.ldw % 8 == 0 && (EPI == EPI_QKV || g.ldo % 16 == 0) &&
         (EPI != EPI_QKV || g.head_dim % 16 == 0) && (int64_t)g.M * (EPI == EPI_QKV ? g.N : g.ldo) < 4294967296ll && !g_force_small &&
@@ -1035,7 +1043,7 @@
     if (g.w_frags) IVIT_REQUIRE(!g.a_blocks || g.lda == g.K, "%s: a block-layout A operand is dense (lda == K)", name);
     IVIT_REQUIRE(!g.lut || (g.w_frags && EPI == EPI_RQ), "%s: the output map needs the fragment-packed weight form (IVIT_W_FRAGS)", name);
     if (g.w_frags) {
-        IVIT_REQUIRE(epi_has_wreg(EPI) && big && g.N >= 128 && g.N % 64 == 0 && (g.K / BK) % 3 == 0 && !g.w_blocks,
+        IVIT_REQUIRE((epi_has_wreg(EPI) || epi_has_wreg16(EPI)) && big && g.N >= 128 && g.N % 64 == 0 && (g.K / BK) % 3 == 0 && !g.w_blocks,
                      "%s: the fragment-packed weight needs M >= 2048, N >= 128, N %% 64 == 0, K %% 192 == 0 and a requantising epilogue", name);
         p.tiles_m = (g.M + WR_TOK - 1) / WR_TOK;
         p.tiles_n = (g.N + WR_CH - 1) / WR_CH;
@@ -1069,7 +1077,7 @@
                      "%s: IVIT_W_FRAGS16 addresses its output (and residual) with 32-bit offsets: operand of 4 GiB or more", name);
         p.form = GEMM_WREG16;
         p.stamped = lab_forms && (EPI == EPI_RQ || EPI == EPI_RESID) && (g_debug_flags2 & LAB2_WR16_STAMPS) && g.stamp;
-        p.res_f32 = EPI == EPI_RESID && g.res_f32;
+        p.res_f32 = (EPI == EPI_RESID || EPI == EPI_EMBED) && g.res_f32;
         return IVIT_OK;
     }
     if (epi_has_pers(EPI) && big && g.N >= BCH) {
@@ -1138,7 +1146,7 @@
                     }
                 }
 #endif
-                if constexpr (EPI == EPI_RESID) {
+                if constexpr (EPI == EPI_RESID || EPI == EPI_EMBED) {
                     if (p.res_f32) {
                         IVIT_GEMM_LAUNCH((gemm_i8_wreg_kernel<EPIW, 4096, true>), BIG_NT);
                         break;
@@ -1166,8 +1174,11 @@
             }
             IVIT_GEMM_NO_KERNEL;
         case GEMM_SMALL:
-            IVIT_GEMM_LAUNCH(gemm_i8_kernel<EPIW>, NT);
-            break;
+            if constexpr (epi_has_small(EPI)) {
+                IVIT_GEMM_LAUNCH(gemm_i8_kernel<EPIW>, NT);
+                break;
+            }
+            IVIT_GEMM_NO_KERNEL;
         default:
             IVIT_GEMM_NO_KERNEL;
     }
@@ -1212,6 +1223,7 @@
 constexpr int LAYOUTS_RQ = IVIT_A_BLOCKS | IVIT_W_BLOCKS | IVIT_OUT_BLOCKS | IVIT_W_FRAGS | IVIT_W_FRAGS16;
 constexpr int LAYOUTS_IN = LAYOUTS_RQ & ~IVIT_OUT_BLOCKS;
 constexpr int LAYOUTS_RQ16_RES16 = IVIT_A_BLOCKS | IVIT_W_FRAGS;
+constexpr int LAYOUTS_EMBED = IVIT_A_BLOCKS | IVIT_W_FRAGS16;
 
 __global__ __launch_bounds__(256) void pack_weight_frags_kernel(const int8_t* W, int64_t ldw, int N, int K, int8_t* dst)
 {
@@ -1381,6 +1393,26 @@
     return ivit_gemm_i8_requant_residual_ex(A, lda, W, ldw, bias, m, e, res, ldr, m_main, e_main, m_res, e_res, out, ldo, M, N, K, 0, stream);
 }
 
+IVIT_EXPORT int ivit_gemm_i8_requant_embed_ex(const int8_t* A, int64_t lda, const int8_t* W, int64_t ldw, const int32_t* bias,
+                                              const uint32_t* m, const int32_t* e, const int8_t* kpos, const int8_t* cls_row,
+                                              uint32_t m1, int32_t e1, uint32_t m2, int32_t e2, int8_t* out, int64_t ldo, int M, int N,
+                                              int K, int tokens, int layouts, ivit_stream_t stream)
+{
+    const char* name = "ivit_gemm_i8_requant_embed_ex";
+    GemmArgs g = gemm_args(A, lda, W, ldw, bias, m, e, out, ldo, M, N, K);
+    g.res = kpos; g.ldr = N;
+    g.cls_row = cls_row;
+    g.tokens = tokens;
+    g.M_main = ivit_dyadic_to_double(m1, e1);
+    g.M_res = ivit_dyadic_to_double(m2, e2);
+    residual_f32_form(g);
+    IVIT_REQUIRE(g.M_main < 1048576.0 && g.M_res < 1048576.0, "%s: residual multiplier >= 2^20 is outside the int8 fast path", name);
+    IVIT_REQUIRE(tokens >= 2 && M > 0 && ((int64_t)M + M / (tokens - 1) + 16) * ldo < 4294967296ll && (int64_t)tokens * N < 4294967296ll,
+                 "%s: tokens=%d below 2, or an output of 4 GiB or more", name, tokens);
+    if (const int rc = gemm_layouts(g, layouts, LAYOUTS_EMBED, name)) return rc;
+    return launch_gemm<EPI_EMBED>(g, name, stream);
+}
+
 IVIT_EXPORT int ivit_gemm_i8_requant_residual_i16_ex(const int8_t* A, int64_t lda, const int8_t* W, int64_t ldw,
                                                   const int32_t* bias, const uint32_t* m, const int32_t* e,
                                                   const int16_t* res, int64_t ldr, uint32_t m_main, int32_t e_main,
@@ -1476,14 +1508,16 @@
 IVIT_EXPORT int ivit_gemm_plan(int epilogue, int M, int N, int K, int layouts, int32_t* out8)
 {
     alignas(16) static int8_t operand[16];
-    static const int allowed[] = {LAYOUTS_RQ, LAYOUTS_IN, LAYOUTS_IN, 0, LAYOUTS_IN, 0, LAYOUTS_RQ16_RES16};
+    static const int allowed[] = {LAYOUTS_RQ, LAYOUTS_IN, LAYOUTS_IN, 0, LAYOUTS_IN, 0, LAYOUTS_RQ16_RES16, 0, LAYOUTS_EMBED};
     const char* name = "ivit_gemm_plan";
-    IVIT_REQUIRE(out8 && epilogue >= EPI_RQ && epilogue <= EPI_RQ16_RES16, "%s: NULL out8 or epilogue %d outside IVIT_GEMM_EPI_*", name, epilogue);
+    IVIT_REQUIRE(out8 && ((epilogue >= EPI_RQ && epilogue <= EPI_RQ16_RES16) || epilogue == EPI_EMBED),
+                 "%s: NULL out8 or epilogue %d outside IVIT_GEMM_EPI_*", name, epilogue);
     const bool qkv = epilogue == EPI_QKV;
     GemmArgs g = gemm_args(operand, K, operand, K, reinterpret_cast<const int32_t*>(operand), reinterpret_cast<const uint32_t*>(operand),
                            reinterpret_cast<const int32_t*>(operand), operand, qkv ? 0 : N, M, N, K);
     g.res = operand; g.ldr = N;
-    g.tokens = 1; g.heads = N / 16; g.head_dim = 16;
+    g.cls_row = operand;
+    g.tokens = epilogue == EPI_EMBED ? 2 : 1; g.heads = N / 16; g.head_dim = 16;
     if (const int rc = gemm_layouts(g, layouts, allowed[epilogue], name)) return rc;
     IVIT_REQUIRE(epilogue != EPI_RQ16_RES16 || g.w_frags || !g.a_blocks, "%s: layouts is 0 or IVIT_W_FRAGS (| IVIT_A_BLOCKS)", name);
     if (const int rc = gemm_check(epilogue, g, name, 1)) return rc;
diff --git a/i-vit_amd/csrc/gemm_common.h b/i-vit_amd/csrc/gemm_common.h
--- a/i-vit_amd/csrc/gemm_common.h
+++ b/i-vit_amd/csrc/gemm_common.h
@@ -37,7 +37,7 @@
 constexpr int W_OFF = BM * BK;
 constexpr int SMEM_BYTES = 2 * STAGE_BYTES;
 
-enum { EPI_RQ = 0, EPI_RESID = 1, EPI_QKV = 2, EPI_I32 = 3, EPI_RESID16 = 4, EPI_RQ16 = 5, EPI_RQ16_RES16 = 6 };
+enum { EPI_RQ = 0, EPI_RESID = 1, EPI_QKV = 2, EPI_I32 = 3, EPI_RESID16 = 4, EPI_RQ16 = 5, EPI_RQ16_RES16 = 6, EPI_EMBED = 8 };
 constexpr int EPI_NARROW_MID = 0x100, EPI_NARROW_OUT = 0x200;
 constexpr int epi_kind(int epiw) { return epiw & 0xff; }
 constexpr int epi_lo(int epiw, int flag) { return (epiw & flag) ? -8 : -128; }
@@ -73,6 +73,7 @@
     int w_frags;
     unsigned long long* stamp;
     const int8_t* lut;
+    const int8_t* cls_row;
 };
 
 IVIT_DEV int swz(int r, int c) { return r * BK + ((c ^ ((r >> 2) & 3)) << 4); }
@@ -450,7 +451,8 @@
     constexpr int EPI = epi_kind(EPIW);
     constexpr int QLO = epi_lo(EPIW, EPI_NARROW_MID), QHI = epi_hi(EPIW, EPI_NARROW_MID);
     constexpr int RLO = epi_lo(EPIW, EPI_NARROW_OUT), RHI = epi_hi(EPIW, EPI_NARROW_OUT);
-    static_assert(NJ % 4 == 0 && (EPI == EPI_RQ || EPI == EPI_RESID || EPI == EPI_QKV), "direct epilogue: int8 outputs");
+    constexpr bool RES = EPI == EPI_RESID || EPI == EPI_EMBED;
+    static_assert(NJ % 4 == 0 && (EPI == EPI_RQ || RES || EPI == EPI_QKV), "direct epilogue: int8 outputs");
     __builtin_amdgcn_s_setprio(2);
     hook.issue();
     const unsigned rq_a = lds_addr(rq_lds) + 8u * (unsigned)(wch + 4 * g4);
@@ -459,7 +461,7 @@
     const int c = ncol + 16 * g4;
     constexpr int NB = NJ / 4;
     unsigned D[NB][4][4];
-    int4 rv[EPI == EPI_RESID ? NB : 1][4];
+    int4 rv[RES ? NB : 1][4];
     v4f lhbuf[2][2];
     lds_read16_async(lhbuf[0][0], rq_a);
     lds_read16_async(lhbuf[0][1], rq_a + 16u);
@@ -517,6 +519,24 @@
                 for (int j = 0; j < 4; ++j) {
                     const int t = min(m0 + 16 * (4 * b2 + j) + l15, g.M - 1);
                     rv[b2][j] = *reinterpret_cast<const int4*>(g.res + ((unsigned)t * (unsigned)g.ldr + (unsigned)min(c, g.N - 16)));
+                }
+            }
+        }
+        if constexpr (EPI == EPI_EMBED) {
+            if (bi == 0) {
+                const unsigned np = (unsigned)g.tokens - 1u, r0 = (unsigned)(m0 + l15);
+                unsigned p = r0 % np;
+#pragma unroll
+                for (int s = 0; s < NJ; ++s) {
+                    if (s > 0) {
+                        if (np >= 16u) {
+                            p += 16u;
+                            if (p >= np) p -= np;
+                        } else {
+                            p = (r0 + 16u * (unsigned)s) % np;
+                        }
+                    }
+                    rv[s >> 2][s & 3] = *reinterpret_cast<const int4*>(g.res + ((p + 1u) * (unsigned)g.ldr + (unsigned)min(c, g.N - 16)));
                 }
             }
         }
@@ -541,10 +561,18 @@
     } else if (EPI == EPI_RQ && g.out_blocks) {
         off0 = block_off(block_row(m0 + l15, g.N), block_col(min(c, g.N - 16)));
         ostep = (unsigned)(g.N >> 6) * 1024u;
+    } else if constexpr (EPI == EPI_EMBED) {
+        const int np = g.tokens - 1;
+        q_b = (int)((unsigned)(m0 + l15) / (unsigned)np);
+        q_tok = m0 + l15 - q_b * np;
+        off0 = (unsigned)(m0 + l15 + 1) * (unsigned)g.ldo + (unsigned)c;
+        ostep = 16u * (unsigned)g.ldo;
     } else {
         off0 = (unsigned)(m0 + l15) * (unsigned)g.ldo + (unsigned)c;
         ostep = 16u * (unsigned)g.ldo;
     }
+    int4 clsv = make_int4(0, 0, 0, 0);
+    if constexpr (EPI == EPI_EMBED) clsv = *reinterpret_cast<const int4*>(g.cls_row + min(c, g.N - 16));
     if constexpr (ABL & 2048) st[4] = __builtin_amdgcn_s_memtime();
 #pragma unroll
     for (int bi = 0; bi < NB; ++bi) {
@@ -562,7 +590,7 @@
             const v2u ac = __builtin_amdgcn_permlane16_swap(ab.x, cd.x, false, false);
             const v2u bd = __builtin_amdgcn_permlane16_swap(ab.y, cd.y, false, false);
             int v[4] = {(int)ac.x, (int)ac.y, (int)bd.x, (int)bd.y};
-            if constexpr (EPI == EPI_RESID) {
+            if constexpr (RES) {
                 if constexpr (ABL & 4096) residual_chunk_f32<RLO, RHI>(v, rv[bi][j], g.Mf_main, g.Mf_res, magic_v);
                 else residual_chunk_f64<RLO, RHI>(v, rv[bi][j], g.M_main, g.M_res);
             }
@@ -590,6 +618,19 @@
                     }
                 }
                 off = off0 + (unsigned)((q_b * g.heads * g.tokens + q_tok) * g.head_dim);
+            } else if constexpr (EPI == EPI_EMBED) {
+                const int np = g.tokens - 1;
+                if (jb + j > 0) {
+                    if (np >= 16) {
+                        q_tok += 16;
+                        if (q_tok >= np) { q_tok -= np; ++q_b; }
+                    } else {
+                        q_b = (int)((unsigned)t / (unsigned)np);
+                        q_tok = t - q_b * np;
+                    }
+                }
+                off = off0 + (unsigned)(jb + j) * ostep + (unsigned)q_b * (unsigned)g.ldo;
+                if (col_ok && t < g.M && q_tok == 0) *reinterpret_cast<int4*>(out + off - (unsigned)g.ldo) = clsv;
             } else {
                 off = off0 + (unsigned)(jb + j) * ostep;
             }
diff --git a/i-vit_amd/csrc/rowops.hip b/i-vit_amd/csrc/rowops.hip
--- a/i-vit_amd/csrc/rowops.hip
+++ b/i-vit_amd/csrc/rowops.hip
@@ -1,4 +1,6 @@
 #include <limits.h>
+
+#include <type_traits>
 
 #include "common.h"
 #include "rowsum.h"
@@ -1052,6 +1054,53 @@
         int64_t row = ((int64_t)b * g + py) * g + px;
         int col = (c * patch + kh) * patch + kw;
         *reinterpret_cast<int*>(A + row * lda + col) = pack4(t[v & 255], t[(v >> 8) & 255], t[(v >> 16) & 255], t[v >> 24]);
+    }
+}
+
+template <typename TP>
+__global__ __launch_bounds__(NT) void patchify_blocks_kernel(const TP* img, int8_t* A, int batch, int chans, int hw, float inv_scale,
+                                                             const int8_t* lut)
+{
+    constexpr bool U8 = sizeof(TP) == 1;
+    typedef typename std::conditional<U8, uint4, float4>::type V;
+    constexpr int NV = U8 ? 1 : 4;
+    __shared__ int8_t s_lut[U8 ? 4 * 256 : 4];
+    if constexpr (U8) {
+        for (int i = threadIdx.x; i < chans * 256; i += NT) s_lut[i] = lut[i];
+        __syncthreads();
+    }
+    const unsigned lane = threadIdx.x & 63, wave = __builtin_amdgcn_readfirstlane(threadIdx.x >> 6);
+    const unsigned g = (unsigned)hw >> 4, np = g * g, rows = (unsigned)batch * np;
+    const unsigned items = ((rows + 15) >> 4) * (unsigned)chans;
+    const unsigned r = lane >> 2, c = (lane & 3) ^ ((lane >> 4) & 3);
+    for (unsigned it = blockIdx.x * WPB + wave; it < items; it += gridDim.x * WPB) {
+        const unsigned R = it / (unsigned)chans, ch = it - R * (unsigned)chans;
+        const unsigned t = 16 * R + r, tc = min(t, rows - 1);
+        const unsigned b = tc / np, p = tc - b * np, py = p / g, px = p - py * g;
+        const TP* src = img + ((size_t)(b * (unsigned)chans + ch) * hw + (16 * py + c)) * hw + 16 * px;
+        V v[4][NV];
+#pragma unroll
+        for (int kq = 0; kq < 4; ++kq)
+#pragma unroll
+            for (int q = 0; q < NV; ++q) v[kq][q] = reinterpret_cast<const V*>(src + (size_t)(4 * kq) * hw)[q];
+        int8_t* dst = A + ((size_t)R * (4 * (unsigned)chans) + 4 * ch) * 1024 + lane * 16;
+#pragma unroll
+        for (int kq = 0; kq < 4; ++kq) {
+            int o[4];
+            if constexpr (U8) {
+                const int8_t* tb = s_lut + 256 * ch;
+                const unsigned w[4] = {v[kq][0].x, v[kq][0].y, v[kq][0].z, v[kq][0].w};
+#pragma unroll
+                for (int q = 0; q < 4; ++q) o[q] = pack4(tb[w[q] & 255], tb[(w[q] >> 8) & 255], tb[(w[q] >> 16) & 255], tb[w[q] >> 24]);
+            } else {
+#pragma unroll
+                for (int q = 0; q < 4; ++q)
+                    o[q] = pack4(quant_sym_i8(v[kq][q].x, inv_scale), quant_sym_i8(v[kq][q].y, inv_scale), quant_sym_i8(v[kq][q].z, inv_scale),
+                                 quant_sym_i8(v[kq][q].w, inv_scale));
+            }
+            const bool live = t < rows;
+            *reinterpret_cast<int4*>(dst + 1024 * kq) = make_int4(live ? o[0] : 0, live ? o[1] : 0, live ? o[2] : 0, live ? o[3] : 0);
+        }
     }
 }
 
@@ -1894,6 +1943,42 @@
 }
 
 template <typename TP>
+static int launch_patchify_blocks(const char* who, const TP* img, int8_t* A, int batch, int chans, int hw, int patch, float inv_scale,
+                                  const int8_t* lut, ivit_stream_t stream)
+{
+    constexpr bool U8 = sizeof(TP) == 1;
+    IVIT_REQUIRE(img && A && (lut || !U8), "%s: NULL operand", who);
+    IVIT_REQUIRE(batch > 0 && chans > 0 && (!U8 || chans <= 4), "%s: batch=%d chans=%d (at least 1%s)", who, batch, chans,
+                 U8 ? ", at most 4 channels" : "");
+    IVIT_REQUIRE(patch == 16 && hw > 0 && hw % 16 == 0, "%s: the block layout is written for 16 x 16 patches (hw=%d patch=%d)", who, hw, patch);
+    IVIT_REQUIRE(((uintptr_t)img % 16 == 0) && ((uintptr_t)A % 16 == 0), "%s: misaligned", who);
+    const int64_t rows = (int64_t)batch * (hw / 16) * (hw / 16);
+    IVIT_REQUIRE((rows + 15) * chans * 256 < 2147483648ll, "%s: a block-layout operand of 2 GiB or more", who);
+    const int64_t items = (rows + 15) / 16 * chans;
+    hipLaunchKernelGGL(patchify_blocks_kernel<TP>, dim3(grid_for_rows(items)), dim3(NT), 0, ivit_stream(stream), img, A, batch, chans, hw,
+                       inv_scale, lut);
+    IVIT_CHECK_LAUNCH(who);
+}
+
+IVIT_EXPORT int ivit_quantize_patchify_f32_i8_ex(const float* img, int8_t* A, int batch, int chans, int hw, int patch, float inv_scale,
+                                                 int layouts, ivit_stream_t stream)
+{
+    const char* who = "ivit_quantize_patchify_f32_i8_ex";
+    IVIT_REQUIRE(layouts == 0 || layouts == 1, "%s: layouts=%d is neither 0 (rows) nor 1 (blocks)", who, layouts);
+    if (!layouts) return launch_patchify(who, img, A, (int64_t)chans * patch * patch, batch, chans, hw, patch, inv_scale, stream);
+    return launch_patchify_blocks<float>(who, img, A, batch, chans, hw, patch, inv_scale, nullptr, stream);
+}
+
+IVIT_EXPORT int ivit_quantize_patchify_u8_i8_ex(const uint8_t* img, int8_t* A, int batch, int chans, int hw, int patch, const int8_t* lut,
+                                                int layouts, ivit_stream_t stream)
+{
+    const char* who = "ivit_quantize_patchify_u8_i8_ex";
+    IVIT_REQUIRE(layouts == 0 || layouts == 1, "%s: layouts=%d is neither 0 (rows) nor 1 (blocks)", who, layouts);
+    if (!layouts) return ivit_quantize_patchify_u8_i8(img, A, (int64_t)chans * patch * patch, batch, chans, hw, patch, lut, stream);
+    return launch_patchify_blocks<uint8_t>(who, img, A, batch, chans, hw, patch, 0.0f, lut, stream);
+}
+
+template <typename TP>
 static int launch_patchify_hw(const char* who, const TP* img, int8_t* A, int64_t lda, int batch, int chans, int h, int w, int patch,
                               float inv_scale, const int8_t* lut, ivit_stream_t stream)
 {
diff --git a/i-vit_amd/engine.py b/i-vit_amd/engine.py
--- a/i-vit_amd/engine.py
+++ b/i-vit_amd/engine.py
@@ -106,6 +106,8 @@
             self.pos_add = dev(pos_add.astype(np.int16))
             self.cls_row = dev(cls_row.astype(np.int8))
         self.embed_me = (int(m1[0]), int(e1[0]))
+        self.kpos = dev(kpos.astype(np.int8)) if sb == 8 else None
+        self.pos_me = (int(m2[0]), int(e2[0]))
 
         self.blocks = []
         for i in range(depth):
@@ -173,6 +175,7 @@
         self.gelu_in_place = True
         self.fuse_res16 = True
         self.fuse_ibert_gelu = True
+        self.fused_stem = None
         self.probe = None
         self._alloc(max_batch)
         self._compact(True)
@@ -184,7 +187,7 @@
         M16 = (M + 15) // 16 * 16
         i8 = dict(dtype=torch.int8, device=self.dev)
         self.ws = dict(
-            a0=torch.empty(B * self.NP, 3 * self.P * self.P, **i8),
+            a0=torch.empty((B * self.NP + 15) // 16 * 16, 3 * self.P * self.P, **i8),
             pe=torch.empty(B * self.NP, C, **i8),
             x=torch.empty(M, C, **i8), x2=torch.empty(M, C, **i8), h=torch.empty(M16, C, **i8),
             qkv=torch.empty(3 * M * C, **i8), ao=torch.empty(M16, C, **i8),
@@ -260,11 +263,26 @@
         if probe is not None:
             probe.end("gemm_resid", st, (M, lin["N"], lin["K"]))
 
-    def _patchify(self, images, B, st):
+    def _stem_weight(self, B, taps):
+        K = 3 * self.P * self.P
+        on = gemm_forms.tiles_fit(self.C) if self.fused_stem is None else self.fused_stem
+        if (not on or self.stream_bits != 8 or taps is not None or self.IMG_H != self.IMG_W or self.P != 16 or not self.block_operands
+                or (B * self.NP + 15) * K >= 1 << 31):
+            return None
+        W, bit = gemm_forms.weight(self.patch, gemm_forms.EMBED, B * self.NP, frags=self.weight_frags, blocks=False)
+        return W if bit == gemm_forms.W_FRAGS16 else None
+
+    def _patchify(self, images, B, st, blocks=False):
         ws = self.ws
         if images.dtype == torch.uint8 and self.input_lut is None:
             self.set_input_normalisation()
-        if self.IMG_H != self.IMG_W:
+        if blocks:
+            if images.dtype == torch.uint8:
+                _lib.call("ivit_quantize_patchify_u8_i8_ex", _lib.ptr(images), _lib.ptr(ws["a0"]), B, 3, self.IMG, self.P,
+                          _lib.ptr(self.input_lut), 1, st)
+            else:
+                _lib.call("ivit_quantize_patchify_f32_i8_ex", _lib.ptr(images), _lib.ptr(ws["a0"]), B, 3, self.IMG, self.P, self.inv_s0, 1, st)
+        elif self.IMG_H != self.IMG_W:
             if images.dtype == torch.uint8:
                 _lib.call("ivit_quantize_patchify_hw_u8_i8", _lib.ptr(images), _lib.ptr(ws["a0"]), 3 * self.P * self.P, B, 3, self.IMG_H,
                           self.IMG_W, self.P, _lib.ptr(self.input_lut), st)
@@ -421,8 +439,15 @@
                     t = ws["untile"]
                 taps[name] = t.reshape(-1)[: int(np.prod(shape))].view(shape).clone()
 
-        self._patchify(images, B, st)
-        if wide:
+        stem_w = self._stem_weight(B, taps)
+        self._patchify(images, B, st, blocks=stem_w is not None)
+        if stem_w is not None:
+            pt, K0 = self.patch, 3 * self.P * self.P
+            _lib.call("ivit_gemm_i8_requant_embed_ex", _lib.ptr(ws["a0"]), K0, _lib.ptr(stem_w), K0, _lib.ptr(pt["b"]), _lib.ptr(pt["m"]),
+                      _lib.ptr(pt["e"]), _lib.ptr(self.kpos), _lib.ptr(self.cls_row), *self.embed_me, *self.pos_me, _lib.ptr(ws["x"]), C,
+                      B * self.NP, C, K0, T, gemm_forms.A_BLOCKS | gemm_forms.W_FRAGS16, st)
+            x, x2 = ws["x"], ws["x2"]
+        elif wide:
             pt = self.patch
             _lib.call("ivit_gemm_i8_requant_i16", _lib.ptr(ws["a0"]), 3 * self.P * self.P, _lib.ptr(pt["W"]), pt["K"], _lib.ptr(pt["b"]),
                       _lib.ptr(pt["m"]), _lib.ptr(pt["e"]), _lib.ptr(ws["pe16"]), C, B * self.NP, C, pt["K"], st)
@@ -432,7 +457,9 @@
                        blocks=bool(self.block_operands), bits=self.stream_bits)
             tap("patch_embed.qact", ws["pe"], (B, self.NP, C))
             x, x2 = ws["x"], ws["x2"]
-        if self.stream_bits == 4:
+        if stem_w is not None:
+            pass
+        elif self.stream_bits == 4:
             _lib.call("ivit_embed_assemble_i8_bits", _lib.ptr(ws["pe"]), _lib.ptr(self.pos_add), _lib.ptr(self.cls_row), self.embed_me[0],
                       self.embed_me[1], _lib.ptr(x), B, T, C, 4, st)
         else:
diff --git a/i-vit_amd/gemm_forms.py b/i-vit_amd/gemm_forms.py
--- a/i-vit_amd/gemm_forms.py
+++ b/i-vit_amd/gemm_forms.py
@@ -3,15 +3,16 @@
 A_BLOCKS, W_BLOCKS, OUT_BLOCKS, W_FRAGS, W_FRAGS16 = 1, 2, 4, 8, 16
 FRAGS = W_FRAGS | W_FRAGS16
 RQ, RESID, QKV, I32, RESID16, RQ16, RQ16_RES16 = range(7)
+EMBED = 8
 SMALL, PERS, WREG, WREG16, SKINNY = range(5)
 LAYOUTS = {RQ: A_BLOCKS | W_BLOCKS | OUT_BLOCKS | FRAGS, RESID: A_BLOCKS | W_BLOCKS | FRAGS, QKV: A_BLOCKS | W_BLOCKS | FRAGS, I32: 0,
-           RESID16: A_BLOCKS | W_BLOCKS | FRAGS, RQ16: 0, RQ16_RES16: A_BLOCKS | W_FRAGS}
+           RESID16: A_BLOCKS | W_BLOCKS | FRAGS, RQ16: 0, RQ16_RES16: A_BLOCKS | W_FRAGS, EMBED: A_BLOCKS | W_FRAGS16}
 
 BIG_MIN_M, BIG_MIN_N = 2048, 128
 SK_MIN_M, SK_MAXK, SK_MAXN = 8192, 128, 320
 WR_CH, WR_WASTE_DEN = 256, 8
 
-_INT8_OUT = (RQ, RESID, QKV)
+_INT8_OUT = (RQ, RESID, QKV, EMBED)
 _NO_TILE_LOOP = (I32, RQ16)
 
 
@@ -63,6 +64,8 @@
         return SKINNY
     if layouts & (A_BLOCKS | W_BLOCKS) and not layouts & FRAGS and not pers_applies(epi, M, N):
         return None
+    if epi == EMBED and not layouts & W_FRAGS16:
+        return None
     if layouts & FRAGS:
         bit = layouts & FRAGS
         if layouts & W_BLOCKS or not frags_apply(epi, M, N, K, bit):
diff --git a/include/ivit_hip.h b/include/ivit_hip.h
--- a/include/ivit_hip.h
+++ b/include/ivit_hip.h
@@ -38,6 +38,10 @@
                                      float inv_scale, ivit_stream_t stream);
 int ivit_quantize_patchify_u8_i8(const uint8_t* img, int8_t* A, int64_t lda, int batch, int chans, int hw, int patch,
                                  const int8_t* lut, ivit_stream_t stream);
+int ivit_quantize_patchify_f32_i8_ex(const float* img, int8_t* A, int batch, int chans, int hw, int patch, float inv_scale,
+                                     int layouts, ivit_stream_t stream);
+int ivit_quantize_patchify_u8_i8_ex(const uint8_t* img, int8_t* A, int batch, int chans, int hw, int patch, const int8_t* lut,
+                                    int layouts, ivit_stream_t stream);
 int ivit_quantize_patchify_hw_f32_i8(const float* img, int8_t* A, int64_t lda, int batch, int chans, int h, int w, int patch,
                                      float inv_scale, ivit_stream_t stream);
 int ivit_quantize_patchify_hw_u8_i8(const uint8_t* img, int8_t* A, int64_t lda, int batch, int chans, int h, int w, int patch,
@@ -129,6 +133,7 @@
 #define IVIT_GEMM_EPI_RESID16 4
 #define IVIT_GEMM_EPI_RQ16 5
 #define IVIT_GEMM_EPI_RQ16_RES16 6
+#define IVIT_GEMM_EPI_EMBED 8
 #define IVIT_GEMM_FORM_SMALL 0
 #define IVIT_GEMM_FORM_PERS 1
 #define IVIT_GEMM_FORM_WREG 2
@@ -231,6 +236,10 @@
                            int32_t e, int8_t* out, int batch, int tokens, int C, ivit_stream_t stream);
 int ivit_embed_assemble_i8_bits(const int8_t* patch, const int16_t* pos_add, const int8_t* cls_row, uint32_t m,
                                 int32_t e, int8_t* out, int batch, int tokens, int C, int bits, ivit_stream_t stream);
+int ivit_gemm_i8_requant_embed_ex(const int8_t* A, int64_t lda, const int8_t* W, int64_t ldw, const int32_t* bias,
+                                  const uint32_t* m, const int32_t* e, const int8_t* kpos, const int8_t* cls_row,
+                                  uint32_t m1, int32_t e1, uint32_t m2, int32_t e2, int8_t* out, int64_t ldo,
+                                  int M, int N, int K, int tokens, int layouts, ivit_stream_t stream);
 
 int ivit_embed_assemble_i16(const int16_t* patch, const int32_t* pos_add, const int16_t* cls_row, uint32_t m,
                             int32_t e, int16_t* out, int batch, int tokens, int C, ivit_stream_t stream);
```

Result: no change. 45750 images/s, median of 6 (+0.7%).
